# iceprincefounder/ZeldaEngine

Hardware: AMD Instinct MI355X
Metric: Mpixels/s shaded (deferred PBR, 1080p, 100k meshlets) + achieved HBM GB/s (higher is better)
Workload: dtype f32

## Files before the change

### include/zelda_render.h

```cpp
#ifndef ZELDA_RENDER_H
#define ZELDA_RENDER_H

#include "zelda_abi.h"

#ifdef __cplusplus
extern "C" {
#endif

#define ZR_OK            0
#define ZR_ERR_ARG      -1
#define ZR_ERR_DEVICE   -2
#define ZR_ERR_OOM      -3
#define ZR_ERR_PARSE    -4
#define ZR_ERR_IO       -5
#define ZR_ERR_STATE    -6
#define ZR_ERR_OVERFLOW -7
#define ZR_ERR_UNSUPPORTED -8

#define ZR_ABI_VERSION 7u

#ifndef ZR_TILE
#define ZR_TILE 32
#endif

// ... 90 lines not shown
int  zr_object_set_instance_visibility(zr_ctx* ctx, uint32_t index, uint32_t first, const uint8_t* visible, uint32_t n);
int  zr_object_update_instance_visibility_async(zr_ctx* ctx, uint32_t index, uint32_t first, const uint32_t* idx_dev,
                                                const uint8_t* visible_dev, uint32_t n, void* hip_stream);
int  zr_object_get_visibility(zr_ctx* ctx, uint32_t index, int* object_visible, uint8_t* dst, uint32_t* n);
int  zr_mesh_set_vertices(zr_ctx* ctx, uint32_t mesh_id, uint32_t first, const XkVertex* v, uint32_t n);
int  zr_mesh_update_vertices_async(zr_ctx* ctx, uint32_t mesh_id, uint32_t first, const XkVertex* v_dev, uint32_t n, void* hip_stream);
int  zr_mesh_get_vertices(zr_ctx* ctx, uint32_t mesh_id, XkVertex* dst, uint32_t* n);
int  zr_object_set_texture(zr_ctx* ctx, uint32_t index, uint32_t slot, const zr_image* img);
int  zr_object_update_texture_async(zr_ctx* ctx, uint32_t index, uint32_t slot, const void* rgba8_dev, uint32_t width, uint32_t height,
                                    void* hip_stream);
int  zr_object_get_texture(zr_ctx* ctx, uint32_t index, uint32_t slot, uint32_t level, uint8_t* dst, size_t cap, uint32_t* w, uint32_t* h,
                           uint32_t* levels);
int  zr_set_cubemap(zr_ctx* ctx, const uint8_t* const faces[6], uint32_t dim);

int  zr_set_skydome(zr_ctx* ctx, const XkVertex* v, uint32_t nv, const uint32_t* idx, uint32_t ni, const zr_image* tex);
int  zr_set_background(zr_ctx* ctx, const zr_image* tex);
int  zr_set_sky_flags(zr_ctx* ctx, int enable_skydome, int enable_background);

int  zr_update_uniforms(zr_ctx* ctx, const zr_camera* cam,
                        const XkLight* dir, uint32_t n_dir, const XkLight* point, uint32_t n_point,
                        const XkLight* spot, uint32_t n_spot, float roll_stage, float roll_light, float time);
int  zr_set_frame(zr_ctx* ctx, const XkUniformBufferMVP* camera, const XkUniformBufferMVP* shadow, const XkView* view);
int  zr_get_frame(zr_ctx* ctx, XkUniformBufferMVP* camera, XkUniformBufferMVP* shadow, XkView* view);
int  zr_set_debug_view(zr_ctx* ctx, uint32_t spec_constants);
#define ZR_SHADING_DEFERRED 0u
#define ZR_SHADING_FORWARD  1u
int  zr_set_shading(zr_ctx* ctx, uint32_t mode);

int  zr_render(zr_ctx* ctx);
int  zr_render_shadow(zr_ctx* ctx);
int  zr_render_gbuffer(zr_ctx* ctx);
int  zr_render_lighting(zr_ctx* ctx);
int  zr_render_geometry(zr_ctx* ctx);
int  zr_stream_wait_shadow(zr_ctx* ctx, void* hip_stream);
int  zr_finish(zr_ctx* ctx);
int  zr_get_pass_times(zr_ctx* ctx, float ms[ZR_PASS_COUNT]);
int  zr_get_pass_times_avg(zr_ctx* ctx, uint32_t last_n, float ms[ZR_PASS_COUNT]);
int  zr_get_frame_latencies(zr_ctx* ctx, uint32_t n, float* ms);
int  zr_get_frame_periods(zr_ctx* ctx, uint32_t n, float* ms);
int  zr_set_timing_interval(zr_ctx* ctx, uint32_t interval);
int  zr_get_stats(zr_ctx* ctx, zr_stats* out, size_t bytes);
#define ZR_LIGHT_PLANE_IGNORED 0u
#define ZR_LIGHT_PLANE_FILLED  1u
#define ZR_LIGHT_PLANE_READ    2u
typedef struct zr_light_keep {
    uint32_t last, _pad;
    uint64_t ignored, filled, read;
    uint64_t plane_bytes;
    uint64_t read_by_arg;
} zr_light_keep;
int  zr_get_light_keep(zr_ctx* ctx, zr_light_keep* out, size_t bytes);
int  zr_get_rest_settled(zr_ctx* ctx, uint32_t* parts, uint32_t* settled);
int  zr_get_rest_settled_parts(zr_ctx* ctx, uint8_t* standing, size_t bytes);

int  zr_read_color(zr_ctx* ctx, uint8_t* rgba8, size_t bytes);
int  zr_read_gbuffer(zr_ctx* ctx, int target, void* dst, size_t bytes);
int  zr_read_shadowmap(zr_ctx* ctx, float* dst, size_t bytes);
int  zr_copy_frame_async(zr_ctx* ctx, void* color_dev, void* shadow_dev);

typedef struct zr_frame_delta {
    uint32_t n_tiles;
    uint32_t total_tiles;
    uint32_t full;
    uint32_t serial;
} zr_frame_delta;
int  zr_set_frame_delta(zr_ctx* ctx, int enable);
int  zr_frame_delta_reset(zr_ctx* ctx);
int  zr_read_frame_delta(zr_ctx* ctx, uint32_t* tiles, uint32_t cap_tiles, uint8_t* pixels, size_t bytes, zr_frame_delta* out, size_t out_bytes);
int  zr_copy_frame_delta_async(zr_ctx* ctx, void* header_dev, void* tiles_dev, void* pixels_dev);

#define ZR_FRAME_DELTA_PACKED 3
#define ZR_FRAME_DELTA_RECORD_MAX 4104u
typedef struct zr_frame_delta_packed {
    uint32_t n_tiles, total_tiles, full, serial;
    uint32_t bytes;
    uint32_t raw_tiles;
    uint32_t reserved[2];
} zr_frame_delta_packed;
int  zr_read_frame_delta_packed(zr_ctx* ctx, uint32_t* tiles, uint32_t cap_tiles, uint32_t* offsets, uint32_t cap_offsets, uint8_t* stream, size_t cap_bytes,
                                zr_frame_delta_packed* out, size_t out_bytes);
int  zr_copy_frame_delta_packed_async(zr_ctx* ctx, void* header_dev, void* tiles_dev, void* offsets_dev, void* stream_dev);
int  zr_frame_delta_decode(const uint32_t* tiles, const uint32_t* offsets, uint32_t n, const uint8_t* stream, size_t bytes, uint32_t width, uint32_t height,
                           uint8_t* client_rgba8);

int  zr_frame_scaled_extent(uint32_t width, uint32_t height, uint32_t scale, uint32_t* w, uint32_t* h);
int  zr_frame_downscale(const uint8_t* rgba8, uint32_t width, uint32_t height, uint32_t scale, uint8_t* dst, size_t bytes);
int  zr_read_color_scaled(zr_ctx* ctx, uint32_t scale, uint8_t* rgba8, size_t bytes);
int  zr_copy_frame_scaled_async(zr_ctx* ctx, uint32_t scale, void* color_dev);
int  zr_set_frame_delta_scale(zr_ctx* ctx, uint32_t scale);
int  zr_get_frame_delta_extent(zr_ctx* ctx, uint32_t* width, uint32_t* height, uint32_t* total_tiles, uint32_t* scale);

typedef struct zr_highlight_style {
    uint8_t  outline[4];
    uint8_t  fill[4];
    uint32_t radius;
    uint32_t reserved;
} zr_highlight_style;
int  zr_highlight_set(zr_ctx* ctx, uint32_t object, uint32_t first, const uint8_t* on, uint32_t n);
int  zr_highlight_clear(zr_ctx* ctx);
int  zr_highlight_get(zr_ctx* ctx, uint8_t* dst, size_t bytes);
int  zr_set_highlight_style(zr_ctx* ctx, const zr_highlight_style* style, size_t bytes);
int  zr_get_highlight_style(zr_ctx* ctx, zr_highlight_style* style, size_t bytes);
int  zr_read_color_highlighted(zr_ctx* ctx, uint32_t scale, uint8_t* rgba8, size_t bytes);
int  zr_copy_frame_highlighted_async(zr_ctx* ctx, uint32_t scale, void* color_dev);
int  zr_set_frame_delta_highlight(zr_ctx* ctx, int on);
int  zr_frame_highlight(const uint8_t* rgba8, const uint8_t* mask, uint32_t width, uint32_t height, const zr_highlight_style* style, size_t style_bytes,
// ... 113 lines not shown
```

### zeldaengine_amd/abi.py

```python
import ctypes as C

import numpy as np

MAX_DIRECTIONAL_LIGHTS = 16
MAX_POINT_LIGHTS = 512
MAX_SPOT_LIGHTS = 16
SHADOWMAP_DIM = 1024
TILE = 32

XkVertex = np.dtype([("Position", "<f4", 3), ("Normal", "<f4", 3), ("Color", "<f4", 3), ("TexCoord", "<f4", 2)])
XkInstanceData = np.dtype([("InstancePosition", "<f4", 3), ("InstanceRotation", "<f4", 3), ("InstancePScale", "<f4"),
                           ("InstanceTexIndex", "u1"), ("_pad", "u1", 3)])
XkMeshlet = np.dtype([("VertexOffset", "<u4"), ("VertexCount", "<u4"), ("TriangleOffset", "<u4"), ("TriangleCount", "<u4"),
                      ("BoundsCenter", "<f4", 3), ("BoundsRadius", "<f4"), ("ConeApex", "<f4", 3), ("ConeAxis", "<f4", 3),
                      ("ConeCutoff", "<f4"), ("BindlessContext", "<u4")])
XkMeshletFileVertex = np.dtype([("pos", "<f4", 3), ("nrm", "<f4", 3), ("uv", "<f4", 2)])
XkLight = np.dtype([("Position", "<f4", 4), ("Color", "<f4", 4), ("Direction", "<f4", 4), ("LightInfo", "<f4", 4)])
XkUniformBufferMVP = np.dtype([("Model", "<f4", 16), ("View", "<f4", 16), ("Proj", "<f4", 16)])
XkView = np.dtype([("ViewProjSpace", "<f4", 16), ("ShadowmapSpace", "<f4", 16), ("LocalToWorld", "<f4", 16),
                   ("CameraInfo", "<f4", 4), ("ViewportInfo", "<f4", 4),
                   ("DirectionalLights", XkLight, MAX_DIRECTIONAL_LIGHTS), ("PointLights", XkLight, MAX_POINT_LIGHTS),
                   ("SpotLights", XkLight, MAX_SPOT_LIGHTS), ("LightsCount", "<i4", 4),
                   ("Time", "<f4"), ("zNear", "<f4"), ("zFar", "<f4")])

# ... 38 lines not shown
    "zr_copy_frame_scaled_async": [vp_, u32_, vp_],
    "zr_set_frame_delta_scale": [vp_, u32_],
    "zr_get_frame_delta_extent": [vp_, C.POINTER(u32_), C.POINTER(u32_), C.POINTER(u32_), C.POINTER(u32_)],
}
FRAME_SCALE_MAX = 8


class HighlightStyle(C.Structure):
    _fields_ = [("outline", C.c_uint8 * 4), ("fill", C.c_uint8 * 4), ("radius", C.c_uint32), ("reserved", C.c_uint32)]


assert C.sizeof(HighlightStyle) == 16
HIGHLIGHT_RADIUS_MAX = 8
HIGHLIGHT_SIGNATURES = {
    "zr_highlight_set": [vp_, u32_, u32_, vp_, u32_],
    "zr_highlight_clear": [vp_],
    "zr_highlight_get": [vp_, vp_, C.c_size_t],
    "zr_set_highlight_style": [vp_, C.POINTER(HighlightStyle), C.c_size_t],
    "zr_get_highlight_style": [vp_, C.POINTER(HighlightStyle), C.c_size_t],
    "zr_read_color_highlighted": [vp_, u32_, vp_, C.c_size_t],
    "zr_copy_frame_highlighted_async": [vp_, u32_, vp_],
    "zr_set_frame_delta_highlight": [vp_, C.c_int],
    "zr_frame_highlight": [vp_, vp_, u32_, u32_, C.POINTER(HighlightStyle), C.c_size_t, vp_, C.c_size_t],
}


class OverlaySegment(C.Structure):
    _fields_ = [("a", C.c_float * 3), ("b", C.c_float * 3), ("rgba", C.c_uint8 * 4), ("flags", C.c_uint32)]


class OverlayStyle(C.Structure):
    _fields_ = [("depth_bias", C.c_float), ("hidden_opacity", C.c_uint32), ("reserved", C.c_uint32 * 2)]


assert C.sizeof(OverlaySegment) == 32 and C.sizeof(OverlayStyle) == 16
OVERLAY_SEGMENT = np.dtype([("a", "<f4", 3), ("b", "<f4", 3), ("rgba", "u1", 4), ("flags", "<u4")])
assert OVERLAY_SEGMENT.itemsize == 32
OVERLAY_XRAY = 1
OVERLAY_MAX_SEGMENTS = 16384
OVERLAY_SIGNATURES = {
    "zr_overlay_set": [vp_, vp_, u32_],
    "zr_overlay_get": [vp_, vp_, C.POINTER(u32_)],
    "zr_set_overlay_style": [vp_, C.POINTER(OverlayStyle), C.c_size_t],
    "zr_get_overlay_style": [vp_, C.POINTER(OverlayStyle), C.c_size_t],
    "zr_read_color_overlaid": [vp_, u32_, C.c_int, vp_, C.c_size_t],
    "zr_copy_frame_overlaid_async": [vp_, u32_, C.c_int, vp_],
    "zr_set_frame_delta_overlay": [vp_, C.c_int],
    "zr_frame_overlay": [vp_, vp_, u32_, u32_, vp_, vp_, u32_, C.POINTER(OverlayStyle), C.c_size_t, vp_, C.c_size_t],
}
REST_SETTLE_SIGNATURES = {
    "zr_get_rest_settled": [C.c_void_p, C.POINTER(C.c_uint32), C.POINTER(C.c_uint32)],
    "zr_get_rest_settled_parts": [C.c_void_p, C.c_void_p, C.c_size_t],
}
EXTENT_SIGNATURES = {
    "zr_resize": [vp_, u32_, u32_],
    "zr_get_extent": [vp_, C.POINTER(u32_), C.POINTER(u32_)],
}
del vp_, u32_


def make_highlight_style(outline=(255, 160, 0, 255), fill=(255, 160, 0, 0), radius=2):
    return HighlightStyle((C.c_uint8 * 4)(*outline), (C.c_uint8 * 4)(*fill), radius, 0)


def make_overlay_style(depth_bias=0.0, hidden_opacity=0):
    return OverlayStyle(depth_bias, hidden_opacity, (C.c_uint32 * 2)(0, 0))


def make_overlay_segments(segments):
    if isinstance(segments, np.ndarray) and segments.dtype == OVERLAY_SEGMENT:
        return np.ascontiguousarray(segments).reshape(-1)
    rows = [tuple(s) for s in segments]
    out = np.zeros(len(rows), dtype=OVERLAY_SEGMENT)
    for i, s in enumerate(rows):
        out[i]["a"], out[i]["b"], out[i]["rgba"], out[i]["flags"] = s[0:3], s[3:6], s[6:10], s[10] if len(s) > 10 else 0
    return out


class Camera(C.Structure):
    _fields_ = [("Position", C.c_float * 3), ("Lookat", C.c_float * 3), ("Speed", C.c_float), ("FOV", C.c_float),
                ("zNear", C.c_float), ("zFar", C.c_float)]


class Config(C.Structure):
    _fields_ = [("width", C.c_uint32), ("height", C.c_uint32), ("shadow_dim", C.c_uint32), ("debug_view", C.c_uint32),
                ("device", C.c_int32), ("tile_rank", C.c_uint32), ("tile_world", C.c_uint32), ("flags", C.c_uint32)]


class Stats(C.Structure):
    _fields_ = [("work_items", C.c_uint64 * 2), ("survivors", C.c_uint64 * 2), ("bin_entries", C.c_uint64 * 2),
                ("covered_pixels", C.c_uint64), ("covered_shadow_texels", C.c_uint64), ("overflow", C.c_uint32), ("hiz_culled", C.c_uint32),
                ("round1_survivors", C.c_uint64), ("shadow_occluded", C.c_uint32), ("shadow_late", C.c_uint32),
                ("hiz_culled_geom", C.c_uint32), ("struct_bytes", C.c_uint32)]


class LightKeep(C.Structure):
    _fields_ = [("last", C.c_uint32), ("_pad", C.c_uint32), ("ignored", C.c_uint64), ("filled", C.c_uint64), ("read", C.c_uint64),
                ("plane_bytes", C.c_uint64), ("read_by_arg", C.c_uint64)]


LIGHT_PLANE_IGNORED, LIGHT_PLANE_FILLED, LIGHT_PLANE_READ = 0, 1, 2


class WorldDelta(C.Structure):
    _fields_ = [("struct_bytes", C.c_uint32), ("differs", C.c_uint32), ("scene_changed", C.c_uint32), ("objects_kept", C.c_uint32),
                ("objects_reinstanced", C.c_uint32), ("objects_added", C.c_uint32), ("objects_removed", C.c_uint32),
# ... 98 lines not shown
```

### zeldaengine_amd/csrc/zr_context.cpp

```cpp
#include "zr_ctx.h"
#include "zr_math.h"

#include <algorithm>
#include <cmath>
#include <cstring>
#include <cstdlib>

int zr_fail(zr_ctx* c, int code, const std::string& msg)
{
    if (c) { try { c->err = msg; } catch (...) { c->err.clear(); } }
    return code;
}

int zr_stage_idle(zr_ctx* c, const char* what, bool hint)
{
    if (c->stage == 0) return ZR_OK;
    return zr_fail(c, ZR_ERR_STATE, std::string(what) + (hint ? " between the stages of a frame (finish it with zr_render_lighting first)"
                                                              : " between the stages of a frame"));
}

hipError_t zr_sync_all(zr_ctx* c)
{
    hipError_t e = hipStreamSynchronize(c->stream);
    if (e == hipSuccess && c->cam_s) e = hipStreamSynchronize(c->cam_s);
// ... 30 lines not shown

#ifndef ZR_CAM_PRIORITY
#define ZR_CAM_PRIORITY 0
#endif
#ifndef ZR_TILE_WG_PER_CU
#define ZR_TILE_WG_PER_CU 12u
#endif

static int create_device_state(zr_ctx* c)
{
    ZrOwn& A = c->own;
    HIPCHK(c, A.stream(&c->own_stream));
    c->stream = c->own_stream;
    for (auto& fr : c->timed) for (auto& e : fr.ev) HIPCHK(c, A.event(&e));
    for (auto& e : c->ev_end) HIPCHK(c, A.event(&e));
    for (FrameCopy& F : c->fc) HIPCHK(c, A.event(&F.ev_ids, hipEventDisableTiming));
    for (FrameCopy& F : c->fc) {
        HIPCHK(c, A.alloc(&F.shadow, (size_t)c->SD * c->SD)); HIPCHK(c, A.alloc(&F.view, 1)); HIPCHK(c, A.alloc(&F.empty_rgba, 1));
    }
    HIPCHK(c, A.alloc(&c->d_stats, 1));
    HIPCHK(c, A.alloc(&c->d_sstats, 1));
    for (auto& r : c->d_rstats) HIPCHK(c, A.alloc(&r, 1));
    c->cov_block = c->d_stats;
    HIPCHK(c, A.alloc(&c->d_lut, 256));
    HIPCHK(c, hipMemcpy(c->d_lut, c->lut, sizeof c->lut, hipMemcpyHostToDevice));
    {
        std::vector<float> ul(1280);
        for (int i = 0; i < 256; ++i) {
            ul[(size_t)i] = (float)i / 255.0f;
            if (fmaf((float)i, ZR_UNORM8_HI, (float)i * ZR_UNORM8_LO) != ul[(size_t)i])
                return zr_fail(c, ZR_ERR_DEVICE, "ZR_UNORM8_HI / ZR_UNORM8_LO do not decode c / 255 exactly");
        }
        for (int i = 0; i < 1024; ++i) ul[256 + (size_t)i] = (float)i / 1023.0f;
        HIPCHK(c, A.alloc(&c->d_unorm_lut, ul.size()));
        HIPCHK(c, hipMemcpy(c->d_unorm_lut, ul.data(), ul.size() * 4, hipMemcpyHostToDevice));
    }

    c->stiles_x = (c->SD + ZR_TILE - 1) / ZR_TILE; c->stiles_y = c->stiles_x; c->sn_tiles = c->stiles_x * c->stiles_y;
    if (c->sn_tiles > 16000u) return zr_fail(c, ZR_ERR_ARG, "too many tiles");
    std::vector<uint32_t> sowned(c->sn_tiles);
    for (uint32_t t = 0; t < c->sn_tiles; ++t) sowned[t] = t;
    HIPCHK(c, upload(A, &c->d_sowned, sowned));
    {
        HIPCHK(c, A.alloc(&c->d_clear_px, 64));
        uint32_t px[16] = { 0 };
        px[0] = 0x3F800000u;
        px[1] = 0xFF000000u; px[2] = 0u; px[3] = 0xFF000000u; px[4] = 0xFF000000u;
        px[6] = 0u; px[7] = 0x3C000000u;
        px[8] = 0u;
        HIPCHK(c, hipMemcpy(c->d_clear_px, px, sizeof px, hipMemcpyHostToDevice));
        uint32_t* w = (uint32_t*)c->d_clear_px;
        c->Gclear.depth = (float*)w; c->Gclear.scene_color = w + 1; c->Gclear.gA = w + 2; c->Gclear.gB = w + 3; c->Gclear.gC = w + 4;
        c->Gclear.gD = (uint2*)(w + 6); c->Gclear.overlay = w + 8;
    }
    {
#ifdef ZR_DIAG
        const char* e;
        if ((e = getenv("ZR_DEBUG_SKIP"))) c->env_skip = (uint32_t)atoi(e);
        if ((e = getenv("ZR_DEBUG_SKIP_LIGHT"))) c->env_skip_light = (uint32_t)atoi(e);
        if ((e = getenv("ZR_LIGHT_LIST_MIN"))) c->env_light_list_min = atoi(e);
        c->env_no_empty_px = getenv("ZR_NO_EMPTY_PIXEL") != nullptr;
#endif
        c->lk.settle_off = getenv("ZR_NO_REST_SETTLE") != nullptr;
        c->end.every = ZR_REST_END_EVERY_DEFAULT;
        if (const char* r = getenv("ZR_REST_END_EVERY")) { const int v = atoi(r); c->end.every = v < 1 ? 1u : (uint32_t)v > kZrEndEveryMax ? kZrEndEveryMax : (uint32_t)v; }
    }
    HIPCHK(c, A.host(&c->h_view_ring, zr_ctx::VIEW_RING));
    for (auto& e : c->view_ev) HIPCHK(c, A.event(&e, hipEventDisableTiming));
    {
        int least = 0, greatest = 0;
        (void)hipDeviceGetStreamPriorityRange(&least, &greatest);
        HIPCHK(c, A.stream(&c->cam_s, ZR_CAM_PRIORITY == 2 ? greatest : ZR_CAM_PRIORITY == 1 ? (least + greatest) / 2 : least));
    }
    HIPCHK(c, A.event(&c->ev_cam, hipEventDisableTiming)); HIPCHK(c, A.event(&c->ev_join, hipEventDisableTiming));
    HIPCHK(c, A.event(&c->ev_lane, hipEventDisableTiming));
    { hipDeviceProp_t prop; if (hipGetDeviceProperties(&prop, c->device) == hipSuccess && prop.multiProcessorCount > 0) c->raster_blocks = (uint32_t)prop.multiProcessorCount * ZR_TILE_WG_PER_CU; }
    c->shadow_blocks = c->raster_blocks / ZR_TILE_WG_PER_CU * 8u;
    c->slow0_cap = std::max<uint32_t>(c->slow0_cap, 128u * c->sn_tiles);
    HIPCHK(c, A.alloc(&c->d_slow0, 4ull * c->slow0_cap));
#ifdef ZR_DIAG
    if (const char* e = getenv("ZR_RASTER_BLOCKS")) c->raster_blocks = (uint32_t)std::max(1, atoi(e));
    if (const char* e = getenv("ZR_SHADOW_BLOCKS")) c->shadow_blocks = (uint32_t)std::max(1, atoi(e));
#endif
    HIPCHK(c, zr_fill_sync({ { c->d_stats, 0, sizeof(ZrDevStats) }, { c->d_sstats, 0, sizeof(ZrDevStats) },
                             { c->d_rstats[0], 0, sizeof(ZrDevStats) }, { c->d_rstats[1], 0, sizeof(ZrDevStats) } }));
    if (int rc = zr_extent_create(c)) return rc;
    for (auto& fr : c->timed) for (auto& e : fr.ev) HIPCHK(c, hipEventRecord(e, c->stream));
    for (auto& e : c->ev_end) HIPCHK(c, hipEventRecord(e, c->stream));
    for (auto& e : c->view_ev) HIPCHK(c, hipEventRecord(e, c->stream));
    HIPCHK(c, hipStreamSynchronize(c->stream));
    return ZR_OK;
}

extern "C" int zr_create(const zr_config* cfg, zr_ctx** out)
{
    if (!cfg || !out) return ZR_ERR_ARG;
    return zr_guard(nullptr, [&]() -> int {
        *out = nullptr;
        if (cfg->width == 0 || cfg->height == 0 || cfg->width > 255u * ZR_TILE || cfg->height > 255u * ZR_TILE) return ZR_ERR_ARG;
        int ndev = 0;
        if (hipGetDeviceCount(&ndev) != hipSuccess || ndev <= 0) return ZR_ERR_DEVICE;
        if (cfg->device < 0 || cfg->device >= ndev) return ZR_ERR_DEVICE;
        if (hipSetDevice(cfg->device) != hipSuccess) return ZR_ERR_DEVICE;
        zr_ctx* c = new zr_ctx();
        c->cfg = *cfg;
        if (c->cfg.tile_world == 0) c->cfg.tile_world = 1;
// ... 63 lines not shown
```

### zeldaengine_amd/csrc/zr_ctx.h

```cpp
#pragma once

#include <atomic>
#include <functional>
#include <initializer_list>
#include <map>
#include <mutex>
#include <new>
#include <stdexcept>
#include <string>
#include <thread>
#include <utility>
#include <vector>

#include "zr_frame_end.h"
#include "zr_frame_plan.h"
#include "zr_ids.h"
#include "zr_meshlet.h"
#include "zr_overlay.h"
#include "zr_scale.h"
#include "zr_settle.h"
#include "zr_timed.h"
#include "zr_types.h"
#include "zr_world_doc.h"

// ... 59 lines not shown
    ZrMeshletSet ms;
    bool has_meshlets = false, uploaded = false;
    float center[3] = { 0, 0, 0 }; float radius = 0;
    XkVertex* d_v = nullptr; ZrRVertex* d_rv = nullptr; ZrRVertex* d_rt = nullptr; uint32_t* d_idx = nullptr; XkMeshlet* d_meshlets = nullptr;
    float4* d_mpos = nullptr; float4* d_mbox = nullptr; uint2* d_mtri = nullptr; uint32_t* d_tri_meshlet = nullptr;
    ZrMeshState upd = {}; bool stale[2] = { false, false }, v_stale = false, ml_stale = false;
};

struct ZrMaterialHost {
    uint32_t texel[7]; float bc_linear[3];
    std::vector<uint8_t> image[7];
    uint32_t w[7], h[7];
};

struct ZrSceneObject {
    ZrOwn mem;
    ZrOwn tex_mem;
    uint32_t mesh = 0, n_inst = 1; bool instanced = false;
    std::vector<XkInstanceData> inst;
    ZrInstance* d_inst = nullptr;
    XkInstanceData* d_raw = nullptr;
    ZrInstanceState upd = {}; uint32_t pending[2] = { 0, 0 }; bool tab1 = false, host_stale = false; uint32_t draw = 0;
    bool hidden = false, flag_pending[2] = { false, false }, vis_stale = false;
    std::vector<uint8_t> vis;
    uint32_t texel[7]; float bc_linear[3];
    uint8_t* d_tex[8] = { nullptr, nullptr, nullptr, nullptr, nullptr, nullptr, nullptr, nullptr };
    uint32_t tex_w[8] = { 0 }, tex_h[8] = { 0 }, tex_levels[8] = { 0 };
    bool mixed_sizes = false;
    std::string profab; uint32_t profab_model = 0; bool from_world = false, mat_pristine = false;
    uint32_t work_base = 0, work_inst = 0, work_meshlets = 0; bool work_valid = false;
};

static const struct { uint32_t ch, n; } kSlotPack[7] = { { ZR_PK_BC, 3 }, { ZR_PK_ME, 1 }, { ZR_PK_RO, 1 }, { ZR_PK_NO, 3 }, { ZR_PK_AO, 1 }, { ZR_PK_EM, 3 }, { ZR_PK_MS, 1 } };
static inline uint32_t zr_mip_next(uint32_t d) { return d > 1 ? d >> 1 : 1; }
struct ZrMipLevel { uint32_t w, h; size_t off; };
static inline ZrMipLevel zr_mip_level(uint32_t w, uint32_t h, uint32_t level)
{
    ZrMipLevel L = { w, h, 0 };
    for (uint32_t l = 0; l < level; ++l) { L.off += (size_t)L.w * L.h; L.w = zr_mip_next(L.w); L.h = zr_mip_next(L.h); }
    return L;
}

struct ZrProfab { uint32_t mesh; ZrMaterialHost mat; };

struct FrameCopy {
    GBufferPtrs G = {};
    float* shadow = nullptr; XkView* view = nullptr;
    uint32_t* empty_rgba = nullptr;
    uint32_t* prim_plane = nullptr;
    bool overlay_dirty = false;
    bool shadow_cleared = false;
    uint64_t view_uploaded = 0;
    uint64_t g_gen = 0;
    hipEvent_t ev_ids = nullptr; bool ids_wait = false;
};

struct ZrDeltaBuffers {
    ZrOwn mem, codec_mem;
    uint32_t *delivered = nullptr, *list = nullptr, *header = nullptr, *scaled = nullptr; uint8_t *packed = nullptr, *flags = nullptr;
    zr_frame_delta* h_header = nullptr;
    struct Codec {
        bool on = false; uint16_t* lens = nullptr; uint32_t *header = nullptr, *offsets = nullptr; uint8_t* stream = nullptr;
        zr_frame_delta_packed* h_header = nullptr;
    } codec;
};

struct zr_ctx {
    ZrOwn own, ext, pool_tiles;
    zr_config cfg;
    int device = 0;
    hipStream_t own_stream = nullptr, stream = nullptr;
    std::string err;

    std::vector<ZrMesh> meshes;
    std::vector<ZrSceneObject> objects;
    bool scene_dirty = true;
    ZrObject* d_objs = nullptr; uint32_t n_objs = 0, n_work = 0;
    ZrObject* d_objs_b[2] = { nullptr, nullptr }; ZrOwn tables;
    struct Update {
        uint64_t reader[2] = { 0, 0 };
        hipEvent_t ev_scatter = nullptr, ev_apply = nullptr; hipStream_t scatter_s = nullptr, apply_s = nullptr;
        bool scatter_wait[2] = { false, false }, apply_done = false, dual = false;
        static constexpr int RING = 4;
        struct Stage { ZrOwn mem; uint8_t* h = nullptr; uint8_t* d = nullptr; size_t cap = 0; hipEvent_t ev = nullptr; } ring[RING];
        uint32_t slot = 0;
        hipEvent_t ev_tex = nullptr; hipStream_t tex_s = nullptr; bool tex_wait = false; float* d_srgb_thr = nullptr;
    } upd;
    ZrFrameFacts facts; ZrFramePlan plan; ZrFrameCarry carry;
    ZrPass list_key[2] = {}, smap_key = {}, cam_prev_key = {};
    ZrPass pass[2]; bool pass_live[2] = { false, false };
    uint64_t caster_epoch = 0, camera_epoch = 0, surface_epoch = 0;
    int smap = 0; uint64_t shadow_draws = 0, cam_draws = 0;

    XkUniformBufferMVP cam, shadow; XkView view; bool frame_valid = false;
    struct Lens { bool valid = false; float fov = 0, zn = 0, zf = 0; } lens;
    uint32_t debug_view = 0;
    uint32_t shading = 0;

    uint32_t W = 0, H = 0, SD = 0;
    uint32_t tiles_x = 0, tiles_y = 0, n_tiles = 0, n_owned = 0, slots_per_rank = 0;
    uint32_t stiles_x = 0, stiles_y = 0, sn_tiles = 0;
    uint32_t *d_owned = nullptr, *d_sowned = nullptr;
    uint32_t* d_tile_map = nullptr;
    struct ZrDist* dist = nullptr;
    uint32_t* d_color = nullptr; uint32_t* d_tiles = nullptr;
    float* d_shadow_ext = nullptr;
    uint32_t shadow_rank = 0, shadow_world = 1; int stage = 0;
    uint32_t stile_rank = 0, stile_world = 1, s_slots_per_rank = 0, n_sowned_rank = 0;
    uint32_t *d_sowned_rank = nullptr, *d_stile_map = nullptr; ZrOwn stile_mem;
    uint32_t* d_tiles_ext = nullptr;

    ZrOwn pools;
    struct CullList { uint32_t *rects = nullptr, *work = nullptr; } sc[2];
    struct ShadowBins { uint32_t *tile_count = nullptr, *tile_offset = nullptr, *tile_cursor = nullptr, *chunk_offset = nullptr;
                        ZrBinEntry* bins = nullptr; uint4* chunk_tab = nullptr; } sb;
    uint32_t bucket_pct = 100;
    ZrTriBins tb = {};
    uint32_t chunk_capacity = 0;
    uint32_t n_inst_total = 0;
    uint8_t* d_clear_px = nullptr; GBufferPtrs Gclear = {}; bool empty_ready = false;
    uint32_t env_skip = 0, env_skip_light = 0; int32_t env_light_list_min = 4; bool env_no_empty_px = false;
    static constexpr int VIEW_RING = kZrViewRing;
    XkView* h_view_ring = nullptr; hipEvent_t view_ev[VIEW_RING] = {}; uint32_t view_slot = 0; bool view_dirty = true;
    uint64_t view_version = 1;
    FrameCopy fc[2]; int fcur = 0;
    hipStream_t cam_s = nullptr;
    hipEvent_t ev_join = nullptr, ev_cam = nullptr;
    ZrPass resolve_P; uint32_t resolve_mark = 0;
    hipEvent_t ev_lane = nullptr;
    unsigned long long* d_sky_keys = nullptr; uint32_t sky_object = 0;
    static constexpr int END_RING = kZrEndRing;
    hipEvent_t ev_end[END_RING] = {}; ZrEndState end;
    unsigned long long* d_vis[2] = { nullptr, nullptr }; uint32_t raster_blocks = 2048, shadow_blocks = 2048;
    uint4* d_slow0 = nullptr; uint32_t slow0_cap = 1u << 18;
    uint32_t work_capacity = 0, bin_capacity = 0; bool any_images = false, mixed_images = false;
    uint32_t limit_record_chunks = 0, limit_slow_triangles = 0;
    uint2* d_pxrect = nullptr; float* d_zmin = nullptr; uint8_t* d_visflag[2] = { nullptr, nullptr };
    uint2* d_spxrect = nullptr; float* d_szmin = nullptr; uint8_t* d_sflag = nullptr;
    bool history_remap = false; uint64_t history_items = 0;
    uint32_t sflag_turn = 0;
    float* d_hiz = nullptr; ZrHiz hiz = {}; int vis_cur = 0; bool last_two_round = false;
    uint32_t vis_mark_prev = 0;
    uint32_t* d_hiz_regions = nullptr; uint32_t n_hiz_regions = 0;
    ZrDevStats* d_stats = nullptr; ZrDevStats h_stats = {};
    ZrDevStats* d_sstats = nullptr;
    ZrDevStats* d_rstats[2] = { nullptr, nullptr }; ZrDevStats* cov_block = nullptr;
    uint64_t last_work[2] = { 0, 0 };

    bool id_capture = false;
    bool ids_frame = false, ids_this = false;
    uint64_t scene_gen = 0;
    struct Ids {
        uint64_t gen = 0, table_gen = ~0ull;
        ZrOwn table, pool;
        ZrIdsDraw* draws = nullptr; uint32_t n_draws = 0, n_slots = 0, slot_cap = 0;
        uint32_t *counts = nullptr, *cov = nullptr, *list = nullptr, *n = nullptr;
        unsigned long long* keys = nullptr; zr_hit* hits = nullptr; uint2* obj = nullptr;
    } ids;

    struct Delta { bool on = false, full = true; uint32_t serial = 0, scale = 1; ZrDeltaBuffers b; } delta;
    uint32_t* d_scaled = nullptr;
    struct Highlight {
        std::vector<uint8_t> set; uint64_t set_gen = ~0ull; bool dirty = true, delta = false;
        zr_highlight_style style = { { 255, 160, 0, 255 }, { 255, 160, 0, 0 }, 2u, 0u };
        ZrOwn bits_mem; uint32_t* bits = nullptr; size_t bits_words = 0;
        unsigned long long* plane = nullptr; uint32_t* frame = nullptr;
    } hl;

    ZrOwn cube_mem; CubeDesc cube = {}; uint32_t cube_dim = 0, cube_levels = 0;
    uint64_t cube_gen = 0;
    struct LightKey {
        float SB[16], cam[3]; uint32_t SD, n_dir, max_mips, cube_dim, cube_levels, debug_skip;
        XkLight dir[XK_MAX_DIRECTIONAL_LIGHTS_NUM];
// ... 149 lines not shown
```

### zeldaengine_amd/csrc/zr_dev.h

```cpp
#pragma once
#include "zr_math.h"
#include "zr_types.h"

#include <algorithm>
#include <cstddef>

#define WAVE 64
#define TILE ZR_TILE
#define TILE_PIX (TILE * TILE)
#ifndef ZR_SHADOW_APRON
#define ZR_SHADOW_APRON 12
#endif
#define SPAN(MODE) ((MODE) == ZR_MODE_SHADOW ? TILE + ZR_SHADOW_APRON : TILE)
#define SPAN_PIX(MODE) (SPAN(MODE) * SPAN(MODE))
#define QCAP 128u
#define RW (ZR_TILE >= 64 ? 8 : 4)
#define RTHREADS (RW * WAVE)
#ifndef ZR_RASTER_WAVES_DEFER
#define ZR_RASTER_WAVES_DEFER 6
#endif
#ifdef ZR_DIAG
#define ZR_DIAG_SKIP(x) (x)
#else
#define ZR_DIAG_SKIP(x) 0u
// ... 235 lines not shown
    if (VEC) return *reinterpret_cast<const uint4*>(p);
    v.x = p[0];
    if (px + 1u < W) v.y = p[1];
    if (px + 2u < W) v.z = p[2];
    if (px + 3u < W) v.w = p[3];
    return v;
}
template <bool VEC> __device__ __forceinline__ void plane_store4(uint32_t* __restrict__ plane, uint32_t W, uint32_t H, uint32_t px, uint32_t py, uint4 v)
{
    if (py >= H || px >= W) return;
    uint32_t* p = plane + (size_t)py * W + px;
    if (VEC) { *reinterpret_cast<uint4*>(p) = v; return; }
    p[0] = v.x;
    if (px + 1u < W) p[1] = v.y;
    if (px + 2u < W) p[2] = v.z;
    if (px + 3u < W) p[3] = v.w;
}

__device__ __forceinline__ bool hiz_occluded(const ZrHiz& Z, uint2 pr, float zmin)
{
    if (!(zmin >= 0.0f)) return false;
    const uint32_t x0 = pr.x & 0xFFFFu, y0 = pr.x >> 16, x1 = pr.y & 0xFFFFu, y1 = pr.y >> 16;
    uint32_t l = 0;
    while (l < 4u && (((x1 >> (2u + l)) - (x0 >> (2u + l))) > 3u || ((y1 >> (2u + l)) - (y0 >> (2u + l))) > 3u)) ++l;
    const uint32_t sh = 2u + l;
    const uint32_t tx0 = x0 >> sh, ty0 = y0 >> sh, tx1 = x1 >> sh, ty1 = y1 >> sh;
    if (tx1 - tx0 > 3u || ty1 - ty0 > 3u) return false;
    const float* __restrict__ L = l == 0u ? Z.fine : Z.lvl[l - 1u];
    const uint32_t hw = l == 0u ? Z.fw : Z.hw[l - 1u];
    float hmax = 0.0f;
#pragma unroll
    for (uint32_t j = 0; j < 4u; ++j)
#pragma unroll
        for (uint32_t i = 0; i < 4u; ++i)
            hmax = __builtin_fmaxf(hmax, L[(size_t)min(ty0 + j, ty1) * hw + min(tx0 + i, tx1)]);
    return zmin > hmax;
}

#ifndef ZR_LIGHT_TB
#define ZR_LIGHT_TB 512
#endif
#ifndef ZR_LIGHT_WAVES
#define ZR_LIGHT_WAVES 6
#endif
#ifndef ZR_LIGHT_KEPT_TB
#define ZR_LIGHT_KEPT_TB 512
#endif
#ifndef ZR_LIGHT_KEPT_WAVES
#define ZR_LIGHT_KEPT_WAVES 8
#endif
#ifndef ZR_REST_RECORDS_ONE_TRIP
#define ZR_REST_RECORDS_ONE_TRIP 1
#endif
#ifndef ZR_PIXELS_PER_THREAD
#define ZR_PIXELS_PER_THREAD 1
#endif
static_assert(TILE_PIX / ZR_PIXELS_PER_THREAD >= ZR_LIGHT_KEPT_TB, "a tile's threads must fill at least one workgroup");
static_assert(TILE_PIX / ZR_PIXELS_PER_THREAD >= ZR_LIGHT_TB && TILE_PIX / ZR_PIXELS_PER_THREAD >= 256, "a tile's threads must fill at least one workgroup");
#ifndef ZR_RESOLVE_TB
#define ZR_RESOLVE_TB 256
#endif
```

### zeldaengine_amd/csrc/zr_frame_host.cpp

```cpp
#include "zr_ctx.h"
#include "zr_math.h"

#include <cmath>
#include <cstring>

static_assert(ZRP_NO_HIZ == ZR_FLAG_NO_HIZ && ZRP_SERIAL_PASSES == ZR_FLAG_SERIAL_PASSES && ZRP_NO_LIST_REUSE == ZR_FLAG_NO_LIST_REUSE &&
              ZRP_NO_SHADOW_OCCLUSION == ZR_FLAG_NO_SHADOW_OCCLUSION && ZRP_SHADOW_OCCLUSION == ZR_FLAG_SHADOW_OCCLUSION &&
              ZRP_SHADING_FORWARD == ZR_SHADING_FORWARD, "zr_frame_plan.h: flags");
static_assert((int)ZR_ROUNDS_ONE == ZR_PLAN_ONE_ROUND && (int)ZR_ROUNDS_TWO == ZR_PLAN_DREW_ROUND2 && (int)ZR_ROUNDS_TWO_KEPT == ZR_PLAN_KEPT_ROUND2, "zr_frame_plan.h: rounds");
static_assert(ZR_TILE == 32, "the triangle-binned camera pass and the shadow pass's occlusion culling are written for 32 x 32 tiles");


static float radiansf(float deg) { return deg * 0.01745329251994329576923690768489f; }
static void perspective_rh_zo(float fovy, float aspect, float zn, float zf, float* m)
{
    const float t = tanf(fovy / 2.0f);
    memset(m, 0, 64);
    m[0] = 1.0f / (aspect * t); m[5] = 1.0f / t; m[10] = zf / (zn - zf); m[11] = -1.0f; m[14] = -(zf * zn) / (zf - zn);
}
static void look_at_rh(zf3 eye, zf3 center, zf3 up, float* m)
{
    const zf3 f = zr_normalize_ieee(center - eye);
    const zf3 s = zr_normalize_ieee(zr_cross(f, up));
    const zf3 u = zr_cross(s, f);
// ... 336 lines not shown
{
    const ZrFramePlan& p = c->plan;
    if (p.shadow == ZR_LANE_NONE) TIMED(c, EV_SHADOW_BINS, EV_SHADOW);
    else if (int rc = shadow_draw(c, lane_stream(c, p.shadow))) return rc;
    if (p.ev_join) HIPCHK(c, hipEventRecord(c->ev_join, c->stream));
    return ZR_OK;
}

static int gbuffer_pass(zr_ctx* c)
{
    const ZrFramePlan& p = c->plan;
    if (p.camera == ZR_LANE_NONE) {
        TIMED(c, EV_CAMERA, EV_CULL, EV_ROUND1, EV_HIZ, EV_ROUND2, EV_RESOLVE);
        return ZR_OK;
    }
    const hipStream_t s = lane_stream(c, p.camera);
    TIMED(c, EV_CAMERA);
    ZrPass P = c->pass[1];
    c->last_work[1] = P.n_work;
    ZrHiz Z = c->hiz;
    Z.tiles_x = c->tiles_x; Z.tile_rank = c->cfg.tile_rank; Z.tile_world = c->cfg.tile_world;
    Z.pxrect = p.hiz_on ? c->d_pxrect : nullptr; Z.zmin = p.hiz_on ? c->d_zmin : nullptr;
    Z.vis_prev = c->d_visflag[c->vis_cur ^ 1]; Z.vis_now = p.hiz_on ? c->d_visflag[c->vis_cur] : nullptr;
    const uint32_t vis_mark = 1u + (uint32_t)(c->cam_draws % 255u);
    Z.vis_stamp = c->vis_mark_prev;
    Z.phase = 0;
    c->last_two_round = p.rounds != ZR_ROUNDS_ONE;
    zr_launch_cull_box(P, c->d_objs, c->sc[1].work, c->sc[1].rects, Z, c->d_stats, 1, s, c->tb.sel, c->last_two_round ? Z.vis_prev : nullptr, p.camera_list_reuse);
    TIMED(c, EV_CULL);
    if (c->last_two_round) Z.phase = 1;
    tri_raster(c, P, Z, 1, s, p.rounds != ZR_ROUNDS_TWO, p.count_first);
    TIMED(c, EV_ROUND1);
    if (p.rounds == ZR_ROUNDS_TWO) {
        zr_launch_hiz_build(c->d_vis[c->fcur], c->W, c->H, Z, c->d_hiz_regions, c->n_hiz_regions, s);
        Z.phase = 2;
        tri_select(c, P, Z, 2, s);
        TIMED(c, EV_HIZ);
        tri_raster(c, P, Z, 2, s, true, false);
    } else
        TIMED(c, EV_HIZ);
    {
        const bool sky = c->sky_set && c->sky_enabled;
        P.write_overlay = (sky || c->fc[c->fcur].overlay_dirty) ? 1u : 0u;
        c->fc[c->fcur].overlay_dirty = sky;
        P.sky_keys = nullptr; P.sky_object = c->sky_object;
        if (sky && c->d_sky_keys) { zr_launch_sky_tiles(P, c->d_objs, c->d_owned, c->n_owned, c->d_sky_keys, s); P.sky_keys = c->d_sky_keys; }
    }
    TIMED(c, EV_ROUND2);
    if (p.resolve_deferred) {
        zr_launch_mark(P, c->d_objs, c->d_owned, c->n_owned, c->d_vis[c->fcur], Z.vis_now, s, vis_mark);
        TIMED(c, EV_MARK);
        c->resolve_P = P; c->resolve_mark = vis_mark;
    } else {
        zr_launch_resolve_gbuffer(P, c->d_objs, c->d_owned, c->n_owned, c->d_vis[c->fcur], c->fc[c->fcur].G, c->d_lut, c->d_unorm_lut, Z.vis_now, c->d_stats, s, vis_mark);
        c->cov_block = c->d_stats; c->fc[c->fcur].g_gen = p.g_gen;
        TIMED(c, EV_RESOLVE);
    }
    if (p.ev_cam == ZR_EVCAM_BEHIND_MARK || p.ev_cam == ZR_EVCAM_BEHIND_RESOLVE) HIPCHK(c, hipEventRecord(c->ev_cam, s));
    c->vis_mark_prev = vis_mark; c->cam_draws++;
    if (P.n_work != 0) zr_launch_plan(c->tb, c->d_owned, c->n_owned, c->d_stats, false, c->bucket_pct, s, p.rounds);
    if (p.hiz_on) c->vis_cur ^= 1;
    HIPCHK(c, hipGetLastError());
    c->cam_prev_key = c->pass[1]; c->carry = zr_frame_carry(c->carry, c->facts, p, ZR_STAGE_CAMERA);
    return ZR_OK;
}

extern "C" int zr_render_gbuffer(zr_ctx* c)
{
    if (!c) return ZR_ERR_ARG;
    return zr_guard(c, [&]() -> int {
        if (c->stage != 1) return zr_fail(c, ZR_ERR_STATE, "zr_render_gbuffer out of order");
        HIPCHK(c, hipSetDevice(c->device));
        const int rc = gbuffer_pass(c);
        if (rc == ZR_OK) c->stage = 2;
        return rc;
    });
}

extern "C" int zr_stream_wait_shadow(zr_ctx* c, void* hip_stream)
{
    if (!c) return ZR_ERR_ARG;
    return zr_guard(c, [&]() -> int {
        HIPCHK(c, hipStreamWaitEvent((hipStream_t)hip_stream, c->ev_join, 0));
        return ZR_OK;
    });
}

static int geometry_passes(zr_ctx* c, ZrEntry entry)
{
    const ZrFramePlan& p = c->plan;
    int rc = frame_begin(c, entry);
    if (rc == ZR_OK) rc = shadow_pass(c);
    if (rc == ZR_OK) rc = gbuffer_pass(c);
    if (rc == ZR_OK && p.one_pixel == ZR_LANE_CAM) rc = empty_pixel_pass(c);
    if (rc == ZR_OK && (p.ev_cam == ZR_EVCAM_BEHIND_ONE_PIXEL || p.ev_cam == ZR_EVCAM_LANE_END)) HIPCHK(c, hipEventRecord(c->ev_cam, c->cam_s));
    if (rc == ZR_OK) c->stage = 2;
    return rc;
}

extern "C" int zr_render_shadow(zr_ctx* c)
{
    if (!c) return ZR_ERR_ARG;
    return zr_guard(c, [&]() -> int {
        int rc = frame_begin(c, ZR_ENTRY_STAGED);
        if (rc == ZR_OK) rc = shadow_pass(c);
        if (rc == ZR_OK) c->stage = 1;
        return rc;
    });
}

extern "C" int zr_render_geometry(zr_ctx* c)
{
    if (!c) return ZR_ERR_ARG;
    return zr_guard(c, [&]() -> int { return geometry_passes(c, ZR_ENTRY_GEOMETRY); });
}

static int deferred_resolve(zr_ctx* c)
{
    const hipStream_t s = lane_stream(c, c->plan.resolve);
    ZrDevStats* const tally = c->d_rstats[c->fcur];
    zr_launch_fill32(tally->covered_part, 0u, 32, s);
    TIMED(c, EV_HOST_RESOLVE);
    zr_launch_resolve_gbuffer(c->resolve_P, c->d_objs, c->d_owned, c->n_owned, c->d_vis[c->fcur], c->fc[c->fcur].G, c->d_lut, c->d_unorm_lut, nullptr, tally, s, c->resolve_mark);
    TIMED(c, EV_RESOLVE);
    c->cov_block = tally; c->fc[c->fcur].g_gen = c->plan.g_gen;
    HIPCHK(c, hipGetLastError());
    return ZR_OK;
}

extern "C" int zr_render_lighting(zr_ctx* c)
{
    if (!c) return ZR_ERR_ARG;
    return zr_guard(c, [&]() -> int {
        if (c->stage != 2) return zr_fail(c, ZR_ERR_STATE, "zr_render_lighting out of order");
        HIPCHK(c, hipSetDevice(c->device));
        const ZrFramePlan& p = c->plan;
        if (p.host_waits_ev_cam) HIPCHK(c, hipStreamWaitEvent(lane_stream(c, p.lighting), c->ev_cam, 0));
        int rc = p.resolve_deferred ? deferred_resolve(c) : ZR_OK;
        if (rc == ZR_OK && p.one_pixel != ZR_LANE_CAM) rc = empty_pixel_pass(c);
        if (rc == ZR_OK) rc = lighting_pass(c);
        return rc;
    });
}

extern "C" int zr_render(zr_ctx* c)
{
    if (!c) return ZR_ERR_ARG;
    return zr_guard(c, [&]() -> int {
        int rc = geometry_passes(c, ZR_ENTRY_RENDER);
        if (rc == ZR_OK) rc = zr_render_lighting(c);
        if (rc != ZR_OK) c->stage = 0;
        return rc;
    });
}

extern "C" int zr_set_shadow_partition(zr_ctx* c, uint32_t rank, uint32_t world)
{
    if (!c) return ZR_ERR_ARG;
    return zr_guard(c, [&]() -> int {
        ARGCHK(c, world >= 1 && rank < world);
        if (world > 1 && c->stile_world > 1) return zr_fail(c, ZR_ERR_STATE, "zr_set_shadow_partition: the map is already owned by tiles (zr_set_shadow_tiles)");
        c->shadow_rank = rank; c->shadow_world = world; zr_casters_changed(c);
        return ZR_OK;
    });
}

extern "C" int zr_set_shadow_tiles(zr_ctx* c, uint32_t rank, uint32_t world)
{
    if (!c) return ZR_ERR_ARG;
    return zr_guard(c, [&]() -> int {
        ARGCHK(c, world >= 1 && rank < world);
        if (int rc = zr_stage_idle(c, "zr_set_shadow_tiles", false)) return rc;
        if (world > 1 && c->shadow_world > 1) return zr_fail(c, ZR_ERR_STATE, "zr_set_shadow_tiles: the casters are already split by instance (zr_set_shadow_partition)");
        HIPCHK(c, hipSetDevice(c->device));
        HIPCHK(c, zr_sync_all(c));
        c->stile_mem.release(); c->d_sowned_rank = c->d_stile_map = nullptr;
        c->stile_rank = 0; c->stile_world = 1; c->s_slots_per_rank = c->sn_tiles; c->n_sowned_rank = 0;
        zr_history_forgotten(c, ZR_HIST_SHADOW_LIST); zr_casters_changed(c);
// ... 52 lines not shown
```

### zeldaengine_amd/csrc/zr_lighting.hip

```cpp
#include "zr_dev.h"
#include "zr_surface.h"
#include "zr_shade.h"

__device__ __forceinline__ bool light_pixel_empty(uint32_t sc, uint32_t A, uint32_t B, uint32_t Cc, uint2 D)
{
    return sc == 0xFF000000u && A == 0u && B == 0xFF000000u && Cc == 0xFF000000u && D.x == 0u && D.y == 0x3C000000u;
}

struct LitPixel { zf3 BaseColor, Normal, N, Pw; float Metallic, Roughness, AO, Mask; };
__device__ __forceinline__ LitPixel light_decode(const float* u8, const float* u10, uint32_t sc, uint32_t A, uint32_t B, uint32_t Cc, uint2 D)
{
    LitPixel q;
    q.BaseColor = zr3(u8[Cc & 255u], u8[(Cc >> 8) & 255u], u8[(Cc >> 16) & 255u]);
    q.Metallic = zr_saturate(u8[B & 255u]);
    q.Roughness = zr_saturate(u8[(B >> 16) & 255u]);
    q.Normal = zr3(__builtin_fmaf(u10[(A >> 20) & 1023u], 2.0f, -1.0f), __builtin_fmaf(u10[(A >> 10) & 1023u], 2.0f, -1.0f),
                   __builtin_fmaf(u10[A & 1023u], 2.0f, -1.0f));
    q.AO = zr_saturate(u8[Cc >> 24]);
    q.Mask = u8[sc >> 24];
    q.Roughness = __builtin_fmaxf(0.01f, q.Roughness);
    q.N = zr_normalize(q.Normal);
    q.Pw = zr3(f16_to_f32_hw(D.x & 0xFFFFu), f16_to_f32_hw(D.x >> 16), f16_to_f32_hw(D.y & 0xFFFFu));
    return q;
}
__device__ __forceinline__ uint32_t light_compose(const ZrLightParams& L, const LitPixel& q, zf3 Direct, zf3 Indirect, zf3 RefC, float ShadowFactor, int px, int py)
{
    zf3 Final = ((Direct + Indirect) + RefC) * q.Mask;
    Final = gamma3(Final);
    zf3 o;
    switch (L.debug_view) {
    case 0: o = Final; break;
    case 1: o = gamma3(q.BaseColor); break;
    case 2: o = zr3(q.Metallic, q.Metallic, q.Metallic); break;
    case 3: o = zr3(q.Roughness, q.Roughness, q.Roughness); break;
    case 4: o = q.Normal; break;
    case 5: o = zr3(q.AO, q.AO, q.AO); break;
    case 7: o = RefC; break;
    case 8: o = zr3(ShadowFactor, ShadowFactor, ShadowFactor); break;
    case 9: o = Final; break;
    case 6: {
        const float u = ((float)px + 0.5f) / (float)L.W, v = ((float)py + 0.5f) / (float)L.H;
        o = v >= u ? zr3(1.0f - v, u, v - u) : zr3(1.0f - u, v, u - v);
        break;
    }
    default: o = Final * ShadowFactor; break;
    }
    return pack_rgb8(o);
}
template <int TB>
__device__ __forceinline__ void light_clear_next_slice(const ZrLightParams& L)
{
    if (!L.clear_next) return;
    const uint32_t per = (L.clear_n + gridDim.x - 1u) / gridDim.x, b = blockIdx.x * per;
    for (uint32_t i = threadIdx.x; i < per && b + i < L.clear_n; i += (uint32_t)TB) L.clear_next[b + i] = 0x3F800000u;
}

template <bool LIGHT_LIST, bool BACKGROUND, int TB, int PPT, uint32_t MODE>
__global__ __launch_bounds__(TB) __attribute__((amdgpu_waves_per_eu(MODE == ZR_LIGHT_KEPT ? ZR_LIGHT_KEPT_WAVES : ZR_LIGHT_WAVES, MODE == ZR_LIGHT_KEPT ? ZR_LIGHT_KEPT_WAVES : ZR_LIGHT_WAVES))) void k_lighting(ZrLightParams L, const XkView* __restrict__ view,
                                                  const uint32_t* __restrict__ owned_tiles, GBufferPtrs G,
                                                  const float* __restrict__ shadowmap, CubeDesc C,
                                                  const float* __restrict__ srgb_lut, const float* __restrict__ unorm_lut,
                                                  uint32_t* __restrict__ out, float4* __restrict__ plane, float4* __restrict__ rest)
{
    __shared__ float tl[512];
    __shared__ float u10[1024];
    float* const slut = tl; float* const u8 = tl + 256;
    constexpr uint32_t T = TILE_PIX / (uint32_t)PPT, PARTS = T / (uint32_t)TB, WAVES = (uint32_t)TB / 64u;
    const uint32_t tid = threadIdx.x + (blockIdx.x % PARTS) * (uint32_t)TB;
    const uint32_t tile_slot = blockIdx.x / PARTS;
    for (uint32_t i = threadIdx.x; i < 256u; i += (uint32_t)TB) { u8[i] = unorm_lut[i]; slut[i] = srgb_lut[i]; }
    for (uint32_t i = threadIdx.x; i < 1024u; i += (uint32_t)TB) u10[i] = unorm_lut[256u + i];
    __syncthreads();
    light_clear_next_slice<TB>(L);
    const uint32_t tile = owned_tiles[tile_slot];
    const int tx0 = (int)(tile % L.tiles_x) * TILE, ty0 = (int)(tile / L.tiles_x) * TILE;
    const zf3 cam = zr3(view->CameraInfo[0], view->CameraInfo[1], view->CameraInfo[2]);
    const uint32_t nDir = (uint32_t)view->LightsCount[0], nPoint = (uint32_t)view->LightsCount[1];
    const float maxmips = (float)(uint32_t)view->LightsCount[3];
    const float dxy = 1.5f * 1.0f / (float)L.SD;

    __shared__ float bbp[LIGHT_LIST ? WAVES : 1][6];
    __shared__ uint32_t lmask[LIGHT_LIST ? XK_MAX_POINT_LIGHTS_NUM / 32 : 1];
    constexpr bool use_mask = LIGHT_LIST;
    constexpr bool RECORDS = MODE == ZR_LIGHT_FILL && PPT == 1;
    if constexpr (LIGHT_LIST || RECORDS) {
        float lo[3] = { __builtin_inff(), __builtin_inff(), __builtin_inff() }, hi[3] = { -__builtin_inff(), -__builtin_inff(), -__builtin_inff() };
        bool odd = false;
        bool empty = false;
        for (uint32_t i = tid; i < TILE_PIX; i += T) {
            const int px = tx0 + (int)(i & (TILE - 1)), py = ty0 + (int)(i / TILE);
            if (px >= (int)L.W || py >= (int)L.H) continue;
            const size_t p = (size_t)py * L.W + (size_t)px;
            if constexpr (RECORDS) empty = light_pixel_empty(G.scene_color[p], G.gA[p], G.gB[p], G.gC[p], G.gD[p]);
            if ((G.scene_color[p] >> 24) == 0u) continue;
            const uint2 D = G.gD[p];
            const float q[3] = { f16_to_f32_hw(D.x & 0xFFFFu), f16_to_f32_hw(D.x >> 16), f16_to_f32_hw(D.y & 0xFFFFu) };
            for (int a = 0; a < 3; ++a) {
                if (!(__builtin_fabsf(q[a]) <= 3.402823466e38f)) odd = true;
                lo[a] = __builtin_fminf(lo[a], q[a]); hi[a] = __builtin_fmaxf(hi[a], q[a]);
            }
        }
        for (int a = 0; a < 3; ++a) { lo[a] = wave_fmin(lo[a]); hi[a] = wave_fmax(hi[a]); }
        const bool wodd = __ballot(odd) != 0ull;
        if constexpr (RECORDS) {
            const unsigned long long em = __ballot(empty);
            if (rest != nullptr && (threadIdx.x & 63u) == 0u) {
                ZrRestRecord* r = (ZrRestRecord*)(rest + ZR_REST_SLOT) + ((size_t)tile_slot * ZR_REST_RECORDS_PER_TILE + (tid >> 6));
                for (int a = 0; a < 3; ++a) { r->lo[a] = wodd ? -__builtin_inff() : lo[a]; r->hi[a] = wodd ? __builtin_inff() : hi[a]; }
                r->empty[0] = (uint32_t)em; r->empty[1] = (uint32_t)(em >> 32);
            }
        }
        if constexpr (LIGHT_LIST) {
            if ((threadIdx.x & 63u) == 0u) {
                float* o = bbp[threadIdx.x >> 6];
                o[0] = wodd ? -__builtin_inff() : lo[0]; o[1] = wodd ? -__builtin_inff() : lo[1]; o[2] = wodd ? -__builtin_inff() : lo[2];
                o[3] = wodd ? __builtin_inff() : hi[0]; o[4] = wodd ? __builtin_inff() : hi[1]; o[5] = wodd ? __builtin_inff() : hi[2];
            }
            for (uint32_t i = threadIdx.x; i < XK_MAX_POINT_LIGHTS_NUM / 32; i += (uint32_t)TB) lmask[i] = 0u;
            __syncthreads();
            float blo[3], bhi[3];
            for (int a = 0; a < 3; ++a) {
                blo[a] = bbp[0][a]; bhi[a] = bbp[0][3 + a];
                for (uint32_t w = 1; w < WAVES; ++w) { blo[a] = __builtin_fminf(blo[a], bbp[w][a]); bhi[a] = __builtin_fmaxf(bhi[a], bbp[w][3 + a]); }
            }
            for (uint32_t li = threadIdx.x; li < nPoint; li += (uint32_t)TB)
                if (light_listed(ViewLight{ &view->PointLights[li] }, blo, bhi)) atomicOr(&lmask[li >> 5], 1u << (li & 31u));
            __syncthreads();
        }
    }

    for (uint32_t i = tid; i < TILE_PIX; i += T) {
        const int px = tx0 + (int)(i & (TILE - 1)), py = ty0 + (int)(i / TILE);
        if (px >= (int)L.W || py >= (int)L.H) continue;
        const size_t p = (size_t)py * L.W + (size_t)px;
        const uint32_t sc = G.scene_color[p], A = G.gA[p], B = G.gB[p], Cc = G.gC[p];
        const uint2 D = G.gD[p];
        if (L.empty_rgba != nullptr && sc == 0xFF000000u && A == 0u && B == 0xFF000000u && Cc == 0xFF000000u && D.x == 0u && D.y == 0x3C000000u) {
            light_emit<BACKGROUND>(L, G, tl, out, *L.empty_rgba, px, py, p, tile_slot, i);
            continue;
        }
        const LitPixel q = light_decode(u8, u10, sc, A, B, Cc, D);
        zf3 Direct, Indirect, RefC; float ShadowFactor;
        if constexpr (MODE == ZR_LIGHT_KEPT) {
            const float4 ka = plane[p], kb = plane[(size_t)L.W * L.H + p];
            Direct = zr3(ka.x, ka.y, ka.z); ShadowFactor = ka.w; RefC = zr3(kb.x, kb.y, kb.z);
            shade_points<use_mask>(L, view, lmask, nDir, nPoint, cam, q.BaseColor, q.Metallic, q.Roughness, q.N, q.Pw, Direct);
            Indirect = shade_indirect(q.BaseColor, q.Metallic, q.AO, ShadowFactor);
        } else if constexpr (MODE == ZR_LIGHT_FILL) {
            shade_standing(L, view, shadowmap, C, slut, nDir, maxmips, dxy, cam, q.BaseColor, q.Metallic, q.Roughness, q.N, q.AO, q.Pw, Direct, RefC, ShadowFactor);
            plane[p] = make_float4(Direct.x, Direct.y, Direct.z, ShadowFactor);
            plane[(size_t)L.W * L.H + p] = make_float4(RefC.x, RefC.y, RefC.z, 0.0f);
            shade_points<use_mask>(L, view, lmask, nDir, nPoint, cam, q.BaseColor, q.Metallic, q.Roughness, q.N, q.Pw, Direct);
            Indirect = shade_indirect(q.BaseColor, q.Metallic, q.AO, ShadowFactor);
        } else
            shade_surface<use_mask>(L, view, shadowmap, C, slut, lmask, nDir, nPoint, maxmips, dxy, cam, q.BaseColor, q.Metallic, q.Roughness, q.N, q.AO, q.Pw,
                                    Direct, Indirect, RefC, ShadowFactor);
        light_emit<BACKGROUND>(L, G, tl, out, light_compose(L, q, Direct, Indirect, RefC, ShadowFactor, px, py), px, py, p, tile_slot, i);
    }
}

#if ZR_PIXELS_PER_THREAD == 1
template <uint32_t WAVES>
__device__ __forceinline__ uint32_t rest_records_fetch(const float4* __restrict__ rest, uint32_t first_record)
{
    constexpr uint32_t RECW = (uint32_t)(sizeof(ZrRestRecord) / 4u);
    const uint32_t* __restrict__ w = (const uint32_t*)(rest + ZR_REST_SLOT) + (size_t)first_record * RECW;
    return w[((threadIdx.x & 7u) % WAVES) * RECW + ((threadIdx.x >> 3) & 7u)];
}

template <bool LIGHT_LIST, bool BACKGROUND, int TB>
__global__ __launch_bounds__(TB) __attribute__((amdgpu_waves_per_eu(ZR_LIGHT_KEPT_WAVES, ZR_LIGHT_KEPT_WAVES)))
void k_lighting_rest(ZrLightParams L, ZrRestArgs R, const uint32_t* __restrict__ owned_tiles, GBufferPtrs G, const float* __restrict__ srgb_lut,
                     const float* __restrict__ unorm_lut, uint32_t* __restrict__ out, const float4* __restrict__ plane, const float4* __restrict__ rest)
{
    static_assert(sizeof(ZrLightParams) + sizeof(ZrRestArgs) + sizeof(GBufferPtrs) + 6 * sizeof(void*) + 256  < 4096,
                  "k_lighting_rest: the argument block");
    constexpr uint32_t PARTS = TILE_PIX / (uint32_t)TB, WAVES = (uint32_t)TB / 64u, NONE = 0xFFFFFFFFu;
    static_assert((WAVES <= 8u || !ZR_REST_RECORDS_ONE_TRIP) && 1536u % (uint32_t)TB == 0u, "k_lighting_rest: a part's records are a dword per lane");
    __shared__ float tab[1536];
    __shared__ uint32_t empty_px;
    __shared__ ZrRestLight lpt[LIGHT_LIST ? ZR_REST_ARG_LIGHTS : 1];
    float* const tl = tab; float* const u8 = tab + 256; float* const u10 = tab + 512;
    const uint32_t part = blockIdx.x % PARTS, tile_slot = blockIdx.x / PARTS;
    const uint32_t i = threadIdx.x + part * (uint32_t)TB;
    const uint32_t first_record = tile_slot * ZR_REST_RECORDS_PER_TILE + part * WAVES;
    uint32_t rec = 0u;
    {
        constexpr uint32_t NT = 1536u / (uint32_t)TB, LW = ZR_REST_ARG_LIGHTS * (uint32_t)(sizeof(ZrRestLight) / 4u), NL = LIGHT_LIST ? (LW + (uint32_t)TB - 1u) / (uint32_t)TB : 0u;
        float tv[NT], lv[NL ? NL : 1u];
#pragma unroll
        for (uint32_t k = 0; k < NT; ++k) { const uint32_t j = threadIdx.x + k * (uint32_t)TB; tv[k] = j < 256u ? srgb_lut[j] : unorm_lut[j - 256u]; }
#pragma unroll
        for (uint32_t k = 0; k < NL; ++k) { const uint32_t j = threadIdx.x + k * (uint32_t)TB; lv[k] = ((const float*)R.pt)[LW % (uint32_t)TB == 0u || j < LW ? j : 0u]; }
        if (ZR_REST_RECORDS_ONE_TRIP) rec = rest_records_fetch<WAVES>(rest, first_record);
#pragma unroll
        for (uint32_t k = 0; k < NT; ++k) tab[threadIdx.x + k * (uint32_t)TB] = tv[k];
#pragma unroll
        for (uint32_t k = 0; k < NL; ++k) { const uint32_t j = threadIdx.x + k * (uint32_t)TB; if (LW % (uint32_t)TB == 0u || j < LW) ((float*)lpt)[j] = lv[k]; }
    }
    const uint32_t tile = owned_tiles[tile_slot];
    __syncthreads();
    light_clear_next_slice<TB>(L);
    const int tx0 = (int)(tile % L.tiles_x) * TILE, ty0 = (int)(tile / L.tiles_x) * TILE;
    const zf3 cam = zr3(R.cam[0], R.cam[1], R.cam[2]);

    const uint32_t wave = (uint32_t)__builtin_amdgcn_readfirstlane((int)(threadIdx.x >> 6));
    float blo[3] = { __builtin_inff(), __builtin_inff(), __builtin_inff() }, bhi[3] = { -__builtin_inff(), -__builtin_inff(), -__builtin_inff() };
    uint32_t first = NONE;
    unsigned long long mine = 0ull;
#if ZR_REST_RECORDS_ONE_TRIP
    if constexpr (LIGHT_LIST) {
        int lo, hi;
        { const int idn = 0x7F800000; int r = (int)rec; ZR_DPP_STEP(op_fmin, 0x111, 0xF); ZR_DPP_STEP(op_fmin, 0x112, 0xF); ZR_DPP_STEP(op_fmin, 0x114, 0xF); lo = r; }
        { const int idn = (int)0xFF800000; int r = (int)rec; ZR_DPP_STEP(op_fmax, 0x111, 0xF); ZR_DPP_STEP(op_fmax, 0x112, 0xF); ZR_DPP_STEP(op_fmax, 0x114, 0xF); hi = r; }
        for (int a = 0; a < 3; ++a) { blo[a] = zr_u2f((uint32_t)__builtin_amdgcn_readlane(lo, 8 * a + 7)); bhi[a] = zr_u2f((uint32_t)__builtin_amdgcn_readlane(hi, 8 * (3 + a) + 7)); }
    }
    {
        const uint32_t lane = threadIdx.x & 63u;
        const unsigned long long nz64 = __ballot(lane >= 48u && (lane & 7u) < WAVES && rec != 0u);
        const uint32_t nz = ((uint32_t)(nz64 >> 48) | (uint32_t)(nz64 >> 56)) & 255u;
        if (nz != 0u) {
            const int w0 = __builtin_ctz(nz);
// ... 192 lines not shown
        if (!(__builtin_fabsf(x) < 1.0e9f)) x = 0.0f;
        if (!(__builtin_fabsf(y) < 1.0e9f)) y = 0.0f;
        const float fx = __builtin_floorf(x), fy = __builtin_floorf(y);
        const float ax = __builtin_floorf(__builtin_fmaf(x - fx, 256.0f, 0.5f)) / 256.0f;
        const float ay = __builtin_floorf(__builtin_fmaf(y - fy, 256.0f, 0.5f)) / 256.0f;
        const int x0 = wrap_index((int)fx, (int)L.W), x1 = wrap_index((int)fx + 1, (int)L.W);
        const int y0 = wrap_index((int)fy, (int)L.H), y1 = wrap_index((int)fy + 1, (int)L.H);
        const GTexel t00 = gbuffer_texel(G, L.W, x0, y0), t10 = gbuffer_texel(G, L.W, x1, y0);
        const GTexel t01 = gbuffer_texel(G, L.W, x0, y1), t11 = gbuffer_texel(G, L.W, x1, y1);
        float g[20];
        for (int k = 0; k < 20; ++k) {
            const float top = __builtin_fmaf(ax, t10.v[k] - t00.v[k], t00.v[k]), bot = __builtin_fmaf(ax, t11.v[k] - t01.v[k], t01.v[k]);
            g[k] = __builtin_fmaf(ay, bot - top, top);
        }
        const zf3 BaseColor = zr3(g[12], g[13], g[14]);
        const float Metallic = zr_saturate(g[8]);
        const float Roughness = __builtin_fmaxf(0.01f, zr_saturate(g[10]));
        const zf3 Normal = zr3(__builtin_fmaf(g[4], 2.0f, -1.0f), __builtin_fmaf(g[5], 2.0f, -1.0f), __builtin_fmaf(g[6], 2.0f, -1.0f));
        const float AO = zr_saturate(g[15]);
        const zf3 N = zr_normalize(Normal);
        const zf3 Pw = zr3(g[16], g[17], g[18]);
        switch (cell) {
        case 0: o = gamma3(BaseColor); break;
        case 1: o = zr3(Metallic, Metallic, Metallic); break;
        case 2: o = zr3(Roughness, Roughness, Roughness); break;
        case 3: o = N; break;
        case 4: o = zr3(AO, AO, AO); break;
        case 5: o = zr3(0.0f, 0.0f, 0.0f); break;
        case 6: {
            const zf3 cam = zr3(view->CameraInfo[0], view->CameraInfo[1], view->CameraInfo[2]);
            const zf3 Vv = zr_normalize(cam - Pw), Nn = zr_normalize(N);
            o = cube_sample(C, srgb_lut, L.cube_dim, (int)L.cube_levels, shade_refract(Nn, Vv), 0.0f) * 10.0f;
            break;
        }
        default: {
            const zf4 s4 = zr_mat4_point(L.SB, Pw);
            const float sx = s4.x / s4.w, sy = s4.y / s4.w, sz = s4.z / s4.w, sw = s4.w / s4.w;
            const float dxy = 1.5f * 1.0f / (float)L.SD;
            float sum = 0.0f;
            for (int xo = -2; xo <= 2; ++xo)
                for (int yo = -2; yo <= 2; ++yo) sum += shadow_tap(shadowmap, (int)L.SD, sx, sy, sz, sw, dxy * (float)xo, dxy * (float)yo);
            const float sf = sum * 0.04f;
            o = zr3(sf, sf, sf);
            break;
        }
        }
    }
    out[(size_t)py * L.W + px] = pack_rgb8(o);
}


void zr_launch_lighting(const ZrLightParams& L, const XkView* view, const uint32_t* owned_tiles, uint32_t n_owned,
                        const GBufferPtrs& G, const float* shadowmap, const CubeDesc& C, const float* lut, const float* unorm_lut,
                        uint32_t* out, hipStream_t s, ZrLightMode mode, float4* plane, float4* rest)
{
    if (n_owned == 0) return;
    if (!plane) mode = ZR_LIGHT_PLAIN;
    if (mode != ZR_LIGHT_FILL) rest = nullptr;
#define ZR_LAUNCH_LIGHTING_TB(LL, BG, TB, MODE) hipLaunchKernelGGL((k_lighting<LL, BG, TB, ZR_PIXELS_PER_THREAD, MODE>), dim3(n_owned * (TILE_PIX / ZR_PIXELS_PER_THREAD / TB)), dim3(TB), 0, s, L, view, owned_tiles, G, shadowmap, C, lut, unorm_lut, out, plane, rest)
#define ZR_LAUNCH_LIGHTING(LL, BG) do { if (mode == ZR_LIGHT_KEPT) ZR_LAUNCH_LIGHTING_TB(LL, BG, ZR_LIGHT_KEPT_TB, ZR_LIGHT_KEPT); \
                                        else if (mode == ZR_LIGHT_FILL) ZR_LAUNCH_LIGHTING_TB(LL, BG, ZR_LIGHT_TB, ZR_LIGHT_FILL); \
                                        else ZR_LAUNCH_LIGHTING_TB(LL, BG, ZR_LIGHT_TB, ZR_LIGHT_PLAIN); } while (0)
    if (L.light_list) { if (L.bg_enabled) ZR_LAUNCH_LIGHTING(true, true); else ZR_LAUNCH_LIGHTING(true, false); }
    else { if (L.bg_enabled) ZR_LAUNCH_LIGHTING(false, true); else ZR_LAUNCH_LIGHTING(false, false); }
#undef ZR_LAUNCH_LIGHTING
#undef ZR_LAUNCH_LIGHTING_TB
}
bool zr_lighting_rest_available() { return ZR_PIXELS_PER_THREAD == 1; }
void zr_launch_lighting_rest(const ZrLightParams& L, const ZrRestArgs& R, const uint32_t* owned_tiles, uint32_t n_owned, const GBufferPtrs& G,
                             const float* lut, const float* unorm_lut, uint32_t* out, hipStream_t s, const float4* plane, const float4* rest)
{
#if ZR_PIXELS_PER_THREAD == 1
    if (n_owned == 0) return;
#define ZR_LAUNCH_REST(LL, BG) hipLaunchKernelGGL((k_lighting_rest<LL, BG, ZR_LIGHT_KEPT_TB>), dim3(n_owned * (TILE_PIX / ZR_LIGHT_KEPT_TB)), dim3(ZR_LIGHT_KEPT_TB), 0, s, L, R, owned_tiles, G, lut, unorm_lut, out, plane, rest)
    if (L.light_list) { if (L.bg_enabled) ZR_LAUNCH_REST(true, true); else ZR_LAUNCH_REST(true, false); }
    else { if (L.bg_enabled) ZR_LAUNCH_REST(false, true); else ZR_LAUNCH_REST(false, false); }
#undef ZR_LAUNCH_REST
#endif
}
uint32_t zr_lighting_stand_parts() { return TILE_PIX / ZR_LIGHT_KEPT_TB; }
void zr_launch_lighting_stand(const ZrLightParams& L, const ZrRestArgs& R, const uint32_t* owned_tiles, uint32_t n_owned, const GBufferPtrs& G,
                              const float* lut, const float* unorm_lut, uint32_t* out, hipStream_t s, const float4* plane, const float4* rest,
                              uint32_t* marks, uint32_t gen)
{
#if ZR_PIXELS_PER_THREAD == 1
    if (n_owned == 0) return;
    const dim3 grid(n_owned * (TILE_PIX / ZR_LIGHT_KEPT_TB)), block(ZR_LIGHT_KEPT_TB);
    if (L.bg_enabled) hipLaunchKernelGGL((k_lighting_stand<true, ZR_LIGHT_KEPT_TB>), grid, block, 0, s, L, R, owned_tiles, G, lut, unorm_lut, out, plane, rest, marks, gen);
    else hipLaunchKernelGGL((k_lighting_stand<false, ZR_LIGHT_KEPT_TB>), grid, block, 0, s, L, R, owned_tiles, G, lut, unorm_lut, out, plane, rest, marks, gen);
#endif
}
void zr_launch_gbuffer_vis(const ZrLightParams& L, const XkView* view, const GBufferPtrs& G, const float* shadowmap, const CubeDesc& C,
                           const float* lut, uint32_t* out, hipStream_t s)
{
    hipLaunchKernelGGL(k_gbuffer_vis, dim3((L.W + 15) / 16, (L.H + 15) / 16), dim3(256), 0, s, L, view, G, shadowmap, C, lut, out);
}
```

### zeldaengine_amd/csrc/zr_lighting_host.cpp

```cpp
#include "zr_ctx.h"
#include "zr_math.h"

#include <cstring>

static void light_params(const zr_ctx* c, ZrLightParams* Lp)
{
    ZrLightParams& L = *Lp; memset(&L, 0, sizeof L);
    static const float Bias[16] = { 0.5f, 0, 0, 0, 0, 0.5f, 0, 0, 0, 0, 1, 0, 0.5f, 0.5f, 0, 1 };
    zr_mat4_mul(Bias, c->view.ShadowmapSpace, L.SB);
    L.W = c->W; L.H = c->H; L.SD = c->SD; L.tiles_x = c->tiles_x; L.debug_view = c->debug_view;
    L.cube_dim = c->cube_dim; L.cube_levels = c->cube_levels; L.tile_world = c->cfg.tile_world;
    L.packed_out = (c->cfg.tile_world > 1 || (c->cfg.flags & ZR_FLAG_PACKED_TILES)) ? 1u : 0u;
    L.debug_skip = c->env_skip_light;
    L.bg_enabled = (c->bg_set && c->bg_enabled) ? 1u : 0u;
    L.has_overlay = c->fc[c->fcur].overlay_dirty ? 1u : 0u;
    { const int32_t np = c->view.LightsCount[1]; L.light_list = (np >= c->env_light_list_min && np <= XK_MAX_POINT_LIGHTS_NUM) ? 1u : 0u; }
    L.bg.data = c->d_bg; L.bg.w = c->bg_w; L.bg.h = c->bg_h; L.bg.levels = c->bg_levels; L.bg._pad = 0;
}

static bool empty_px_on(const zr_ctx* c) { return c->shading != ZR_SHADING_FORWARD && c->debug_view != 6u && !c->env_no_empty_px; }

static void light_key(const zr_ctx* c, zr_ctx::LightKey* K)
{
    ZrLightParams L; light_params(c, &L);
// ... 3 lines not shown
    const int32_t nd = c->view.LightsCount[0];
    K->n_dir = (uint32_t)nd;
    for (int32_t i = 0; i < nd && i < XK_MAX_DIRECTIONAL_LIGHTS_NUM; ++i) K->dir[i] = c->view.DirectionalLights[i];
}

static bool rest_launch_fits(const zr_ctx* c)
{
    const int32_t np = c->view.LightsCount[1];
    return np >= 0 && np <= ZR_REST_ARG_LIGHTS && c->lk.rest != nullptr && c->debug_view != 9u;
}

void zr_light_facts(zr_ctx* c, ZrFrameFacts* f)
{
    light_key(c, &c->lk.now);
    f->light_plane_ok = !c->lk.alloc_failed;
    f->light_uniforms_same = c->lk.plane != nullptr && memcmp(&c->lk.now, &c->lk.key, sizeof c->lk.key) == 0;
    f->cube_gen = c->cube_gen;
    f->light_empty_px = empty_px_on(c);
    f->light_slot = zr_lighting_rest_available() && (c->lk.rest != nullptr || (c->lk.plane == nullptr && !c->lk.alloc_failed));
    f->light_by_arg = zr_lighting_rest_available() && f->light_empty_px && rest_launch_fits(c);
}

bool zr_light_plane_make(zr_ctx* c)
{
    if (c->lk.plane) return true;
    if (!c->lk.alloc_failed && c->ext.alloc(&c->lk.plane, 2 * (size_t)c->W * c->H) != hipSuccess) {
        (void)hipGetLastError();
        c->lk.plane = nullptr; c->lk.alloc_failed = true;
    }
    if (c->lk.plane && !c->lk.rest && zr_lighting_rest_available() &&
        c->ext.alloc(&c->lk.rest, ZR_REST_SLOT + (size_t)c->n_owned * ZR_REST_RECORDS_PER_TILE * (sizeof(ZrRestRecord) / sizeof(float4))) != hipSuccess) {
        (void)hipGetLastError();
        c->lk.rest = nullptr;
    }
    if (c->lk.rest && !c->lk.marks && !c->lk.settle_off) {
        const size_t n = (size_t)c->n_owned * zr_lighting_stand_parts();
        if (c->ext.alloc(&c->lk.marks, n) != hipSuccess || hipMemsetAsync(c->lk.marks, 0, (n ? n : 1) * sizeof(uint32_t), c->stream) != hipSuccess) {
            (void)hipGetLastError();
            c->lk.marks = nullptr;
        }
        zr_settle_forget(&c->lk.settle);
    }
    return c->lk.plane != nullptr;
}

int empty_pixel_pass(zr_ctx* c)
{
    c->empty_ready = false;
    const bool fill_slot = c->plan.light_fill && c->lk.rest != nullptr;
    if (c->plan.one_pixel == ZR_LANE_NONE || (!empty_px_on(c) && !fill_slot)) return ZR_OK;
    ZrLightParams L; light_params(c, &L);
    L.W = 1; L.H = 1; L.tiles_x = 1; L.packed_out = 0; L.bg_enabled = 0;
    zr_launch_lighting(L, c->fc[c->fcur].view, c->d_sowned, 1, c->Gclear, shadow_buf(c), c->cube, c->d_lut, c->d_unorm_lut, c->fc[c->fcur].empty_rgba,
                       lane_stream(c, c->plan.one_pixel), fill_slot ? ZR_LIGHT_FILL : ZR_LIGHT_PLAIN, fill_slot ? c->lk.rest : nullptr);
    HIPCHK(c, hipGetLastError());
    c->empty_ready = empty_px_on(c);
    return ZR_OK;
}

static void rest_args(const zr_ctx* c, ZrRestArgs* R)
{
    const XkView& V = c->view;
    memset(R, 0, sizeof *R);
    memcpy(R->cam, V.CameraInfo, sizeof R->cam);
    R->nDir = (uint32_t)V.LightsCount[0]; R->nPoint = (uint32_t)V.LightsCount[1];
    for (uint32_t i = 0; i < R->nPoint && i < ZR_REST_ARG_LIGHTS; ++i) {
        memcpy(R->pt[i].color, V.PointLights[i].Color, sizeof R->pt[i].color);
        memcpy(R->pt[i].pos_falloff, V.PointLights[i].Position, 3 * sizeof(float));
        R->pt[i].pos_falloff[3] = V.PointLights[i].Direction[3];
    }
}

static bool settle_allowed(const zr_ctx* c)
{
    return c->lk.marks != nullptr && !c->lk.settle_off && !c->lk.handed_out && c->d_tiles_ext == nullptr && c->dist == nullptr && c->cfg.tile_world <= 1u;
}
static void settle_key(const zr_ctx* c, const ZrLightParams& L, const ZrRestArgs& R, const uint32_t* out, zr_ctx::SettleKey* K)
{
    memset(K, 0, sizeof *K);
    K->L = L; K->L.clear_next = nullptr; K->L.clear_n = 0;
    memcpy(K->cam, R.cam, sizeof K->cam); K->nDir = R.nDir; K->n_owned = c->n_owned;
    K->out = out; K->plane = c->lk.plane; K->rest = c->lk.rest; K->owned = c->d_owned; K->marks = c->lk.marks;
}

int lighting_pass(zr_ctx* c)
{
    const ZrFramePlan& p = c->plan;
    const hipStream_t s = lane_stream(c, p.lighting);
    ZrLightParams L; light_params(c, &L);
    const FrameCopy& F = c->fc[c->fcur];
    L.empty_rgba = c->empty_ready ? F.empty_rgba : nullptr;
    FrameCopy& next = c->fc[c->smap ^ 1];
    if (c->n_owned && !c->d_shadow_ext && !next.shadow_cleared) { L.clear_next = (uint32_t*)next.shadow; L.clear_n = c->SD * c->SD; next.shadow_cleared = true; }
    uint32_t* const frame_out = L.packed_out ? (c->d_tiles_ext ? c->d_tiles_ext : c->d_tiles) : c->d_color;
    ZrLightMode mode = p.light_keep ? ZR_LIGHT_KEPT : p.light_fill ? ZR_LIGHT_FILL : ZR_LIGHT_PLAIN;
    const bool shortcut_as_planned = p.light_args ? empty_px_on(c) : c->facts.light_empty_px == c->empty_ready;
    bool by_arg = p.light_args && rest_launch_fits(c);
    if (mode != ZR_LIGHT_PLAIN && (c->facts.cube_gen != c->cube_gen || !shortcut_as_planned || !c->lk.plane || c->shading == ZR_SHADING_FORWARD || (p.light_args && !by_arg))) {
        mode = ZR_LIGHT_PLAIN; by_arg = false; zr_history_forgotten(c, ZR_HIST_LIGHT_PLANE);
    }
    if (p.light_args && !by_arg) { if (int rc = zr_frame_uniforms(c, s, false, false)) return rc; }
    bool stood = false;
    if (c->shading == ZR_SHADING_FORWARD) {
        if (L.clear_next) { zr_launch_fill32(L.clear_next, 0x3F800000u, L.clear_n, s); L.clear_next = nullptr; }
        zr_launch_forward(c->pass[1], L, F.view, c->d_objs, c->d_owned, c->n_owned, F.G, shadow_buf(c), c->cube, c->d_lut, c->d_unorm_lut, frame_out, s);
    } else if (by_arg) {
        ZrRestArgs R; rest_args(c, &R);
        if (settle_allowed(c)) {
            zr_ctx::SettleKey K; settle_key(c, L, R, frame_out, &K);
            ZrSettleFacts sf; sf.stand = true; sf.key_same = memcmp(&K, &c->lk.settle_key, sizeof K) == 0;
            const ZrSettleStep step = zr_settle_step(c->lk.settle, sf);
            if (step.wipe) HIPCHK(c, hipMemsetAsync(c->lk.marks, 0, (size_t)c->n_owned * zr_lighting_stand_parts() * sizeof(uint32_t), s));
            zr_launch_lighting_stand(L, R, c->d_owned, c->n_owned, F.G, c->d_lut, c->d_unorm_lut, frame_out, s, c->lk.plane, c->lk.rest, c->lk.marks, step.gen);
            c->lk.settle = step.next; c->lk.settle_key = K; stood = true;
        } else
            zr_launch_lighting_rest(L, R, c->d_owned, c->n_owned, F.G, c->d_lut, c->d_unorm_lut, frame_out, s, c->lk.plane, c->lk.rest);
        c->lk.by_arg++;
    } else {
        zr_launch_lighting(L, F.view, c->d_owned, c->n_owned, F.G, shadow_buf(c), c->cube, c->d_lut, c->d_unorm_lut, frame_out, s, mode, c->lk.plane, c->lk.rest);
        if (c->debug_view == 9u)
            zr_launch_gbuffer_vis(L, F.view, F.G, shadow_buf(c), c->cube, c->d_lut, c->d_color, s);
    }
    if (!stood) c->lk.settle = zr_settle_step(c->lk.settle, ZrSettleFacts{}).next;
    TIMED(c, EV_LIGHTING);
    const bool end_recorded = zr_end_records(c->end, c->frame_no, p.light_args);
    if (end_recorded) HIPCHK(c, hipEventRecord(c->ev_end[c->frame_no % zr_ctx::END_RING], s));
    zr_end_enqueued(&c->end, c->frame_no, p.light_args, end_recorded);
    HIPCHK(c, hipGetLastError());
    if (mode == ZR_LIGHT_FILL) { c->lk.key = c->lk.now; c->carry = zr_frame_carry(c->carry, c->facts, p, ZR_STAGE_LIGHTING); }
    c->lk.last = (uint32_t)mode; c->lk.count[mode]++;
    if (c->timing_now) c->sample_no++;
    c->rendered = true; c->frame_no++; c->stage = 0;
    c->ids_frame = c->ids_this; c->ids.gen = c->scene_gen;
    return ZR_OK;
}

static_assert(ZR_LIGHT_PLANE_IGNORED == (uint32_t)ZR_LIGHT_PLAIN && ZR_LIGHT_PLANE_FILLED == (uint32_t)ZR_LIGHT_FILL && ZR_LIGHT_PLANE_READ == (uint32_t)ZR_LIGHT_KEPT,
              "zelda_render.h: what a lighting pass did with the plane");

extern "C" int zr_get_light_keep(zr_ctx* c, zr_light_keep* out, size_t bytes)
{
    if (!c || !out) return ZR_ERR_ARG;
    return zr_guard(c, [&]() -> int {
        zr_light_keep k;
        memset(&k, 0, sizeof k);
        k.last = c->rendered ? c->lk.last : ZR_LIGHT_PLANE_IGNORED;
        k.ignored = c->lk.count[ZR_LIGHT_PLAIN]; k.filled = c->lk.count[ZR_LIGHT_FILL]; k.read = c->lk.count[ZR_LIGHT_KEPT];
        k.plane_bytes = c->lk.plane ? 32ull * c->W * c->H : 0ull;
        k.read_by_arg = c->lk.by_arg;
        memcpy(out, &k, bytes < sizeof k ? bytes : sizeof k);
        return ZR_OK;
    });
}

static int settled_parts(zr_ctx* c, std::vector<uint8_t>* out)
{
    out->assign((size_t)c->n_owned * zr_lighting_stand_parts(), 0);
    if (!c->lk.marks || !c->lk.settle.standing || c->lk.settle.gen == 0u || out->empty()) return ZR_OK;
    HIPCHK(c, hipSetDevice(c->device));
    int rc = zr_finish(c);
    if (rc) return rc;
    std::vector<uint32_t> m(out->size());
    HIPCHK(c, hipMemcpy(m.data(), c->lk.marks, m.size() * sizeof(uint32_t), hipMemcpyDeviceToHost));
    for (size_t k = 0; k < m.size(); ++k) (*out)[k] = m[k] == c->lk.settle.gen ? 1 : 0;
    return ZR_OK;
}
extern "C" int zr_get_rest_settled(zr_ctx* c, uint32_t* parts, uint32_t* settled)
{
    if (!c || !parts || !settled) return ZR_ERR_ARG;
    return zr_guard(c, [&]() -> int {
        std::vector<uint8_t> st;
        int rc = settled_parts(c, &st);
// ... 19 lines not shown
```

### zeldaengine_amd/csrc/zr_readback.cpp

```cpp
#include "zr_ctx.h"

#include <algorithm>
#include <cstdio>
#include <cstddef>
#include <cstring>
#include <cstdlib>

static void merge_shadow_stats(zr_ctx* c, const ZrDevStats& sh)
{
    ZrDevStats& h = c->h_stats;
    h.survivors[0] = sh.survivors[0]; h.bin_entries[0] = sh.bin_entries[0]; h.n_chunks[0] = sh.n_chunks[0];
    h.n_slow[0] = sh.n_slow[0]; h.n_vis_work[0] = sh.n_vis_work[0];
    h.shadow_occluded = 0; for (uint32_t v : sh.covered_part) h.shadow_occluded += v;
    h.shadow_late = sh.shadow_late;
    h.survivors[0] += h.shadow_occluded + h.shadow_late;
    h.overflow |= sh.overflow;
    if (!h.overflow_sticky) h.overflow_sticky = sh.overflow_sticky;
}

extern "C" int zr_finish(zr_ctx* c)
{
    if (!c) return ZR_ERR_ARG;
    return zr_guard(c, [&]() -> int {
        HIPCHK(c, hipSetDevice(c->device));
// ... 126 lines not shown
            zr_launch_count_shadow((const uint32_t*)shadow_buf(c), (size_t)c->SD * c->SD, c->d_stats, c->stream);
            (void)hipStreamSynchronize(c->stream);
            (void)hipMemcpy(&c->h_stats.covered_shadow, &c->d_stats->covered_shadow, 4, hipMemcpyDeviceToHost);
        }
#ifdef ZR_DIAG
        if (getenv("ZR_DUMP_STATS")) {
            const ZrDevStats& h = c->h_stats;
            fprintf(stderr, "zr stats: survivors %u %u %u  bin_entries %u %u %u  n_sel %u %u %u  n_slow %u %u %u  hiz_culled %u  n_chunks %u %u %u  overflow records %u %u\n",
                    h.survivors[0], h.survivors[1], h.survivors[2], h.bin_entries[0], h.bin_entries[1], h.bin_entries[2], h.n_sel[0], h.n_sel[1], h.n_sel[2],
                    h.n_slow[0], h.n_slow[1], h.n_slow[2], h.hiz_culled, h.n_chunks[0], h.n_chunks[1], h.n_chunks[2], h.pool_used[1], h.pool_used[2]);
        }
#endif
        memset(out, 0, sizeof *out);
        for (int i = 0; i < 2; ++i) {
            out->work_items[i] = c->last_work[i]; out->survivors[i] = c->h_stats.survivors[i]; out->bin_entries[i] = c->h_stats.bin_entries[i];
        }
        out->survivors[1] += c->h_stats.survivors[2]; out->bin_entries[1] += c->h_stats.bin_entries[2];
        out->hiz_culled = c->h_stats.hiz_culled; out->round1_survivors = c->last_two_round ? c->h_stats.survivors[1] : 0;
        out->covered_pixels = 0; for (uint32_t v : c->h_stats.covered_part) out->covered_pixels += v;
        out->covered_shadow_texels = c->h_stats.covered_shadow; out->overflow = c->h_stats.overflow;
        out->shadow_occluded = c->h_stats.shadow_occluded; out->shadow_late = c->h_stats.shadow_late;
        out->hiz_culled_geom = c->h_stats.hiz_culled_geom; out->struct_bytes = (uint32_t)sizeof(zr_stats);
        memcpy(out_user, out, std::min(bytes, sizeof(zr_stats)));
        return rc;
    });
}


extern "C" int zr_read_color(zr_ctx* c, uint8_t* dst, size_t bytes)
{
    if (!c) return ZR_ERR_ARG;
    return zr_guard(c, [&]() -> int {
        ARGCHK(c, dst && bytes == (size_t)c->W * c->H * 4);
        int rc = zr_finish(c);
        if (rc) return rc;
        HIPCHK(c, hipMemcpy(dst, c->d_color, bytes, hipMemcpyDeviceToHost));
        return ZR_OK;
    });
}
extern "C" int zr_read_gbuffer(zr_ctx* c, int target, void* dst, size_t bytes)
{
    if (!c) return ZR_ERR_ARG;
    return zr_guard(c, [&]() -> int {
        const GBufferPtrs& G = c->fc[c->fcur].G;
        const void* src[6] = { G.depth, G.scene_color, G.gA, G.gB, G.gC, G.gD };
        ARGCHK(c, dst && target >= 0 && target < 6);
        ARGCHK(c, bytes == (size_t)c->W * c->H * (target == 5 ? 8 : 4));
        int rc = zr_finish(c);
        if (rc) return rc;
        HIPCHK(c, hipMemcpy(dst, src[target], bytes, hipMemcpyDeviceToHost));
        return ZR_OK;
    });
}
extern "C" int zr_read_shadowmap(zr_ctx* c, float* dst, size_t bytes)
{
    if (!c) return ZR_ERR_ARG;
    return zr_guard(c, [&]() -> int {
        ARGCHK(c, dst && bytes == (size_t)c->SD * c->SD * 4);
        int rc = zr_finish(c);
        if (rc) return rc;
        HIPCHK(c, hipMemcpy(dst, shadow_buf(c), bytes, hipMemcpyDeviceToHost));
        return ZR_OK;
    });
}

extern "C" int zr_copy_frame_async(zr_ctx* c, void* color_dev, void* shadow_dev)
{
    if (!c) return ZR_ERR_ARG;
    return zr_guard(c, [&]() -> int {
        if (!c->rendered || c->stage != 0) return zr_fail(c, ZR_ERR_STATE, "zr_copy_frame_async: no finished frame enqueued");
        HIPCHK(c, hipSetDevice(c->device));
        if (color_dev) HIPCHK(c, hipMemcpyAsync(color_dev, c->d_color, (size_t)c->W * c->H * 4, hipMemcpyDeviceToDevice, c->stream));
        if (shadow_dev) HIPCHK(c, hipMemcpyAsync(shadow_dev, shadow_buf(c), (size_t)c->SD * c->SD * 4, hipMemcpyDeviceToDevice, c->stream));
        return ZR_OK;
    });
}


int ids_prepare(zr_ctx* c)
{
    if (c->ids.table_gen == c->scene_gen && c->ids.draws) return ZR_OK;
    std::vector<uint32_t> slot_base(c->objects.size());
    uint32_t slots = 0;
    for (size_t i = 0; i < c->objects.size(); ++i) { slot_base[i] = slots; slots += c->objects[i].n_inst; }
    std::vector<ZrIdsDraw> tab;
    uint32_t prim = 0;
    for (int pass = 0; pass < 2; ++pass)
        for (size_t i = 0; i < c->objects.size(); ++i) {
            const ZrSceneObject& o = c->objects[i];
            if ((int)o.instanced != pass) continue;
            const uint32_t nt = (uint32_t)(c->meshes[o.mesh].idx.size() / 3);
            tab.push_back({ prim, nt ? nt : 1u, (uint32_t)i, slot_base[i] });
            prim += nt * o.n_inst;
        }
    tab.push_back({ prim, 1u, 0xFFFFFFFFu, slots });
    HIPCHK(c, zr_sync_all(c));
    c->ids.table.release(); c->ids.draws = nullptr;
    HIPCHK(c, upload(c->ids.table, &c->ids.draws, tab));
    c->ids.n_draws = (uint32_t)tab.size() - 1u;
    c->ids.n_slots = slots;
    if (slots > c->ids.slot_cap || !c->ids.counts) {
        ZrOwn& P = c->ids.pool;
        P.release(); c->ids.counts = c->ids.cov = c->ids.list = c->ids.n = nullptr; c->ids.keys = nullptr; c->ids.hits = nullptr;
        c->ids.slot_cap = 0;
        const size_t cap = std::max<uint32_t>(slots, 1u);
        HIPCHK(c, P.alloc(&c->ids.counts, cap)); HIPCHK(c, P.alloc(&c->ids.cov, cap)); HIPCHK(c, P.alloc(&c->ids.list, cap));
// ... 189 lines not shown
```

### zeldaengine_amd/csrc/zr_resize.cpp

```cpp
#include "zr_ctx.h"

#include <cstring>

namespace {

struct ZrExtentState {
    ZrOwn mem, pool_mem;
    uint32_t W = 0, H = 0, tiles_x = 0, tiles_y = 0, n_tiles = 0, n_owned = 0, slots_per_rank = 0;
    GBufferPtrs G[2] = {}; uint32_t* prim_plane[2] = { nullptr, nullptr };
    uint32_t *d_color = nullptr, *d_tiles = nullptr, *d_tile_map = nullptr, *d_owned = nullptr;
    unsigned long long* d_vis[2] = { nullptr, nullptr }; unsigned long long* d_sky_keys = nullptr;
    float* d_hiz = nullptr; ZrHiz hiz = {}; uint32_t* d_hiz_regions = nullptr; uint32_t n_hiz_regions = 0;
    uint32_t *tile_count = nullptr, *tile_offset = nullptr, *tile_cursor = nullptr, *chunk_offset = nullptr;
    bool pools = false; ZrTriBins tb = {}; uint4* chunk_tab = nullptr; uint32_t chunk_capacity = 0;
};

bool extent_ok(uint32_t W, uint32_t H)
{
    if (W == 0 || H == 0 || W > 255u * ZR_TILE || H > 255u * ZR_TILE) return false;
    return ((W + ZR_TILE - 1) / ZR_TILE) * ((H + ZR_TILE - 1) / ZR_TILE) <= 16000u;
}

int make_extent_state(zr_ctx* c, uint32_t W, uint32_t H, ZrExtentState* Ep)
{
    ZrExtentState& E = *Ep;
    ZrOwn& A = E.mem;
    if (!extent_ok(W, H)) return zr_fail(c, ZR_ERR_ARG, "too many tiles");
    E.W = W; E.H = H;
    const size_t n = (size_t)W * H;
    for (int i = 0; i < 2; ++i) {
        GBufferPtrs& G = E.G[i];
        HIPCHK(c, A.alloc(&G.depth, n)); HIPCHK(c, A.alloc(&G.scene_color, n)); HIPCHK(c, A.alloc(&G.gA, n)); HIPCHK(c, A.alloc(&G.gB, n));
        HIPCHK(c, A.alloc(&G.gC, n)); HIPCHK(c, A.alloc(&G.gD, n)); HIPCHK(c, A.alloc(&G.overlay, n));
        if (c->fc[i].G.prim) { HIPCHK(c, A.alloc(&E.prim_plane[i], n)); G.prim = E.prim_plane[i]; }
    }
    HIPCHK(c, A.alloc(&E.d_color, n));
    for (auto& v : E.d_vis) HIPCHK(c, A.alloc(&v, n));
    if (c->d_sky_keys) HIPCHK(c, A.alloc(&E.d_sky_keys, n));

    E.tiles_x = (W + ZR_TILE - 1) / ZR_TILE; E.tiles_y = (H + ZR_TILE - 1) / ZR_TILE; E.n_tiles = E.tiles_x * E.tiles_y;
    const ZrTilePartition tp = zr_partition(E.tiles_x, E.tiles_y, c->cfg.tile_world, c->cfg.tile_rank);
    E.slots_per_rank = tp.slots_per_rank; E.n_owned = (uint32_t)tp.owned.size();
    HIPCHK(c, upload(A, &E.d_tile_map, tp.map)); HIPCHK(c, upload(A, &E.d_owned, tp.owned));
    const size_t tile_words = (size_t)E.slots_per_rank * ZR_TILE * ZR_TILE;
    HIPCHK(c, A.alloc(&E.d_tiles, tile_words));
    const uint32_t mt = (E.n_tiles > c->sn_tiles ? E.n_tiles : c->sn_tiles) * ZR_TSTRIDE + 1;
    HIPCHK(c, A.alloc(&E.tile_count, mt)); HIPCHK(c, A.alloc(&E.tile_offset, mt));
    HIPCHK(c, A.alloc(&E.tile_cursor, mt)); HIPCHK(c, A.alloc(&E.chunk_offset, mt));

    size_t hiz_texels = 0;
    {
        for (int l = 0; l < 4; ++l) { E.hiz.hw[l] = (W + (8u << l) - 1) / (8u << l); E.hiz.hh[l] = (H + (8u << l) - 1) / (8u << l); hiz_texels += (size_t)E.hiz.hw[l] * E.hiz.hh[l]; }
        E.hiz.fw = (W + 3u) / 4u; E.hiz.fh = (H + 3u) / 4u;
        hiz_texels += (size_t)E.hiz.fw * E.hiz.fh;
        HIPCHK(c, A.alloc(&E.d_hiz, hiz_texels));
        static_assert(ZR_TILE == 32 && ZR_SUPERTILE_SHIFT >= 1, "a 64 x 64 region of the pyramid must lie inside one super-tile");
        std::vector<uint32_t> regions;
        for (uint32_t ry = 0; ry < (H + 63u) / 64u; ++ry)
            for (uint32_t rx = 0; rx < (W + 63u) / 64u; ++rx)
                if (zr_tile_owner(rx * 2u, ry * 2u, c->cfg.tile_world) == c->cfg.tile_rank) regions.push_back(rx | ry << 16);
        E.n_hiz_regions = (uint32_t)regions.size();
        HIPCHK(c, upload(A, &E.d_hiz_regions, regions));
        float* p = E.d_hiz;
        for (int l = 0; l < 4; ++l) { E.hiz.lvl[l] = p; p += (size_t)E.hiz.hw[l] * E.hiz.hh[l]; }
        E.hiz.fine = p;
    }
    HIPCHK(c, zr_fill_sync({ { E.G[0].overlay, 0, n * 4 }, { E.G[1].overlay, 0, n * 4 }, { E.d_color, 0, n * 4 },
                             { E.d_tiles, 0, tile_words * 4 },
                             { E.tile_count, 0, (size_t)mt * 4 },
                             { E.tile_cursor, 0, (size_t)mt * 4 },
                             { E.d_hiz, 0, hiz_texels * sizeof(float) } }));
    for (uint32_t* p : E.prim_plane) if (p) HIPCHK(c, zr_fill_sync({ { p, 0xFF, n * 4 } }));
    for (auto& v : E.d_vis) zr_launch_fill64(v, ZR_EMPTY_KEY, n, c->stream);
    HIPCHK(c, hipGetLastError());
    HIPCHK(c, hipStreamSynchronize(c->stream));

    if (c->work_capacity != 0) {
        E.tb = c->tb;
        if (int rc = zr_make_pool_tiles(c, E.pool_mem, E.n_tiles, &E.tb, &E.chunk_tab, &E.chunk_capacity)) return rc;
        E.pools = true;
    }
    return ZR_OK;
}

void commit_extent_state(zr_ctx* c, ZrExtentState& E)
{
    c->W = c->cfg.width = E.W; c->H = c->cfg.height = E.H;
    c->tiles_x = E.tiles_x; c->tiles_y = E.tiles_y; c->n_tiles = E.n_tiles; c->n_owned = E.n_owned; c->slots_per_rank = E.slots_per_rank;
    for (int i = 0; i < 2; ++i) { c->fc[i].G = E.G[i]; c->fc[i].prim_plane = E.prim_plane[i]; c->d_vis[i] = E.d_vis[i]; }
    c->d_color = E.d_color; c->d_tiles = E.d_tiles; c->d_tile_map = E.d_tile_map; c->d_owned = E.d_owned; c->d_sky_keys = E.d_sky_keys;
    c->d_hiz = E.d_hiz; c->hiz = E.hiz; c->d_hiz_regions = E.d_hiz_regions; c->n_hiz_regions = E.n_hiz_regions;
    c->sb.tile_count = E.tile_count; c->sb.tile_offset = E.tile_offset; c->sb.tile_cursor = E.tile_cursor; c->sb.chunk_offset = E.chunk_offset;
    c->lk.plane = nullptr; c->lk.rest = nullptr; c->lk.alloc_failed = false;
    c->lk.marks = nullptr; c->lk.handed_out = false; zr_settle_forget(&c->lk.settle);
    c->d_scaled = nullptr; c->ids.obj = nullptr; c->hl.plane = nullptr; c->hl.frame = nullptr; c->ov.frame = nullptr;
    c->d_tiles_ext = nullptr;
    memset(&c->resolve_P, 0, sizeof c->resolve_P); memset(c->pass, 0, sizeof c->pass); c->pass_live[0] = c->pass_live[1] = false;
    if (E.pools) {
        c->tb = E.tb; c->sb.chunk_tab = E.chunk_tab; c->chunk_capacity = E.chunk_capacity;
        c->pool_tiles = std::move(E.pool_mem);
    }
    c->ext = std::move(E.mem);
}

}

int zr_extent_create(zr_ctx* c)
{
    ZrExtentState E;
    if (int rc = make_extent_state(c, c->W, c->H, &E)) return rc;
    commit_extent_state(c, E);
    return ZR_OK;
}

extern "C" int zr_resize(zr_ctx* c, uint32_t width, uint32_t height)
{
    if (!c) return ZR_ERR_ARG;
    return zr_guard(c, [&]() -> int {
        if (!extent_ok(width, height)) return zr_fail(c, ZR_ERR_ARG, "zr_resize: a zero extent, one beyond 255 tiles a side, or more than 16000 tiles");
        if (int rc = zr_stage_idle(c, "zr_resize")) return rc;
        if (c->dist) return zr_fail(c, ZR_ERR_UNSUPPORTED, "zr_resize: the native multi-GPU host is attached (its buffers are sized at zr_dist_prepare)");
        if (width == c->W && height == c->H) return ZR_OK;
        HIPCHK(c, hipSetDevice(c->device));
        HIPCHK(c, zr_sync_all(c));
        ZrExtentState E;
        ZrDeltaBuffers D;
        int rc = make_extent_state(c, width, height, &E);
        if (rc == ZR_OK && c->delta.on) rc = zr_delta_make(c, width, height, c->delta.b.codec.on, &D);
        if (rc) { (void)hipGetLastError(); return rc; }
        commit_extent_state(c, E);
        if (c->delta.on) { c->delta.b = std::move(D); c->delta.full = true; }
        for (FrameCopy& F : c->fc) { F.g_gen = 0; F.overlay_dirty = false; F.ids_wait = false; }
        zr_history_forgotten(c, ZR_HIST_CAMERA_LIST | ZR_HIST_PLAN | ZR_HIST_VISIBILITY | ZR_HIST_LIGHT_PLANE);
        c->carry.cam_prev_valid = c->carry.r2_settled = c->carry.plan_two_round = c->carry.plan_behind_cam = false;
        memset(&c->cam_prev_key, 0, sizeof c->cam_prev_key); memset(&c->list_key[1], 0, sizeof c->list_key[1]);
        zr_camera_changed(c);
        c->rendered = false; c->ids_frame = false; c->last_two_round = false; c->empty_ready = false;
        c->cov_block = c->d_stats; c->last_work[1] = 0; c->h_stats = ZrDevStats{};
        if (c->lens.valid) zr_uniforms_reproject(c);
        if (E.pools) HIPCHK(c, zr_pool_plan_reset(c));
        return ZR_OK;
    });
// ... 12 lines not shown
```

### zeldaengine_amd/csrc/zr_resolve.hip

```cpp
#include "zr_dev.h"
#include "zr_surface.h"

#ifndef ZR_RESOLVE_IMG_WAVES
#define ZR_RESOLVE_IMG_WAVES 3
#endif
template <int IMAGES, int TB, int PPT>
__global__ __launch_bounds__(TB, TB == 64 ? ZR_RESOLVE_IMG_WAVES : 1) void k_resolve_gbuffer(ZrPass P, const ZrObject* __restrict__ objs,
                                                        const uint32_t* __restrict__ owned_tiles,
                                                        unsigned long long* __restrict__ vis64, GBufferPtrs G,
                                                        const float* __restrict__ srgb_lut, const float* __restrict__ unorm_lut,
                                                        uint8_t* __restrict__ vis_now, ZrDevStats* __restrict__ stats, uint32_t vis_mark)
{
    __shared__ uint32_t covered_s;
    __shared__ float tlut[IMAGES ? 512 : 1];
    constexpr uint32_t T = TILE_PIX / (uint32_t)PPT, PARTS = T / (uint32_t)TB;
    const uint32_t tid = threadIdx.x + (blockIdx.x % PARTS) * (uint32_t)TB;
    if (IMAGES) for (uint32_t i = threadIdx.x; i < 256u; i += (uint32_t)TB) { tlut[i] = srgb_lut[i]; tlut[256u + i] = unorm_lut[i]; }
    const float* __restrict__ dlut = IMAGES ? tlut : srgb_lut;
    const uint32_t tile = owned_tiles[blockIdx.x / PARTS];
    const int tx0 = (int)(tile % P.tiles_x) * TILE, ty0 = (int)(tile / P.tiles_x) * TILE;
    if (threadIdx.x == 0) covered_s = 0;
    __syncthreads();
    uint32_t ncov = 0;
    unsigned long long keys[PPT];
#pragma unroll
    for (uint32_t q = 0; q < (uint32_t)PPT; ++q) {
        const uint32_t i = tid + q * T;
        const int px = tx0 + (int)(i & (TILE - 1)), py = ty0 + (int)(i / TILE);
        keys[q] = ZR_EMPTY_KEY;
        if (px < (int)P.W && py < (int)P.H) {
            const size_t p = (size_t)py * P.W + (size_t)px;
            keys[q] = vis64[p];
            vis64[p] = ZR_EMPTY_KEY;
        }
    }
#pragma unroll
    for (uint32_t q = 0; q < (uint32_t)PPT; ++q) {
        const uint32_t i = tid + q * T;
        const int px = tx0 + (int)(i & (TILE - 1)), py = ty0 + (int)(i / TILE);
        if (px >= (int)P.W || py >= (int)P.H) continue;
        const unsigned long long k = keys[q];
        ncov += resolve_pixel<IMAGES>(P, objs, (uint32_t)k, zr_u2f((uint32_t)(k >> 32)), px, py, G, dlut, vis_now, vis_mark) ? 1u : 0u;
        if (G.prim) G.prim[(size_t)py * P.W + (size_t)px] = (uint32_t)k;
        if (IMAGES != 0 && P.sky_keys != nullptr) {
            const unsigned long long ks = P.sky_keys[(size_t)py * P.W + (size_t)px];
            if ((uint32_t)ks != ZR_EMPTY_PRIM && zr_u2f((uint32_t)(ks >> 32)) < zr_u2f((uint32_t)(k >> 32)))
                resolve_pixel<IMAGES>(P, objs, objs[P.sky_object].prim_base + (uint32_t)ks, zr_u2f((uint32_t)(ks >> 32)), px, py, G, dlut, nullptr);
        }
    }
    if (ncov) atomicAdd(&covered_s, ncov);
    __syncthreads();
    if (threadIdx.x == 0 && covered_s) atomicAdd(&stats->covered_part[blockIdx.x & 31u], covered_s);
}

__global__ __launch_bounds__(256) void k_mark(ZrPass P, const ZrObject* __restrict__ objs, const uint32_t* __restrict__ owned_tiles,
                                              const unsigned long long* __restrict__ vis64, uint8_t* __restrict__ vis_now, uint32_t vis_mark)
{
    const uint32_t i = threadIdx.x + (blockIdx.x % (TILE_PIX / 256u)) * 256u;
    const uint32_t tile = owned_tiles[blockIdx.x / (TILE_PIX / 256u)];
    const int px = (int)(tile % P.tiles_x) * TILE + (int)(i & (TILE - 1)), py = (int)(tile / P.tiles_x) * TILE + (int)(i / TILE);
    uint32_t mi = 0xFFFFFFFFu;
    if (px < (int)P.W && py < (int)P.H) {
        const uint32_t prim = (uint32_t)vis64[(size_t)py * P.W + (size_t)px];
        if (prim != ZR_EMPTY_PRIM) {
            const ZrObject* __restrict__ O = objs + find_object_prim(objs, (int)P.n_objects, prim);
            const uint32_t local = prim - O->prim_base;
            const uint32_t inst_i = local / O->n_tris, tri = local - inst_i * O->n_tris;
            mi = O->work_base + inst_i * O->n_meshlets + ld_global(O->tri_meshlet + tri);
        }
    }
    const uint32_t left = (uint32_t)__builtin_amdgcn_update_dpp((int)0xFFFFFFFEu, (int)mi, 0x111, 0xF, 0xF, false);
    if (mi != 0xFFFFFFFFu && mi != left) vis_now[mi] = (uint8_t)vis_mark;
}


void zr_launch_mark(const ZrPass& P, const ZrObject* objs, const uint32_t* owned_tiles, uint32_t n_owned, const unsigned long long* vis64,
                    uint8_t* vis_now, hipStream_t s, uint32_t vis_mark)
{
    if (n_owned == 0 || vis_now == nullptr) return;
    hipLaunchKernelGGL(k_mark, dim3(n_owned * (TILE_PIX / 256u)), dim3(256), 0, s, P, objs, owned_tiles, vis64, vis_now, vis_mark);
}

void zr_launch_resolve_gbuffer(const ZrPass& P, const ZrObject* objs, const uint32_t* owned_tiles, uint32_t n_owned,
                               unsigned long long* vis64, const GBufferPtrs& G, const float* srgb_lut, const float* unorm_lut, uint8_t* vis_now,
                               ZrDevStats* stats, hipStream_t s, uint32_t vis_mark)
{
    if (n_owned == 0) return;
#define ZR_LAUNCH_RESOLVE(IM, TB, PPT) hipLaunchKernelGGL((k_resolve_gbuffer<IM, TB, PPT>), dim3(n_owned * (TILE_PIX / (PPT) / (TB))), dim3(TB), 0, s, P, objs, owned_tiles, vis64, G, srgb_lut, unorm_lut, vis_now, stats, vis_mark)
    if (P.images == 1u) ZR_LAUNCH_RESOLVE(1, 64, ZR_PIXELS_PER_THREAD);
    else if (P.images) ZR_LAUNCH_RESOLVE(2, 64, ZR_PIXELS_PER_THREAD);
    else ZR_LAUNCH_RESOLVE(0, ZR_RESOLVE_TB, ZR_PIXELS_PER_THREAD);
#undef ZR_LAUNCH_RESOLVE
}
```

### zeldaengine_amd/csrc/zr_surface.h

```cpp
#pragma once
#include "zr_dev.h"
#include "zr_texture.h"

struct Bary { float b0, b1, b2; };
struct FastSetup { int X0, Y0; float a1, b1, a2, b2, rw0, rw1, rw2; };

__device__ __forceinline__ Bary bary_screen(const FastSetup& s, int px, int py)
{
    const float fx = (float)(px * 256 + 128 - s.X0), fy = (float)(py * 256 + 128 - s.Y0);
    const float l1 = __builtin_fmaf(s.b1, fy, s.a1 * fx), l2 = __builtin_fmaf(s.b2, fy, s.a2 * fx);
    const float l0 = (1.0f - l1) - l2;
    const float q0 = l0 * s.rw0, q1 = l1 * s.rw1, q2 = l2 * s.rw2;
    const float inv = 1.0f / ((q0 + q1) + q2);
    Bary r; r.b0 = q0 * inv; r.b1 = q1 * inv; r.b2 = q2 * inv;
    return r;
}
__device__ __forceinline__ Bary bary_homog(const zf4* c, float hw, float hh, int px, int py)
{
    const float u = (((float)px + 0.5f) - hw) / hw, v = (((float)py + 0.5f) - hh) / hh;
    float k[3];
    for (int i = 0; i < 3; ++i) {
        const zf4 p = c[(i + 1) % 3], q = c[(i + 2) % 3];
        const float kx = __builtin_fmaf(p.y, q.w, -(q.y * p.w));
        const float ky = __builtin_fmaf(q.x, p.w, -(p.x * q.w));
// ... 54 lines not shown
    Bary b0;
};
__device__ __forceinline__ PixGeom pixel_geom(const ZrPass& P, const ZrObject* __restrict__ objs, uint32_t prim, int px, int py,
                                              uint8_t* __restrict__ vis_now = nullptr, uint32_t vis_mark = 1u)
{
    PixGeom g;
    const ZrObject* __restrict__ O = objs + find_object_prim(objs, (int)P.n_objects, prim);
    const uint32_t local = prim - O->prim_base;
    const uint32_t inst_i = local / O->n_tris, tri = local - inst_i * O->n_tris;
    const bool instanced = O->instanced != 0;
    const ZrInstance I = ld_record(O->inst + inst_i);
    g.O = O; g.tri = tri; g.inst_i = inst_i;
    if (vis_now) vis_now[O->work_base + inst_i * O->n_meshlets + ld_global(O->tri_meshlet + tri)] = (uint8_t)vis_mark;
    zf4 clip[3]; zf3 WP[3], WN[3]; float U[3], V[3]; uint32_t fl[3];
    for (int k = 0; k < 3; ++k) {
        const float4* __restrict__ rv = (const float4*)(O->rtris + 3u * tri + (uint32_t)k);
        const float4 q0 = ld_global(rv), q1 = ld_global(rv + 1);
        const zf3 pos = vs_position(zr3(q0.x, q0.y, q0.z), I, instanced);
        clip[k] = zr_mat4_point(P.PVM, pos);
        WP[k] = model_point(P, pos);
        const zf3 mn = model_point(P, zr3(q1.x, q1.y, q1.z));
        WN[k] = instanced ? zr_rowvec_mat3(mn, I.R) : mn;
        U[k] = q0.w; V[k] = q1.w;
        fl[k] = vertex_flags(clip[k]);
    }
    const int cls = classify(fl[0], fl[1], fl[2]);
    const int qx = px ^ 1, qy = py ^ 1;
    Bary b0, bh, bv;
    if (cls == 1) {
        const SV s0 = project(clip[0], P.hw, P.hh), s1 = project(clip[1], P.hw, P.hh), s2 = project(clip[2], P.hw, P.hh);
        const long long A = (long long)(s1.X - s0.X) * (s2.Y - s0.Y) - (long long)(s2.X - s0.X) * (s1.Y - s0.Y);
        const float invA = 1.0f / (float)A;
        FastSetup fs;
        fs.X0 = s0.X; fs.Y0 = s0.Y;
        fs.a1 = (float)(s2.Y - s0.Y) * invA; fs.b1 = (float)(s0.X - s2.X) * invA;
        fs.a2 = (float)(s0.Y - s1.Y) * invA; fs.b2 = (float)(s1.X - s0.X) * invA;
        fs.rw0 = s0.rw; fs.rw1 = s1.rw; fs.rw2 = s2.rw;
        b0 = bary_screen(fs, px, py); bh = bary_screen(fs, qx, py); bv = bary_screen(fs, px, qy);
    } else {
        b0 = bary_homog(clip, P.hw, P.hh, px, py); bh = bary_homog(clip, P.hw, P.hh, qx, py); bv = bary_homog(clip, P.hw, P.hh, px, qy);
    }
    const zf3 P0 = interp3(b0, WP[0], WP[1], WP[2]), Ph = interp3(bh, WP[0], WP[1], WP[2]), Pv = interp3(bv, WP[0], WP[1], WP[2]);
    g.P0 = P0; g.b0 = b0;
    g.N0 = interp3(b0, WN[0], WN[1], WN[2]);
    const float u0 = interp1(b0, U[0], U[1], U[2]), uh = interp1(bh, U[0], U[1], U[2]), uv_ = interp1(bv, U[0], U[1], U[2]);
    const float v0 = interp1(b0, V[0], V[1], V[2]), vh = interp1(bh, V[0], V[1], V[2]), vv = interp1(bv, V[0], V[1], V[2]);
    const float sx = (px & 1) ? 1.0f : -1.0f, sy = (py & 1) ? 1.0f : -1.0f;
    g.pos_dx = (P0 - Ph) * sx; g.pos_dy = (P0 - Pv) * sy;
    g.u0 = u0; g.v0 = v0;
    g.s1 = (u0 - uh) * sx; g.t1 = (v0 - vh) * sx; g.s2 = (u0 - uv_) * sy; g.t2 = (v0 - vv) * sy;
    return g;
}

template <int IMAGES>
__device__ __forceinline__ bool resolve_pixel(const ZrPass& P, const ZrObject* __restrict__ objs, uint32_t prim, float depth,
                                              int px, int py, const GBufferPtrs& G, const float* __restrict__ lut,
                                              uint8_t* __restrict__ vis_now, uint32_t vis_mark = 1u)
{
    const size_t p = (size_t)py * P.W + (size_t)px;
    if (prim == ZR_EMPTY_PRIM) {
        G.depth[p] = 1.0f; G.scene_color[p] = 0xFF000000u; G.gA[p] = 0u; G.gB[p] = 0xFF000000u; G.gC[p] = 0xFF000000u;
        G.gD[p] = make_uint2(0u, 0x3C000000u);
        if (P.write_overlay) G.overlay[p] = 0u;
        return false;
    }
    const PixGeom g = pixel_geom(P, objs, prim, px, py, vis_now, vis_mark);
    const ZrObject* __restrict__ O = g.O;
    const zf3 P0 = g.P0, N0 = g.N0, pos_dx = g.pos_dx, pos_dy = g.pos_dy;
    const float u0 = g.u0, v0 = g.v0, s1 = g.s1, t1 = g.t1, s2 = g.s2, t2 = g.t2;

    if (O->flags & ZR_OBJ_SKY) {
        const zf4 sk = tex_sample<IMAGES>(O->tex[0], O->texc[0], true, lut, u0, v0, s1, t1, s2, t2);
        G.overlay[p] = pack_rgb8(gamma3(zr3(sk.x, sk.y, sk.z)));
        return false;
    }
    if (P.write_overlay) G.overlay[p] = 0u;
    uint32_t w_sc, w_gB, w_gC;
    zf3 ts;
    if (!IMAGES) {
        w_sc = O->c_scene_color; w_gB = O->c_gB; w_gC = O->c_gC;
        ts = zr3(O->ts_const[0], O->ts_const[1], O->ts_const[2]);
    } else {
        zf4 tb, tme, tro, tno, tao, tem, tms;
        if (IMAGES == 1) {
            tb.x = O->texc[0][0]; tb.y = O->texc[0][1]; tb.z = O->texc[0][2]; tme.x = O->texc[1][0]; tro.x = O->texc[2][0];
            tno.x = O->texc[3][0]; tno.y = O->texc[3][1]; tno.z = O->texc[3][2]; tao.x = O->texc[4][0];
            tem.x = O->texc[5][0]; tem.y = O->texc[5][1]; tem.z = O->texc[5][2]; tms.x = O->texc[6][0];
            if (O->packed.data != nullptr) {
                float pk[ZR_PK_CHANNELS];
                tex_sample_packed(O->packed, lut, u0, v0, s1, t1, s2, t2, pk);
                const uint32_t cs = O->const_slots;
                if (!(cs & 1u)) { tb.x = pk[ZR_PK_BC]; tb.y = pk[ZR_PK_BC + 1]; tb.z = pk[ZR_PK_BC + 2]; }
                if (!(cs & 2u)) tme.x = pk[ZR_PK_ME];
                if (!(cs & 4u)) tro.x = pk[ZR_PK_RO];
                if (!(cs & 8u)) { tno.x = pk[ZR_PK_NO]; tno.y = pk[ZR_PK_NO + 1]; tno.z = pk[ZR_PK_NO + 2]; }
                if (!(cs & 16u)) tao.x = pk[ZR_PK_AO];
                if (!(cs & 32u)) { tem.x = pk[ZR_PK_EM]; tem.y = pk[ZR_PK_EM + 1]; tem.z = pk[ZR_PK_EM + 2]; }
                if (!(cs & 64u)) tms.x = pk[ZR_PK_MS];
            }
        } else {
            zf4 ms[ZR_MATERIAL_SLOTS];
            tex_sample_material(O, lut, u0, v0, s1, t1, s2, t2, ms);
            tb = ms[0]; tme = ms[1]; tro = ms[2]; tno = ms[3]; tao = ms[4]; tem = ms[5]; tms = ms[6];
        }
        const float Rough = __builtin_fmaxf(0.01f, tro.x);
        w_sc = zr_unorm(tem.x, 255.0f) | zr_unorm(tem.y, 255.0f) << 8 | zr_unorm(tem.z, 255.0f) << 16 | zr_unorm(tms.x, 255.0f) << 24;
        w_gB = zr_unorm(tme.x, 255.0f) | zr_unorm(1.0f, 255.0f) << 8 | zr_unorm(Rough, 255.0f) << 16 | 255u << 24;
        w_gC = zr_unorm(tb.x, 255.0f) | zr_unorm(tb.y, 255.0f) << 8 | zr_unorm(tb.z, 255.0f) << 16 | zr_unorm(tao.x, 255.0f) << 24;
        ts = (O->const_slots & 8u) ? zr3(O->ts_const[0], O->ts_const[1], O->ts_const[2]) : zr_tangent_space_normal(zr3(tno.x, tno.y, tno.z));
    }
    const zf3 Nw = compute_normal(pos_dx, pos_dy, s1, t1, s2, t2, N0, ts);
    const zf3 Nn = zr_normalize(Nw);
    const zf3 NP = zr3((Nn.x + 1.0f) / 2.0f, (Nn.y + 1.0f) / 2.0f, (Nn.z + 1.0f) / 2.0f);
    G.depth[p] = depth;
    G.scene_color[p] = w_sc;
    G.gA[p] = zr_unorm(NP.z, 1023.0f) | zr_unorm(NP.y, 1023.0f) << 10 | zr_unorm(NP.x, 1023.0f) << 20 | 3u << 30;
    G.gB[p] = w_gB;
    G.gC[p] = w_gC;
    G.gD[p] = make_uint2(f32_to_f16_hw(P0.x) | f32_to_f16_hw(P0.y) << 16, f32_to_f16_hw(P0.z) | 0x3C000000u);
    return true;
}
```

### zeldaengine_amd/csrc/zr_types.h

```cpp
#pragma once

#include <stdint.h>
#include <hip/hip_runtime.h>
#include "../../include/zelda_abi.h"
#include "../../include/zelda_render.h"

#define ZR_EMPTY_PRIM 0xFFFFFFFFu
#define ZR_EMPTY_KEY ((unsigned long long)0x3F800000u << 32 | ZR_EMPTY_PRIM)
#define ZR_GUARD 4.0f
#define ZR_RECT_CULLED 0xFFFFFFFFu
#ifndef ZR_CHUNK
#define ZR_CHUNK 64u
#endif

enum { ZR_MODE_GBUFFER = 0, ZR_MODE_SHADOW = 1 };
#define ZR_OBJ_SKY 1u
#define ZR_OBJ_HIDDEN 2u

struct ZrInstance {
    float R[9];
    float t[3];
    float s;
    float _pad[3];
};
// ... 204 lines not shown
    uint32_t* tile_cap;
    uint32_t* cursor;
    uint32_t  n_rec, bucket_max;
    uint32_t* plan;
    uint32_t* over_tile;
    uint32_t* over_cursor;
    uint4*    unit_tab;
    uint32_t  unit_cap; uint32_t* n_units;
    uint32_t  n_tiles;
    uint32_t  n_waves;
    uint32_t* wave_culled;
    uint32_t* r2_count;
    uint32_t* r2_stats;
    uint4*    slow; uint32_t slow_cap;
};
#define ZR_R2_WORDS 8u
enum { ZR_PLAN_ONE_ROUND = 0, ZR_PLAN_DREW_ROUND2 = 1, ZR_PLAN_KEPT_ROUND2 = 2 };
#define ZR_OVER_SECTIONS 64u
#ifndef ZR_TSTRIDE
#define ZR_TSTRIDE 4u
#endif
#ifdef ZR_TCHUNK_AB
#define ZR_TCHUNK ZR_TCHUNK_AB
#else
#define ZR_TCHUNK 512u
#endif
#ifndef ZR_TBATCHES
#define ZR_TBATCHES 4u
#endif
void zr_launch_select(const ZrPass& P, const ZrObject* objs, const uint32_t* work, const uint32_t* rects, const ZrHiz& Z, const ZrTriBins& B, ZrDevStats* stats,
                      int slot, hipStream_t s);
void zr_launch_geom(const ZrPass& P, const ZrHiz& Z, const ZrTriBins& B, ZrDevStats* stats, int slot, bool count_only, hipStream_t s);
void zr_launch_plan(const ZrTriBins& B, const uint32_t* owned_tiles, uint32_t n_owned, ZrDevStats* stats, bool exact, uint32_t bucket_pct, hipStream_t s,
                    uint32_t round2 = ZR_PLAN_ONE_ROUND);
void zr_launch_tile(const ZrPass& P, const ZrTriBins& B, ZrDevStats* stats, int slot, unsigned long long* vis64, uint32_t n_blocks, hipStream_t s, bool last,
                    const uint32_t* owned_tiles, uint32_t n_owned);
void zr_launch_cull_box(const ZrPass& P, const ZrObject* objs, uint32_t* work, uint32_t* rects, const ZrHiz& Z, ZrDevStats* stats,
                        int slot, hipStream_t s, ZrBinEntry* sel = nullptr, const uint8_t* vis_prev = nullptr, bool reuse_list = false);
void zr_launch_bin_fill(const ZrPass& P, const ZrObject* objs, const uint32_t* work, const uint32_t* rects, const uint32_t* tile_offset,
                        uint32_t* tile_cursor, ZrBinEntry* bins, const ZrHiz& Z, ZrDevStats* stats, hipStream_t s);
void zr_launch_frame_begin(ZrDevStats* stats, const XkView* view_src_pinned, XkView* view_dst, uint32_t rebuild_lists, hipStream_t s);
void zr_launch_fill32(uint32_t* p, uint32_t v, size_t n, hipStream_t s);
void zr_launch_fill64(unsigned long long* p, unsigned long long v, size_t n, hipStream_t s);
void zr_launch_shadow_occlusion(const ZrPass& P, const ZrObject* objs, const uint32_t* work, const uint32_t* rects, const uint2* pxrect,
                                const float* zmin, uint8_t* flags, const uint32_t* shadow_bits, ZrBinEntry* bins, ZrDevStats* stats,
                                uint32_t n_blocks, uint32_t retest, hipStream_t s);
void zr_launch_raster_chunks(const ZrPass& P, const ZrObject* objs, const uint4* chunk_tab, const ZrBinEntry* bins, ZrDevStats* stats,
                             uint32_t* shadow_bits, uint32_t n_blocks, hipStream_t s, uint4* slow, uint32_t slow_cap, const uint32_t* tiles,
                             uint32_t n_tiles, int stage);
void zr_launch_mark(const ZrPass& P, const ZrObject* objs, const uint32_t* owned_tiles, uint32_t n_owned, const unsigned long long* vis64,
                    uint8_t* vis_now, hipStream_t s, uint32_t vis_mark);
void zr_launch_resolve_gbuffer(const ZrPass& P, const ZrObject* objs, const uint32_t* owned_tiles, uint32_t n_owned,
                               unsigned long long* vis64, const GBufferPtrs& G, const float* srgb_lut, const float* unorm_lut, uint8_t* vis_now,
                               ZrDevStats* stats, hipStream_t s, uint32_t vis_mark = 1u);
void zr_launch_sky_tiles(const ZrPass& P, const ZrObject* objs, const uint32_t* owned_tiles, uint32_t n_owned, unsigned long long* sky64, hipStream_t s);
void zr_launch_count_shadow(const uint32_t* bits, size_t n, ZrDevStats* stats, hipStream_t s);
enum ZrLightMode : uint32_t { ZR_LIGHT_PLAIN = 0u, ZR_LIGHT_FILL = 1u, ZR_LIGHT_KEPT = 2u };
#define ZR_REST_ARG_LIGHTS 64
struct ZrRestLight { float color[4]; float pos_falloff[4]; };
struct ZrRestArgs { float cam[3]; uint32_t nDir, nPoint, _pad[3]; ZrRestLight pt[ZR_REST_ARG_LIGHTS]; };
struct ZrRestRecord { float lo[3], hi[3]; uint32_t empty[2]; };
#define ZR_REST_SLOT 2u
#define ZR_REST_RECORDS_PER_TILE 16u
static_assert(sizeof(ZrRestRecord) == 32 && sizeof(ZrRestLight) == 32 && sizeof(ZrRestArgs) == 32 + 32 * ZR_REST_ARG_LIGHTS, "zr_types.h: the resting frame's records");
void zr_launch_lighting(const ZrLightParams& L, const XkView* view, const uint32_t* owned_tiles, uint32_t n_owned,
                        const GBufferPtrs& G, const float* shadowmap, const CubeDesc& C, const float* lut, const float* unorm_lut,
                        uint32_t* out, hipStream_t s, ZrLightMode mode = ZR_LIGHT_PLAIN, float4* plane = nullptr, float4* rest = nullptr);
bool zr_lighting_rest_available();
void zr_launch_lighting_rest(const ZrLightParams& L, const ZrRestArgs& R, const uint32_t* owned_tiles, uint32_t n_owned, const GBufferPtrs& G,
                             const float* lut, const float* unorm_lut, uint32_t* out, hipStream_t s, const float4* plane, const float4* rest);
uint32_t zr_lighting_stand_parts();
void zr_launch_lighting_stand(const ZrLightParams& L, const ZrRestArgs& R, const uint32_t* owned_tiles, uint32_t n_owned, const GBufferPtrs& G,
                              const float* lut, const float* unorm_lut, uint32_t* out, hipStream_t s, const float4* plane, const float4* rest,
                              uint32_t* marks, uint32_t gen);
void zr_launch_forward(const ZrPass& P, const ZrLightParams& L, const XkView* view, const ZrObject* objs, const uint32_t* owned_tiles, uint32_t n_owned,
                       const GBufferPtrs& G, const float* shadowmap, const CubeDesc& C, const float* lut, const float* unorm_lut, uint32_t* out, hipStream_t s);
void zr_launch_gbuffer_vis(const ZrLightParams& L, const XkView* view, const GBufferPtrs& G, const float* shadowmap, const CubeDesc& C,
                           const float* lut, uint32_t* out, hipStream_t s);
void zr_launch_untile(const uint32_t* gathered, const uint32_t* tile_map, uint32_t* frame, uint32_t W, uint32_t H, uint32_t tiles_x,
                      uint32_t n_tiles, hipStream_t s);
void zr_launch_pack_tiles(const uint32_t* plane, const uint32_t* tiles, uint32_t n_tiles, uint32_t* packed, uint32_t W, uint32_t H, uint32_t tiles_x,
                          uint32_t pad, hipStream_t s);
void zr_launch_frame_delta(const uint32_t* frame, uint32_t* delivered, uint8_t* flags, uint32_t* header, uint32_t* list, void* packed,
                           uint32_t W, uint32_t H, uint32_t tiles_x, uint32_t n_tiles, uint32_t full, uint32_t serial, hipStream_t s);
void zr_launch_frame_delta_packed(const uint32_t* frame, uint32_t* delivered, uint8_t* flags, uint16_t* lens, uint32_t* header, uint32_t* list, uint32_t* offsets,
                                  void* stream, uint32_t W, uint32_t H, uint32_t tiles_x, uint32_t n_tiles, uint32_t full, uint32_t serial, hipStream_t s);
void zr_launch_frame_scale(const uint32_t* frame, uint32_t* dst, uint32_t W, uint32_t H, uint32_t s, hipStream_t st);
```

### zeldaengine_amd/engine.py

```python
import ctypes as C
import os

import numpy as np

from . import abi

_HERE = os.path.dirname(os.path.abspath(__file__))
LIB_PATH = os.environ.get("ZELDA_RENDER_LIB") or os.path.join(_HERE, "libzelda_render.so")

_lib = None


class ZeldaRenderError(RuntimeError):
    def __init__(self, code, msg):
        super().__init__("zelda_render error %d: %s" % (code, msg))
        self.code = code


def lib():
    global _lib
    if _lib is not None:
        return _lib
    if not os.path.exists(LIB_PATH):
        raise ImportError("libzelda_render.so is not built: run `python -m zeldaengine_amd.build` "
                          "(hipcc --offload-arch=gfx950); there is no fallback path")
    try:
        import torch
    except ImportError:
        pass
    L = C.CDLL(LIB_PATH)
    vp, u32, sz = C.c_void_p, C.c_uint32, C.c_size_t
    sig = {
        "zr_create": [C.POINTER(abi.Config), C.POINTER(vp)],
        "zr_set_stream": [vp, vp],
        "zr_mesh_create": [vp, vp, u32, vp, u32, C.POINTER(u32)],
        "zr_mesh_set_meshlets": [vp, u32, vp, u32, vp, sz, vp, sz],
        "zr_mesh_build_meshlets": [vp, u32, u32, u32, C.c_float],
        "zr_mesh_get_meshlets": [vp, u32, vp, C.POINTER(u32), vp, C.POINTER(sz), vp, C.POINTER(sz)],
        "zr_meshlets_build": [vp, u32, vp, u32, u32, u32, C.c_float, vp, C.POINTER(u32), vp, C.POINTER(sz), vp, C.POINTER(sz), vp],
        "zr_object_add": [vp, u32, vp, vp, u32],
        "zr_scene_clear": [vp],
        "zr_set_limits": [vp, u32, u32],
        "zr_set_bucket_share": [vp, u32],
        "zr_object_count": [vp, C.POINTER(u32)],
        "zr_object_get_instances": [vp, u32, C.POINTER(u32), vp, C.POINTER(u32)],
        "zr_object_set_instances": [vp, u32, u32, vp, u32],
        "zr_object_update_instances_async": [vp, u32, u32, vp, vp, u32, vp],
        "zr_mesh_set_vertices": [vp, u32, u32, vp, u32],
        "zr_mesh_update_vertices_async": [vp, u32, u32, vp, u32, vp],
        "zr_mesh_get_vertices": [vp, u32, vp, C.POINTER(u32)],
        **abi.TEXTURE_UPDATE_SIGNATURES,
        **abi.VISIBILITY_SIGNATURES,
        **abi.FRAME_DELTA_SIGNATURES,
        **abi.FRAME_SCALE_SIGNATURES,
        **abi.HIGHLIGHT_SIGNATURES,
        **abi.OVERLAY_SIGNATURES,
        **abi.EXTENT_SIGNATURES,
        **abi.REST_SETTLE_SIGNATURES,
        "zr_set_cubemap": [vp, vp, u32],
        "zr_set_skydome": [vp, vp, u32, vp, u32, vp],
        "zr_set_background": [vp, vp],
        "zr_set_sky_flags": [vp, C.c_int, C.c_int],
        "zr_update_uniforms": [vp, vp, vp, u32, vp, u32, vp, u32, C.c_float, C.c_float, C.c_float],
        "zr_set_frame": [vp, vp, vp, vp],
        "zr_get_frame": [vp, vp, vp, vp],
        "zr_set_debug_view": [vp, u32],
        "zr_set_shading": [vp, u32],
        "zr_render": [vp],
        "zr_render_shadow": [vp], "zr_render_gbuffer": [vp], "zr_render_lighting": [vp],
        "zr_render_geometry": [vp], "zr_stream_wait_shadow": [vp, vp],
        "zr_set_shadow_partition": [vp, u32, u32], "zr_set_shadow_buffer": [vp, vp],
        "zr_set_shadow_tiles": [vp, u32, u32], "zr_shadow_tiles_bytes": [vp, C.POINTER(sz)],
        "zr_shadow_pack": [vp, vp, vp], "zr_shadow_unpack": [vp, vp, vp],
        "zr_finish": [vp],
        "zr_get_pass_times": [vp, vp],
        "zr_get_pass_times_avg": [vp, u32, vp],
        "zr_set_timing_interval": [vp, u32],
        "zr_get_frame_latencies": [vp, u32, vp],
        "zr_get_frame_periods": [vp, u32, vp],
        "zr_get_stats": [vp, C.POINTER(abi.Stats), sz],
        "zr_get_light_keep": [vp, C.POINTER(abi.LightKeep), sz],
        "zr_read_color": [vp, vp, sz],
        "zr_read_gbuffer": [vp, C.c_int, vp, sz],
        "zr_read_shadowmap": [vp, vp, sz],
        "zr_copy_frame_async": [vp, vp, vp],
        "zr_set_id_capture": [vp, C.c_int],
        "zr_read_ids": [vp, C.c_int, vp, sz],
        "zr_pick": [vp, u32, u32, u32, u32, vp, u32, C.POINTER(u32)],
        "zr_instance_coverage": [vp, vp, sz],
        "zr_instance_coverage_async": [vp, vp, sz],
        "zr_tiles_device_buffer": [vp, C.POINTER(vp), C.POINTER(sz)],
        "zr_composite": [vp, vp],
        "zr_read_tiles": [vp, vp, sz],
        "zr_set_tiles_buffer": [vp, vp],
        "zr_tile_size": [],
        "zr_color_device_ptr": [vp, C.POINTER(vp)],
        "zr_tile_partition": [u32, u32, u32, u32, vp, C.POINTER(u32), C.POINTER(u32)],
        "zr_dist_unique_id": [vp, sz],
        "zr_dist_init": [vp, vp, sz, u32, u32, u32],
        "zr_dist_prepare": [vp, u32, u32, u32],
        "zr_dist_connect": [vp, vp, sz],
        "zr_dist_frame": [vp],
        "zr_dist_copy_frame_async": [vp, vp],
        "zr_profab_register": [vp, C.c_char_p, u32, vp],
        "zr_world_load_json": [vp, C.c_char_p, sz],
        "zr_set_asset_root": [vp, C.c_char_p],
        "zr_asset_path_search": [vp, C.c_char_p, vp, sz, C.POINTER(sz)],
        "zr_load_obj": [C.c_char_p, vp, C.POINTER(u32), vp, C.POINTER(u32)],
        "zr_load_png_rgba8": [C.c_char_p, vp, sz, C.POINTER(u32), C.POINTER(u32)],
        "zr_load_meshlet_file": [vp, C.c_char_p, C.POINTER(u32)],
        "zr_world_load_file": [vp, C.c_char_p],
# ... 486 lines not shown

    def set_shadow_buffer(self, dev_ptr):
        self._chk(self.L.zr_set_shadow_buffer(self.h, C.c_void_p(dev_ptr) if dev_ptr else None))

    def finish(self):
        self._chk(self.L.zr_finish(self.h))

    def set_timing_interval(self, interval):
        self._chk(self.L.zr_set_timing_interval(self.h, interval))

    def pass_times(self, last_n=1):
        ms = (C.c_float * len(abi.PASS_NAMES))()
        self._chk(self.L.zr_get_pass_times_avg(self.h, last_n, ms))
        return dict(zip(abi.PASS_NAMES, [float(x) for x in ms]))

    def frame_latencies(self, n=64):
        ms = (C.c_float * n)()
        got = self.L.zr_get_frame_latencies(self.h, n, ms)
        if got < 0:
            self._chk(got)
        return [float(ms[i]) for i in range(got)]

    def frame_periods(self, n=511):
        ms = (C.c_float * n)()
        got = self.L.zr_get_frame_periods(self.h, n, ms)
        if got < 0:
            self._chk(got)
        return [float(ms[i]) for i in range(got)]

    def stats(self):
        s = abi.Stats()
        self._chk(self.L.zr_get_stats(self.h, C.byref(s), C.sizeof(s)))
        return {"work_items": list(s.work_items), "survivors": list(s.survivors), "bin_entries": list(s.bin_entries),
                "covered_pixels": int(s.covered_pixels), "covered_shadow_texels": int(s.covered_shadow_texels), "overflow": int(s.overflow),
                "hiz_culled": int(s.hiz_culled), "hiz_culled_geom": int(s.hiz_culled_geom), "round1_survivors": int(s.round1_survivors),
                "shadow_occluded": int(s.shadow_occluded), "shadow_late": int(s.shadow_late)}

    def light_keep(self):
        k = abi.LightKeep()
        self._chk(self.L.zr_get_light_keep(self.h, C.byref(k), C.sizeof(k)))
        return {"last": ("ignored", "filled", "read")[int(k.last)], "ignored": int(k.ignored), "filled": int(k.filled), "read": int(k.read),
                "plane_bytes": int(k.plane_bytes), "read_by_arg": int(k.read_by_arg)}

    def rest_settled(self):
        parts, settled = C.c_uint32(), C.c_uint32()
        self._chk(self.L.zr_get_rest_settled(self.h, C.byref(parts), C.byref(settled)))
        return int(parts.value), int(settled.value)

    def rest_settled_parts(self):
        out = np.zeros(self.rest_settled()[0], dtype=np.uint8)
        self._chk(self.L.zr_get_rest_settled_parts(self.h, _ptr(out) if out.size else None, out.nbytes))
        return out

    def color(self):
        out = np.zeros((self.H, self.W, 4), dtype=np.uint8)
        self._chk(self.L.zr_read_color(self.h, _ptr(out), out.nbytes))
        return out

    def gbuffer(self, target):
        out = np.zeros((self.H, self.W), dtype=abi.GBUFFER_DTYPES[target])
        self._chk(self.L.zr_read_gbuffer(self.h, target, _ptr(out), out.nbytes))
        return out

    def shadowmap(self):
        out = np.zeros((self.SD, self.SD), dtype=np.float32)
        self._chk(self.L.zr_read_shadowmap(self.h, _ptr(out), out.nbytes))
        return out

    def copy_frame_async(self, color_dev=None, shadow_dev=None):
        self._chk(self.L.zr_copy_frame_async(self.h, C.c_void_p(color_dev) if color_dev else None, C.c_void_p(shadow_dev) if shadow_dev else None))

    def set_frame_delta(self, on=True):
        self._chk(self.L.zr_set_frame_delta(self.h, int(on)))

    def frame_delta_reset(self):
        self._chk(self.L.zr_frame_delta_reset(self.h))

    def frame_delta_tiles(self):
        return self.frame_delta_extent()[2]

    def set_frame_delta_scale(self, s):
        self._chk(self.L.zr_set_frame_delta_scale(self.h, s))

    def frame_delta_extent(self):
        w, h, t, s = C.c_uint32(), C.c_uint32(), C.c_uint32(), C.c_uint32()
        self._chk(self.L.zr_get_frame_delta_extent(self.h, C.byref(w), C.byref(h), C.byref(t), C.byref(s)))
        return w.value, h.value, t.value, s.value

    def _scaled_shape(self, s):
        s = max(s, 1)
        return -(-self.H // s), -(-self.W // s), 4

    def color_scaled(self, s):
        out = np.zeros(self._scaled_shape(s), dtype=np.uint8)
        self._chk(self.L.zr_read_color_scaled(self.h, s, _ptr(out), out.nbytes))
        return out

    def copy_frame_scaled_async(self, s, color_dev):
        self._chk(self.L.zr_copy_frame_scaled_async(self.h, s, C.c_void_p(color_dev) if color_dev else None))

    def highlight_set(self, obj, on=True, first=0):
        on = np.ascontiguousarray(np.atleast_1d(np.asarray(on)) != 0, dtype=np.uint8)
        self._chk(self.L.zr_highlight_set(self.h, obj, first, _ptr(on), on.size))

    def highlight_clear(self):
        self._chk(self.L.zr_highlight_clear(self.h))
# ... 244 lines not shown
```

Baseline: 114,800.

## Emit per-wave bbox/empty records in G-buffer resolve and consume them in lighting

The G-buffer resolve pass now also writes per-wave tile records (position bounding box plus an empty-pixel mask). The plain lighting kernel reads these records instead of rescanning the G-buffer to build its light-culling box. It also skips loading G-buffer words for pixels marked empty. This removes a full G-buffer read pass inside lighting and the loads for background pixels, in exchange for extra record writes during resolve and a new kernel variant.

```diff
diff --git a/include/zelda_render.h b/include/zelda_render.h
--- a/include/zelda_render.h
+++ b/include/zelda_render.h
@@ -166,6 +166,8 @@
 int  zr_get_light_keep(zr_ctx* ctx, zr_light_keep* out, size_t bytes);
 int  zr_get_rest_settled(zr_ctx* ctx, uint32_t* parts, uint32_t* settled);
 int  zr_get_rest_settled_parts(zr_ctx* ctx, uint8_t* standing, size_t bytes);
+typedef struct zr_gbuffer_record { float lo[3], hi[3]; uint32_t empty[2]; } zr_gbuffer_record;
+int  zr_get_gbuffer_records(zr_ctx* ctx, int copy, zr_gbuffer_record* out, size_t bytes);
 
 int  zr_read_color(zr_ctx* ctx, uint8_t* rgba8, size_t bytes);
 int  zr_read_gbuffer(zr_ctx* ctx, int target, void* dst, size_t bytes);
diff --git a/zeldaengine_amd/abi.py b/zeldaengine_amd/abi.py
--- a/zeldaengine_amd/abi.py
+++ b/zeldaengine_amd/abi.py
@@ -114,6 +114,11 @@
     "zr_get_rest_settled": [C.c_void_p, C.POINTER(C.c_uint32), C.POINTER(C.c_uint32)],
     "zr_get_rest_settled_parts": [C.c_void_p, C.c_void_p, C.c_size_t],
 }
+GBUFFER_RECORD_DTYPE = [("lo", "<f4", (3,)), ("hi", "<f4", (3,)), ("empty", "<u4", (2,))]
+GBUFFER_RECORDS_PER_TILE = 16
+GBUFFER_RECORD_SIGNATURES = {
+    "zr_get_gbuffer_records": [C.c_void_p, C.c_int, C.c_void_p, C.c_size_t],
+}
 EXTENT_SIGNATURES = {
     "zr_resize": [vp_, u32_, u32_],
     "zr_get_extent": [vp_, C.POINTER(u32_), C.POINTER(u32_)],
diff --git a/zeldaengine_amd/csrc/zr_context.cpp b/zeldaengine_amd/csrc/zr_context.cpp
--- a/zeldaengine_amd/csrc/zr_context.cpp
+++ b/zeldaengine_amd/csrc/zr_context.cpp
@@ -106,6 +106,11 @@
         uint32_t* w = (uint32_t*)c->d_clear_px;
         c->Gclear.depth = (float*)w; c->Gclear.scene_color = w + 1; c->Gclear.gA = w + 2; c->Gclear.gB = w + 3; c->Gclear.gC = w + 4;
         c->Gclear.gD = (uint2*)(w + 6); c->Gclear.overlay = w + 8;
+        ZrRestRecord rec[ZR_REST_RECORDS_PER_TILE];
+        for (ZrRestRecord& r : rec) r = ZrRestRecord{ { INFINITY, INFINITY, INFINITY }, { -INFINITY, -INFINITY, -INFINITY }, { 0u, 0u } };
+        rec[0] = ZrRestRecord{ { 0.0f, 0.0f, 0.0f }, { 0.0f, 0.0f, 0.0f }, { 1u, 0u } };
+        HIPCHK(c, A.alloc(&c->d_clear_records, ZR_REST_RECORDS_PER_TILE));
+        HIPCHK(c, hipMemcpy(c->d_clear_records, rec, sizeof rec, hipMemcpyHostToDevice));
     }
     {
 #ifdef ZR_DIAG
diff --git a/zeldaengine_amd/csrc/zr_ctx.h b/zeldaengine_amd/csrc/zr_ctx.h
--- a/zeldaengine_amd/csrc/zr_ctx.h
+++ b/zeldaengine_amd/csrc/zr_ctx.h
@@ -135,6 +135,7 @@
     bool shadow_cleared = false;
     uint64_t view_uploaded = 0;
     uint64_t g_gen = 0;
+    ZrRestRecord* records = nullptr; bool records_valid = false;
     hipEvent_t ev_ids = nullptr; bool ids_wait = false;
 };
 
@@ -202,6 +203,7 @@
     uint32_t chunk_capacity = 0;
     uint32_t n_inst_total = 0;
     uint8_t* d_clear_px = nullptr; GBufferPtrs Gclear = {}; bool empty_ready = false;
+    ZrRestRecord* d_clear_records = nullptr;
     uint32_t env_skip = 0, env_skip_light = 0; int32_t env_light_list_min = 4; bool env_no_empty_px = false;
     static constexpr int VIEW_RING = kZrViewRing;
     XkView* h_view_ring = nullptr; hipEvent_t view_ev[VIEW_RING] = {}; uint32_t view_slot = 0; bool view_dirty = true;
diff --git a/zeldaengine_amd/csrc/zr_dev.h b/zeldaengine_amd/csrc/zr_dev.h
--- a/zeldaengine_amd/csrc/zr_dev.h
+++ b/zeldaengine_amd/csrc/zr_dev.h
@@ -311,6 +311,12 @@
 #ifndef ZR_REST_RECORDS_ONE_TRIP
 #define ZR_REST_RECORDS_ONE_TRIP 1
 #endif
+#ifndef ZR_LIGHT_BOX_FROM_RECORDS
+#define ZR_LIGHT_BOX_FROM_RECORDS 1
+#endif
+#ifndef ZR_LIGHT_SKIP_EMPTY_LOADS
+#define ZR_LIGHT_SKIP_EMPTY_LOADS 1
+#endif
 #ifndef ZR_PIXELS_PER_THREAD
 #define ZR_PIXELS_PER_THREAD 1
 #endif
diff --git a/zeldaengine_amd/csrc/zr_frame_host.cpp b/zeldaengine_amd/csrc/zr_frame_host.cpp
--- a/zeldaengine_amd/csrc/zr_frame_host.cpp
+++ b/zeldaengine_amd/csrc/zr_frame_host.cpp
@@ -412,8 +412,9 @@
         TIMED(c, EV_MARK);
         c->resolve_P = P; c->resolve_mark = vis_mark;
     } else {
-        zr_launch_resolve_gbuffer(P, c->d_objs, c->d_owned, c->n_owned, c->d_vis[c->fcur], c->fc[c->fcur].G, c->d_lut, c->d_unorm_lut, Z.vis_now, c->d_stats, s, vis_mark);
-        c->cov_block = c->d_stats; c->fc[c->fcur].g_gen = p.g_gen;
+        zr_launch_resolve_gbuffer(P, c->d_objs, c->d_owned, c->n_owned, c->d_vis[c->fcur], c->fc[c->fcur].G, c->d_lut, c->d_unorm_lut, Z.vis_now, c->d_stats, s, vis_mark,
+                                  c->fc[c->fcur].records);
+        c->cov_block = c->d_stats; c->fc[c->fcur].g_gen = p.g_gen; c->fc[c->fcur].records_valid = zr_lighting_rest_available() && c->fc[c->fcur].records != nullptr;
         TIMED(c, EV_RESOLVE);
     }
     if (p.ev_cam == ZR_EVCAM_BEHIND_MARK || p.ev_cam == ZR_EVCAM_BEHIND_RESOLVE) HIPCHK(c, hipEventRecord(c->ev_cam, s));
@@ -481,9 +482,10 @@
     ZrDevStats* const tally = c->d_rstats[c->fcur];
     zr_launch_fill32(tally->covered_part, 0u, 32, s);
     TIMED(c, EV_HOST_RESOLVE);
-    zr_launch_resolve_gbuffer(c->resolve_P, c->d_objs, c->d_owned, c->n_owned, c->d_vis[c->fcur], c->fc[c->fcur].G, c->d_lut, c->d_unorm_lut, nullptr, tally, s, c->resolve_mark);
+    zr_launch_resolve_gbuffer(c->resolve_P, c->d_objs, c->d_owned, c->n_owned, c->d_vis[c->fcur], c->fc[c->fcur].G, c->d_lut, c->d_unorm_lut, nullptr, tally, s, c->resolve_mark,
+                              c->fc[c->fcur].records);
     TIMED(c, EV_RESOLVE);
-    c->cov_block = tally; c->fc[c->fcur].g_gen = c->plan.g_gen;
+    c->cov_block = tally; c->fc[c->fcur].g_gen = c->plan.g_gen; c->fc[c->fcur].records_valid = zr_lighting_rest_available() && c->fc[c->fcur].records != nullptr;
     HIPCHK(c, hipGetLastError());
     return ZR_OK;
 }
diff --git a/zeldaengine_amd/csrc/zr_lighting.hip b/zeldaengine_amd/csrc/zr_lighting.hip
--- a/zeldaengine_amd/csrc/zr_lighting.hip
+++ b/zeldaengine_amd/csrc/zr_lighting.hip
@@ -1,11 +1,7 @@
 #include "zr_dev.h"
 #include "zr_surface.h"
 #include "zr_shade.h"
-
-__device__ __forceinline__ bool light_pixel_empty(uint32_t sc, uint32_t A, uint32_t B, uint32_t Cc, uint2 D)
-{
-    return sc == 0xFF000000u && A == 0u && B == 0xFF000000u && Cc == 0xFF000000u && D.x == 0u && D.y == 0x3C000000u;
-}
+#include "zr_rest_record.h"
 
 struct LitPixel { zf3 BaseColor, Normal, N, Pw; float Metallic, Roughness, AO, Mask; };
 __device__ __forceinline__ LitPixel light_decode(const float* u8, const float* u10, uint32_t sc, uint32_t A, uint32_t B, uint32_t Cc, uint2 D)
@@ -55,6 +51,7 @@
     for (uint32_t i = threadIdx.x; i < per && b + i < L.clear_n; i += (uint32_t)TB) L.clear_next[b + i] = 0x3F800000u;
 }
 
+constexpr uint32_t ZR_LIGHT_PLAIN_RECORDS = 3u;
 template <bool LIGHT_LIST, bool BACKGROUND, int TB, int PPT, uint32_t MODE>
 __global__ __launch_bounds__(TB) __attribute__((amdgpu_waves_per_eu(MODE == ZR_LIGHT_KEPT ? ZR_LIGHT_KEPT_WAVES : ZR_LIGHT_WAVES, MODE == ZR_LIGHT_KEPT ? ZR_LIGHT_KEPT_WAVES : ZR_LIGHT_WAVES))) void k_lighting(ZrLightParams L, const XkView* __restrict__ view,
                                                   const uint32_t* __restrict__ owned_tiles, GBufferPtrs G,
@@ -66,55 +63,60 @@
     __shared__ float u10[1024];
     float* const slut = tl; float* const u8 = tl + 256;
     constexpr uint32_t T = TILE_PIX / (uint32_t)PPT, PARTS = T / (uint32_t)TB, WAVES = (uint32_t)TB / 64u;
+    constexpr bool FROM_RECORDS = MODE == ZR_LIGHT_PLAIN_RECORDS;
+    static_assert(!FROM_RECORDS || (PPT == 1 && WAVES <= 8u), "k_lighting: a part's records are a dword per lane of a kernel with one pixel per thread");
+    const ZrRestRecord* __restrict__ const records = FROM_RECORDS ? (const ZrRestRecord*)rest : nullptr;
+    constexpr bool BOX_RECORDS = FROM_RECORDS && LIGHT_LIST && ZR_LIGHT_BOX_FROM_RECORDS != 0;
+    constexpr bool SKIP_LOADS = FROM_RECORDS && ZR_LIGHT_SKIP_EMPTY_LOADS != 0;
     const uint32_t tid = threadIdx.x + (blockIdx.x % PARTS) * (uint32_t)TB;
     const uint32_t tile_slot = blockIdx.x / PARTS;
+    __shared__ float bbp[LIGHT_LIST && !BOX_RECORDS ? WAVES : 1][6];
+    __shared__ uint32_t lmask[LIGHT_LIST ? XK_MAX_POINT_LIGHTS_NUM / 32 : 1];
+    constexpr bool use_mask = LIGHT_LIST;
+    uint32_t rec = 0u;
+    if constexpr (BOX_RECORDS || SKIP_LOADS) rec = rest_records_fetch_at<WAVES>(records, tile_slot * ZR_REST_RECORDS_PER_TILE + (blockIdx.x % PARTS) * WAVES);
+    uint32_t tile_ahead = 0u;
+    if constexpr (FROM_RECORDS) tile_ahead = owned_tiles[tile_slot];
     for (uint32_t i = threadIdx.x; i < 256u; i += (uint32_t)TB) { u8[i] = unorm_lut[i]; slut[i] = srgb_lut[i]; }
     for (uint32_t i = threadIdx.x; i < 1024u; i += (uint32_t)TB) u10[i] = unorm_lut[256u + i];
+    if constexpr (BOX_RECORDS)
+        for (uint32_t i = threadIdx.x; i < XK_MAX_POINT_LIGHTS_NUM / 32; i += (uint32_t)TB) lmask[i] = 0u;
     __syncthreads();
     light_clear_next_slice<TB>(L);
-    const uint32_t tile = owned_tiles[tile_slot];
+    const uint32_t tile = FROM_RECORDS ? tile_ahead : owned_tiles[tile_slot];
     const int tx0 = (int)(tile % L.tiles_x) * TILE, ty0 = (int)(tile / L.tiles_x) * TILE;
     const zf3 cam = zr3(view->CameraInfo[0], view->CameraInfo[1], view->CameraInfo[2]);
     const uint32_t nDir = (uint32_t)view->LightsCount[0], nPoint = (uint32_t)view->LightsCount[1];
     const float maxmips = (float)(uint32_t)view->LightsCount[3];
     const float dxy = 1.5f * 1.0f / (float)L.SD;
 
-    __shared__ float bbp[LIGHT_LIST ? WAVES : 1][6];
-    __shared__ uint32_t lmask[LIGHT_LIST ? XK_MAX_POINT_LIGHTS_NUM / 32 : 1];
-    constexpr bool use_mask = LIGHT_LIST;
     constexpr bool RECORDS = MODE == ZR_LIGHT_FILL && PPT == 1;
-    if constexpr (LIGHT_LIST || RECORDS) {
-        float lo[3] = { __builtin_inff(), __builtin_inff(), __builtin_inff() }, hi[3] = { -__builtin_inff(), -__builtin_inff(), -__builtin_inff() };
-        bool odd = false;
+    if constexpr (BOX_RECORDS) {
+        float blo[3], bhi[3];
+        rest_records_box(rec, blo, bhi);
+        for (uint32_t li = threadIdx.x; li < nPoint; li += (uint32_t)TB)
+            if (light_listed(ViewLight{ &view->PointLights[li] }, blo, bhi)) atomicOr(&lmask[li >> 5], 1u << (li & 31u));
+        __syncthreads();
+    } else if constexpr (LIGHT_LIST || RECORDS) {
+        RestBox box = rest_box_none();
         bool empty = false;
         for (uint32_t i = tid; i < TILE_PIX; i += T) {
             const int px = tx0 + (int)(i & (TILE - 1)), py = ty0 + (int)(i / TILE);
             if (px >= (int)L.W || py >= (int)L.H) continue;
             const size_t p = (size_t)py * L.W + (size_t)px;
             if constexpr (RECORDS) empty = light_pixel_empty(G.scene_color[p], G.gA[p], G.gB[p], G.gC[p], G.gD[p]);
-            if ((G.scene_color[p] >> 24) == 0u) continue;
-            const uint2 D = G.gD[p];
-            const float q[3] = { f16_to_f32_hw(D.x & 0xFFFFu), f16_to_f32_hw(D.x >> 16), f16_to_f32_hw(D.y & 0xFFFFu) };
-            for (int a = 0; a < 3; ++a) {
-                if (!(__builtin_fabsf(q[a]) <= 3.402823466e38f)) odd = true;
-                lo[a] = __builtin_fminf(lo[a], q[a]); hi[a] = __builtin_fmaxf(hi[a], q[a]);
-            }
-        }
-        for (int a = 0; a < 3; ++a) { lo[a] = wave_fmin(lo[a]); hi[a] = wave_fmax(hi[a]); }
-        const bool wodd = __ballot(odd) != 0ull;
+            if (!rest_box_counts(G.scene_color[p])) continue;
+            rest_box_count(box, G.gD[p]);
+        }
+        rest_box_wave(box);
         if constexpr (RECORDS) {
-            const unsigned long long em = __ballot(empty);
-            if (rest != nullptr && (threadIdx.x & 63u) == 0u) {
-                ZrRestRecord* r = (ZrRestRecord*)(rest + ZR_REST_SLOT) + ((size_t)tile_slot * ZR_REST_RECORDS_PER_TILE + (tid >> 6));
-                for (int a = 0; a < 3; ++a) { r->lo[a] = wodd ? -__builtin_inff() : lo[a]; r->hi[a] = wodd ? __builtin_inff() : hi[a]; }
-                r->empty[0] = (uint32_t)em; r->empty[1] = (uint32_t)(em >> 32);
-            }
+            if (rest != nullptr) rest_record_write((ZrRestRecord*)(rest + ZR_REST_SLOT) + ((size_t)tile_slot * ZR_REST_RECORDS_PER_TILE + (tid >> 6)), box, empty);
         }
         if constexpr (LIGHT_LIST) {
             if ((threadIdx.x & 63u) == 0u) {
                 float* o = bbp[threadIdx.x >> 6];
-                o[0] = wodd ? -__builtin_inff() : lo[0]; o[1] = wodd ? -__builtin_inff() : lo[1]; o[2] = wodd ? -__builtin_inff() : lo[2];
-                o[3] = wodd ? __builtin_inff() : hi[0]; o[4] = wodd ? __builtin_inff() : hi[1]; o[5] = wodd ? __builtin_inff() : hi[2];
+                o[0] = rest_box_lo(box, 0); o[1] = rest_box_lo(box, 1); o[2] = rest_box_lo(box, 2);
+                o[3] = rest_box_hi(box, 0); o[4] = rest_box_hi(box, 1); o[5] = rest_box_hi(box, 2);
             }
             for (uint32_t i = threadIdx.x; i < XK_MAX_POINT_LIGHTS_NUM / 32; i += (uint32_t)TB) lmask[i] = 0u;
             __syncthreads();
@@ -128,14 +130,22 @@
             __syncthreads();
         }
     }
+    unsigned long long mine = 0ull;
+    if constexpr (SKIP_LOADS) mine = rest_records_empty(rec, (uint32_t)__builtin_amdgcn_readfirstlane((int)(threadIdx.x >> 6)));
 
     for (uint32_t i = tid; i < TILE_PIX; i += T) {
         const int px = tx0 + (int)(i & (TILE - 1)), py = ty0 + (int)(i / TILE);
         if (px >= (int)L.W || py >= (int)L.H) continue;
         const size_t p = (size_t)py * L.W + (size_t)px;
+        if constexpr (SKIP_LOADS) {
+            if (L.empty_rgba != nullptr && ((mine >> (threadIdx.x & 63u)) & 1ull) != 0ull) {
+                light_emit<BACKGROUND>(L, G, tl, out, *L.empty_rgba, px, py, p, tile_slot, i);
+                continue;
+            }
+        }
         const uint32_t sc = G.scene_color[p], A = G.gA[p], B = G.gB[p], Cc = G.gC[p];
         const uint2 D = G.gD[p];
-        if (L.empty_rgba != nullptr && sc == 0xFF000000u && A == 0u && B == 0xFF000000u && Cc == 0xFF000000u && D.x == 0u && D.y == 0x3C000000u) {
+        if (!SKIP_LOADS && L.empty_rgba != nullptr && sc == 0xFF000000u && A == 0u && B == 0xFF000000u && Cc == 0xFF000000u && D.x == 0u && D.y == 0x3C000000u) {
             light_emit<BACKGROUND>(L, G, tl, out, *L.empty_rgba, px, py, p, tile_slot, i);
             continue;
         }
@@ -160,14 +170,6 @@
 }
 
 #if ZR_PIXELS_PER_THREAD == 1
-template <uint32_t WAVES>
-__device__ __forceinline__ uint32_t rest_records_fetch(const float4* __restrict__ rest, uint32_t first_record)
-{
-    constexpr uint32_t RECW = (uint32_t)(sizeof(ZrRestRecord) / 4u);
-    const uint32_t* __restrict__ w = (const uint32_t*)(rest + ZR_REST_SLOT) + (size_t)first_record * RECW;
-    return w[((threadIdx.x & 7u) % WAVES) * RECW + ((threadIdx.x >> 3) & 7u)];
-}
-
 template <bool LIGHT_LIST, bool BACKGROUND, int TB>
 __global__ __launch_bounds__(TB) __attribute__((amdgpu_waves_per_eu(ZR_LIGHT_KEPT_WAVES, ZR_LIGHT_KEPT_WAVES)))
 void k_lighting_rest(ZrLightParams L, ZrRestArgs R, const uint32_t* __restrict__ owned_tiles, GBufferPtrs G, const float* __restrict__ srgb_lut,
@@ -466,18 +468,28 @@
 
 void zr_launch_lighting(const ZrLightParams& L, const XkView* view, const uint32_t* owned_tiles, uint32_t n_owned,
                         const GBufferPtrs& G, const float* shadowmap, const CubeDesc& C, const float* lut, const float* unorm_lut,
-                        uint32_t* out, hipStream_t s, ZrLightMode mode, float4* plane, float4* rest)
+                        uint32_t* out, hipStream_t s, ZrLightMode mode, float4* plane, float4* rest, const ZrRestRecord* records)
 {
     if (n_owned == 0) return;
     if (!plane) mode = ZR_LIGHT_PLAIN;
     if (mode != ZR_LIGHT_FILL) rest = nullptr;
+    constexpr bool pieces = ZR_PIXELS_PER_THREAD == 1 && (ZR_LIGHT_BOX_FROM_RECORDS != 0 || ZR_LIGHT_SKIP_EMPTY_LOADS != 0);
+    const bool from_records = pieces && mode == ZR_LIGHT_PLAIN && records != nullptr;
+    if (from_records) rest = (float4*)records;
 #define ZR_LAUNCH_LIGHTING_TB(LL, BG, TB, MODE) hipLaunchKernelGGL((k_lighting<LL, BG, TB, ZR_PIXELS_PER_THREAD, MODE>), dim3(n_owned * (TILE_PIX / ZR_PIXELS_PER_THREAD / TB)), dim3(TB), 0, s, L, view, owned_tiles, G, shadowmap, C, lut, unorm_lut, out, plane, rest)
+#if ZR_PIXELS_PER_THREAD == 1
+#define ZR_LAUNCH_LIGHTING_PLAIN(LL, BG) do { if (from_records) ZR_LAUNCH_LIGHTING_TB(LL, BG, ZR_LIGHT_TB, ZR_LIGHT_PLAIN_RECORDS); \
+                                              else ZR_LAUNCH_LIGHTING_TB(LL, BG, ZR_LIGHT_TB, ZR_LIGHT_PLAIN); } while (0)
+#else
+#define ZR_LAUNCH_LIGHTING_PLAIN(LL, BG) ZR_LAUNCH_LIGHTING_TB(LL, BG, ZR_LIGHT_TB, ZR_LIGHT_PLAIN)
+#endif
 #define ZR_LAUNCH_LIGHTING(LL, BG) do { if (mode == ZR_LIGHT_KEPT) ZR_LAUNCH_LIGHTING_TB(LL, BG, ZR_LIGHT_KEPT_TB, ZR_LIGHT_KEPT); \
                                         else if (mode == ZR_LIGHT_FILL) ZR_LAUNCH_LIGHTING_TB(LL, BG, ZR_LIGHT_TB, ZR_LIGHT_FILL); \
-                                        else ZR_LAUNCH_LIGHTING_TB(LL, BG, ZR_LIGHT_TB, ZR_LIGHT_PLAIN); } while (0)
+                                        else ZR_LAUNCH_LIGHTING_PLAIN(LL, BG); } while (0)
     if (L.light_list) { if (L.bg_enabled) ZR_LAUNCH_LIGHTING(true, true); else ZR_LAUNCH_LIGHTING(true, false); }
     else { if (L.bg_enabled) ZR_LAUNCH_LIGHTING(false, true); else ZR_LAUNCH_LIGHTING(false, false); }
 #undef ZR_LAUNCH_LIGHTING
+#undef ZR_LAUNCH_LIGHTING_PLAIN
 #undef ZR_LAUNCH_LIGHTING_TB
 }
 bool zr_lighting_rest_available() { return ZR_PIXELS_PER_THREAD == 1; }
diff --git a/zeldaengine_amd/csrc/zr_lighting_host.cpp b/zeldaengine_amd/csrc/zr_lighting_host.cpp
--- a/zeldaengine_amd/csrc/zr_lighting_host.cpp
+++ b/zeldaengine_amd/csrc/zr_lighting_host.cpp
@@ -79,7 +79,7 @@
     ZrLightParams L; light_params(c, &L);
     L.W = 1; L.H = 1; L.tiles_x = 1; L.packed_out = 0; L.bg_enabled = 0;
     zr_launch_lighting(L, c->fc[c->fcur].view, c->d_sowned, 1, c->Gclear, shadow_buf(c), c->cube, c->d_lut, c->d_unorm_lut, c->fc[c->fcur].empty_rgba,
-                       lane_stream(c, c->plan.one_pixel), fill_slot ? ZR_LIGHT_FILL : ZR_LIGHT_PLAIN, fill_slot ? c->lk.rest : nullptr);
+                       lane_stream(c, c->plan.one_pixel), fill_slot ? ZR_LIGHT_FILL : ZR_LIGHT_PLAIN, fill_slot ? c->lk.rest : nullptr, nullptr, c->d_clear_records);
     HIPCHK(c, hipGetLastError());
     c->empty_ready = empty_px_on(c);
     return ZR_OK;
@@ -144,7 +144,8 @@
             zr_launch_lighting_rest(L, R, c->d_owned, c->n_owned, F.G, c->d_lut, c->d_unorm_lut, frame_out, s, c->lk.plane, c->lk.rest);
         c->lk.by_arg++;
     } else {
-        zr_launch_lighting(L, F.view, c->d_owned, c->n_owned, F.G, shadow_buf(c), c->cube, c->d_lut, c->d_unorm_lut, frame_out, s, mode, c->lk.plane, c->lk.rest);
+        zr_launch_lighting(L, F.view, c->d_owned, c->n_owned, F.G, shadow_buf(c), c->cube, c->d_lut, c->d_unorm_lut, frame_out, s, mode, c->lk.plane, c->lk.rest,
+                           F.records_valid ? F.records : nullptr);
         if (c->debug_view == 9u)
             zr_launch_gbuffer_vis(L, F.view, F.G, shadow_buf(c), c->cube, c->d_lut, c->d_color, s);
     }
diff --git a/zeldaengine_amd/csrc/zr_readback.cpp b/zeldaengine_amd/csrc/zr_readback.cpp
--- a/zeldaengine_amd/csrc/zr_readback.cpp
+++ b/zeldaengine_amd/csrc/zr_readback.cpp
@@ -202,6 +202,22 @@
         return ZR_OK;
     });
 }
+extern "C" int zr_get_gbuffer_records(zr_ctx* c, int copy, zr_gbuffer_record* out, size_t bytes)
+{
+    if (!c) return ZR_ERR_ARG;
+    return zr_guard(c, [&]() -> int {
+        static_assert(sizeof(zr_gbuffer_record) == sizeof(ZrRestRecord), "zelda_render.h: zr_gbuffer_record is ZrRestRecord");
+        ARGCHK(c, copy >= -1 && copy <= 1);
+        ARGCHK(c, (out || bytes == 0) && bytes == (size_t)c->n_owned * ZR_REST_RECORDS_PER_TILE * sizeof(ZrRestRecord));
+        const FrameCopy& F = c->fc[copy < 0 ? c->fcur : copy];
+        if (!F.records_valid) return zr_fail(c, ZR_ERR_STATE, "zr_get_gbuffer_records: no resolve has written this copy's records (no frame drawn since zr_create or zr_resize)");
+        HIPCHK(c, hipSetDevice(c->device));
+        int rc = zr_finish(c);
+        if (rc) return rc;
+        if (bytes) HIPCHK(c, hipMemcpy(out, F.records, bytes, hipMemcpyDeviceToHost));
+        return ZR_OK;
+    });
+}
 extern "C" int zr_read_shadowmap(zr_ctx* c, float* dst, size_t bytes)
 {
     if (!c) return ZR_ERR_ARG;
diff --git a/zeldaengine_amd/csrc/zr_resize.cpp b/zeldaengine_amd/csrc/zr_resize.cpp
--- a/zeldaengine_amd/csrc/zr_resize.cpp
+++ b/zeldaengine_amd/csrc/zr_resize.cpp
@@ -7,7 +7,7 @@
 struct ZrExtentState {
     ZrOwn mem, pool_mem;
     uint32_t W = 0, H = 0, tiles_x = 0, tiles_y = 0, n_tiles = 0, n_owned = 0, slots_per_rank = 0;
-    GBufferPtrs G[2] = {}; uint32_t* prim_plane[2] = { nullptr, nullptr };
+    GBufferPtrs G[2] = {}; uint32_t* prim_plane[2] = { nullptr, nullptr }; ZrRestRecord* records[2] = { nullptr, nullptr };
     uint32_t *d_color = nullptr, *d_tiles = nullptr, *d_tile_map = nullptr, *d_owned = nullptr;
     unsigned long long* d_vis[2] = { nullptr, nullptr }; unsigned long long* d_sky_keys = nullptr;
     float* d_hiz = nullptr; ZrHiz hiz = {}; uint32_t* d_hiz_regions = nullptr; uint32_t n_hiz_regions = 0;
@@ -42,6 +42,7 @@
     const ZrTilePartition tp = zr_partition(E.tiles_x, E.tiles_y, c->cfg.tile_world, c->cfg.tile_rank);
     E.slots_per_rank = tp.slots_per_rank; E.n_owned = (uint32_t)tp.owned.size();
     HIPCHK(c, upload(A, &E.d_tile_map, tp.map)); HIPCHK(c, upload(A, &E.d_owned, tp.owned));
+    for (auto& r : E.records) HIPCHK(c, A.alloc(&r, (size_t)E.n_owned * ZR_REST_RECORDS_PER_TILE));
     const size_t tile_words = (size_t)E.slots_per_rank * ZR_TILE * ZR_TILE;
     HIPCHK(c, A.alloc(&E.d_tiles, tile_words));
     const uint32_t mt = (E.n_tiles > c->sn_tiles ? E.n_tiles : c->sn_tiles) * ZR_TSTRIDE + 1;
@@ -88,6 +89,7 @@
     c->W = c->cfg.width = E.W; c->H = c->cfg.height = E.H;
     c->tiles_x = E.tiles_x; c->tiles_y = E.tiles_y; c->n_tiles = E.n_tiles; c->n_owned = E.n_owned; c->slots_per_rank = E.slots_per_rank;
     for (int i = 0; i < 2; ++i) { c->fc[i].G = E.G[i]; c->fc[i].prim_plane = E.prim_plane[i]; c->d_vis[i] = E.d_vis[i]; }
+    for (int i = 0; i < 2; ++i) { c->fc[i].records = E.records[i]; c->fc[i].records_valid = false; }
     c->d_color = E.d_color; c->d_tiles = E.d_tiles; c->d_tile_map = E.d_tile_map; c->d_owned = E.d_owned; c->d_sky_keys = E.d_sky_keys;
     c->d_hiz = E.d_hiz; c->hiz = E.hiz; c->d_hiz_regions = E.d_hiz_regions; c->n_hiz_regions = E.n_hiz_regions;
     c->sb.tile_count = E.tile_count; c->sb.tile_offset = E.tile_offset; c->sb.tile_cursor = E.tile_cursor; c->sb.chunk_offset = E.chunk_offset;
diff --git a/zeldaengine_amd/csrc/zr_resolve.hip b/zeldaengine_amd/csrc/zr_resolve.hip
--- a/zeldaengine_amd/csrc/zr_resolve.hip
+++ b/zeldaengine_amd/csrc/zr_resolve.hip
@@ -1,5 +1,6 @@
 #include "zr_dev.h"
 #include "zr_surface.h"
+#include "zr_rest_record.h"
 
 #ifndef ZR_RESOLVE_IMG_WAVES
 #define ZR_RESOLVE_IMG_WAVES 3
@@ -9,7 +10,8 @@
                                                         const uint32_t* __restrict__ owned_tiles,
                                                         unsigned long long* __restrict__ vis64, GBufferPtrs G,
                                                         const float* __restrict__ srgb_lut, const float* __restrict__ unorm_lut,
-                                                        uint8_t* __restrict__ vis_now, ZrDevStats* __restrict__ stats, uint32_t vis_mark)
+                                                        uint8_t* __restrict__ vis_now, ZrDevStats* __restrict__ stats, uint32_t vis_mark,
+                                                        ZrRestRecord* __restrict__ records)
 {
     __shared__ uint32_t covered_s;
     __shared__ float tlut[IMAGES ? 512 : 1];
@@ -23,6 +25,7 @@
     __syncthreads();
     uint32_t ncov = 0;
     unsigned long long keys[PPT];
+    GBufferWords words = {}; bool inside = false;
 #pragma unroll
     for (uint32_t q = 0; q < (uint32_t)PPT; ++q) {
         const uint32_t i = tid + q * T;
@@ -40,12 +43,22 @@
         const int px = tx0 + (int)(i & (TILE - 1)), py = ty0 + (int)(i / TILE);
         if (px >= (int)P.W || py >= (int)P.H) continue;
         const unsigned long long k = keys[q];
-        ncov += resolve_pixel<IMAGES>(P, objs, (uint32_t)k, zr_u2f((uint32_t)(k >> 32)), px, py, G, dlut, vis_now, vis_mark) ? 1u : 0u;
+        inside = true;
+        ncov += resolve_pixel<IMAGES>(P, objs, (uint32_t)k, zr_u2f((uint32_t)(k >> 32)), px, py, G, dlut, vis_now, vis_mark, PPT == 1 ? &words : nullptr) ? 1u : 0u;
         if (G.prim) G.prim[(size_t)py * P.W + (size_t)px] = (uint32_t)k;
         if (IMAGES != 0 && P.sky_keys != nullptr) {
             const unsigned long long ks = P.sky_keys[(size_t)py * P.W + (size_t)px];
             if ((uint32_t)ks != ZR_EMPTY_PRIM && zr_u2f((uint32_t)(ks >> 32)) < zr_u2f((uint32_t)(k >> 32)))
                 resolve_pixel<IMAGES>(P, objs, objs[P.sky_object].prim_base + (uint32_t)ks, zr_u2f((uint32_t)(ks >> 32)), px, py, G, dlut, nullptr);
+        }
+    }
+    if constexpr (PPT == 1) {
+        if (records != nullptr) {
+            RestBox box = rest_box_none();
+            if (inside && rest_box_counts(words.sc)) rest_box_count(box, words.D);
+            rest_box_wave(box);
+            rest_record_write(records + ((size_t)(blockIdx.x / PARTS) * ZR_REST_RECORDS_PER_TILE + (tid >> 6)), box,
+                              inside && light_pixel_empty(words.sc, words.A, words.B, words.Cc, words.D));
         }
     }
     if (ncov) atomicAdd(&covered_s, ncov);
@@ -83,10 +96,10 @@
 
 void zr_launch_resolve_gbuffer(const ZrPass& P, const ZrObject* objs, const uint32_t* owned_tiles, uint32_t n_owned,
                                unsigned long long* vis64, const GBufferPtrs& G, const float* srgb_lut, const float* unorm_lut, uint8_t* vis_now,
-                               ZrDevStats* stats, hipStream_t s, uint32_t vis_mark)
+                               ZrDevStats* stats, hipStream_t s, uint32_t vis_mark, ZrRestRecord* records)
 {
     if (n_owned == 0) return;
-#define ZR_LAUNCH_RESOLVE(IM, TB, PPT) hipLaunchKernelGGL((k_resolve_gbuffer<IM, TB, PPT>), dim3(n_owned * (TILE_PIX / (PPT) / (TB))), dim3(TB), 0, s, P, objs, owned_tiles, vis64, G, srgb_lut, unorm_lut, vis_now, stats, vis_mark)
+#define ZR_LAUNCH_RESOLVE(IM, TB, PPT) hipLaunchKernelGGL((k_resolve_gbuffer<IM, TB, PPT>), dim3(n_owned * (TILE_PIX / (PPT) / (TB))), dim3(TB), 0, s, P, objs, owned_tiles, vis64, G, srgb_lut, unorm_lut, vis_now, stats, vis_mark, records)
     if (P.images == 1u) ZR_LAUNCH_RESOLVE(1, 64, ZR_PIXELS_PER_THREAD);
     else if (P.images) ZR_LAUNCH_RESOLVE(2, 64, ZR_PIXELS_PER_THREAD);
     else ZR_LAUNCH_RESOLVE(0, ZR_RESOLVE_TB, ZR_PIXELS_PER_THREAD);
diff --git a/zeldaengine_amd/csrc/zr_rest_record.h b/zeldaengine_amd/csrc/zr_rest_record.h
--- /dev/null
+++ b/zeldaengine_amd/csrc/zr_rest_record.h
@@ -0,0 +1,63 @@
+#pragma once
+#include "zr_dev.h"
+#include "zr_surface.h"
+
+__device__ __forceinline__ bool light_pixel_empty(uint32_t sc, uint32_t A, uint32_t B, uint32_t Cc, uint2 D)
+{
+    return sc == 0xFF000000u && A == 0u && B == 0xFF000000u && Cc == 0xFF000000u && D.x == 0u && D.y == 0x3C000000u;
+}
+
+struct RestBox { float lo[3], hi[3]; bool odd; };
+__device__ __forceinline__ RestBox rest_box_none()
+{
+    return RestBox{ { __builtin_inff(), __builtin_inff(), __builtin_inff() }, { -__builtin_inff(), -__builtin_inff(), -__builtin_inff() }, false };
+}
+__device__ __forceinline__ bool rest_box_counts(uint32_t sc) { return (sc >> 24) != 0u; }
+__device__ __forceinline__ void rest_box_count(RestBox& b, uint2 D)
+{
+    const float q[3] = { f16_to_f32_hw(D.x & 0xFFFFu), f16_to_f32_hw(D.x >> 16), f16_to_f32_hw(D.y & 0xFFFFu) };
+    for (int a = 0; a < 3; ++a) {
+        if (!(__builtin_fabsf(q[a]) <= 3.402823466e38f)) b.odd = true;
+        b.lo[a] = __builtin_fminf(b.lo[a], q[a]); b.hi[a] = __builtin_fmaxf(b.hi[a], q[a]);
+    }
+}
+__device__ __forceinline__ void rest_box_wave(RestBox& b)
+{
+    for (int a = 0; a < 3; ++a) { b.lo[a] = wave_fmin(b.lo[a]); b.hi[a] = wave_fmax(b.hi[a]); }
+    b.odd = __ballot(b.odd) != 0ull;
+}
+__device__ __forceinline__ float rest_box_lo(const RestBox& b, int a) { return b.odd ? -__builtin_inff() : b.lo[a]; }
+__device__ __forceinline__ float rest_box_hi(const RestBox& b, int a) { return b.odd ? __builtin_inff() : b.hi[a]; }
+__device__ __forceinline__ void rest_record_write(ZrRestRecord* __restrict__ r, const RestBox& wave_box, bool empty)
+{
+    const unsigned long long em = __ballot(empty);
+    if ((threadIdx.x & 63u) == 0u) {
+        for (int a = 0; a < 3; ++a) { r->lo[a] = rest_box_lo(wave_box, a); r->hi[a] = rest_box_hi(wave_box, a); }
+        r->empty[0] = (uint32_t)em; r->empty[1] = (uint32_t)(em >> 32);
+    }
+}
+
+template <uint32_t WAVES>
+__device__ __forceinline__ uint32_t rest_records_fetch_at(const ZrRestRecord* __restrict__ recs, uint32_t first_record)
+{
+    constexpr uint32_t RECW = (uint32_t)(sizeof(ZrRestRecord) / 4u);
+    const uint32_t* __restrict__ w = (const uint32_t*)recs + (size_t)first_record * RECW;
+    return w[((threadIdx.x & 7u) % WAVES) * RECW + ((threadIdx.x >> 3) & 7u)];
+}
+template <uint32_t WAVES>
+__device__ __forceinline__ uint32_t rest_records_fetch(const float4* __restrict__ rest, uint32_t first_record)
+{
+    return rest_records_fetch_at<WAVES>((const ZrRestRecord*)(rest + ZR_REST_SLOT), first_record);
+}
+__device__ __forceinline__ void rest_records_box(uint32_t rec, float* blo, float* bhi)
+{
+    int lo, hi;
+    { const int idn = 0x7F800000; int r = (int)rec; ZR_DPP_STEP(op_fmin, 0x111, 0xF); ZR_DPP_STEP(op_fmin, 0x112, 0xF); ZR_DPP_STEP(op_fmin, 0x114, 0xF); lo = r; }
+    { const int idn = (int)0xFF800000; int r = (int)rec; ZR_DPP_STEP(op_fmax, 0x111, 0xF); ZR_DPP_STEP(op_fmax, 0x112, 0xF); ZR_DPP_STEP(op_fmax, 0x114, 0xF); hi = r; }
+    for (int a = 0; a < 3; ++a) { blo[a] = zr_u2f((uint32_t)__builtin_amdgcn_readlane(lo, 8 * a + 7)); bhi[a] = zr_u2f((uint32_t)__builtin_amdgcn_readlane(hi, 8 * (3 + a) + 7)); }
+}
+__device__ __forceinline__ unsigned long long rest_records_empty(uint32_t rec, uint32_t wave)
+{
+    return (unsigned long long)(uint32_t)__builtin_amdgcn_readlane((int)rec, 48 + (int)wave) |
+           (unsigned long long)(uint32_t)__builtin_amdgcn_readlane((int)rec, 56 + (int)wave) << 32;
+}
diff --git a/zeldaengine_amd/csrc/zr_surface.h b/zeldaengine_amd/csrc/zr_surface.h
--- a/zeldaengine_amd/csrc/zr_surface.h
+++ b/zeldaengine_amd/csrc/zr_surface.h
@@ -130,16 +130,19 @@
     return g;
 }
 
+struct GBufferWords { uint32_t sc, A, B, Cc; uint2 D; };
 template <int IMAGES>
 __device__ __forceinline__ bool resolve_pixel(const ZrPass& P, const ZrObject* __restrict__ objs, uint32_t prim, float depth,
                                               int px, int py, const GBufferPtrs& G, const float* __restrict__ lut,
-                                              uint8_t* __restrict__ vis_now, uint32_t vis_mark = 1u)
+                                              uint8_t* __restrict__ vis_now, uint32_t vis_mark = 1u, GBufferWords* words = nullptr)
 {
     const size_t p = (size_t)py * P.W + (size_t)px;
     if (prim == ZR_EMPTY_PRIM) {
-        G.depth[p] = 1.0f; G.scene_color[p] = 0xFF000000u; G.gA[p] = 0u; G.gB[p] = 0xFF000000u; G.gC[p] = 0xFF000000u;
-        G.gD[p] = make_uint2(0u, 0x3C000000u);
+        const GBufferWords w = { 0xFF000000u, 0u, 0xFF000000u, 0xFF000000u, make_uint2(0u, 0x3C000000u) };
+        G.depth[p] = 1.0f; G.scene_color[p] = w.sc; G.gA[p] = w.A; G.gB[p] = w.B; G.gC[p] = w.Cc;
+        G.gD[p] = w.D;
         if (P.write_overlay) G.overlay[p] = 0u;
+        if (words) *words = w;
         return false;
     }
     const PixGeom g = pixel_geom(P, objs, prim, px, py, vis_now, vis_mark);
@@ -150,6 +153,7 @@
     if (O->flags & ZR_OBJ_SKY) {
         const zf4 sk = tex_sample<IMAGES>(O->tex[0], O->texc[0], true, lut, u0, v0, s1, t1, s2, t2);
         G.overlay[p] = pack_rgb8(gamma3(zr3(sk.x, sk.y, sk.z)));
+        if (words) *words = GBufferWords{ G.scene_color[p], G.gA[p], G.gB[p], G.gC[p], G.gD[p] };
         return false;
     }
     if (P.write_overlay) G.overlay[p] = 0u;
@@ -190,11 +194,14 @@
     const zf3 Nw = compute_normal(pos_dx, pos_dy, s1, t1, s2, t2, N0, ts);
     const zf3 Nn = zr_normalize(Nw);
     const zf3 NP = zr3((Nn.x + 1.0f) / 2.0f, (Nn.y + 1.0f) / 2.0f, (Nn.z + 1.0f) / 2.0f);
+    const GBufferWords w = { w_sc, zr_unorm(NP.z, 1023.0f) | zr_unorm(NP.y, 1023.0f) << 10 | zr_unorm(NP.x, 1023.0f) << 20 | 3u << 30, w_gB, w_gC,
+                             make_uint2(f32_to_f16_hw(P0.x) | f32_to_f16_hw(P0.y) << 16, f32_to_f16_hw(P0.z) | 0x3C000000u) };
     G.depth[p] = depth;
-    G.scene_color[p] = w_sc;
-    G.gA[p] = zr_unorm(NP.z, 1023.0f) | zr_unorm(NP.y, 1023.0f) << 10 | zr_unorm(NP.x, 1023.0f) << 20 | 3u << 30;
-    G.gB[p] = w_gB;
-    G.gC[p] = w_gC;
-    G.gD[p] = make_uint2(f32_to_f16_hw(P0.x) | f32_to_f16_hw(P0.y) << 16, f32_to_f16_hw(P0.z) | 0x3C000000u);
+    G.scene_color[p] = w.sc;
+    G.gA[p] = w.A;
+    G.gB[p] = w.B;
+    G.gC[p] = w.Cc;
+    G.gD[p] = w.D;
+    if (words) *words = w;
     return true;
 }
diff --git a/zeldaengine_amd/csrc/zr_types.h b/zeldaengine_amd/csrc/zr_types.h
--- a/zeldaengine_amd/csrc/zr_types.h
+++ b/zeldaengine_amd/csrc/zr_types.h
@@ -280,7 +280,7 @@
                     uint8_t* vis_now, hipStream_t s, uint32_t vis_mark);
 void zr_launch_resolve_gbuffer(const ZrPass& P, const ZrObject* objs, const uint32_t* owned_tiles, uint32_t n_owned,
                                unsigned long long* vis64, const GBufferPtrs& G, const float* srgb_lut, const float* unorm_lut, uint8_t* vis_now,
-                               ZrDevStats* stats, hipStream_t s, uint32_t vis_mark = 1u);
+                               ZrDevStats* stats, hipStream_t s, uint32_t vis_mark, struct ZrRestRecord* records);
 void zr_launch_sky_tiles(const ZrPass& P, const ZrObject* objs, const uint32_t* owned_tiles, uint32_t n_owned, unsigned long long* sky64, hipStream_t s);
 void zr_launch_count_shadow(const uint32_t* bits, size_t n, ZrDevStats* stats, hipStream_t s);
 enum ZrLightMode : uint32_t { ZR_LIGHT_PLAIN = 0u, ZR_LIGHT_FILL = 1u, ZR_LIGHT_KEPT = 2u };
@@ -293,7 +293,8 @@
 static_assert(sizeof(ZrRestRecord) == 32 && sizeof(ZrRestLight) == 32 && sizeof(ZrRestArgs) == 32 + 32 * ZR_REST_ARG_LIGHTS, "zr_types.h: the resting frame's records");
 void zr_launch_lighting(const ZrLightParams& L, const XkView* view, const uint32_t* owned_tiles, uint32_t n_owned,
                         const GBufferPtrs& G, const float* shadowmap, const CubeDesc& C, const float* lut, const float* unorm_lut,
-                        uint32_t* out, hipStream_t s, ZrLightMode mode = ZR_LIGHT_PLAIN, float4* plane = nullptr, float4* rest = nullptr);
+                        uint32_t* out, hipStream_t s, ZrLightMode mode = ZR_LIGHT_PLAIN, float4* plane = nullptr, float4* rest = nullptr,
+                        const ZrRestRecord* records = nullptr);
 bool zr_lighting_rest_available();
 void zr_launch_lighting_rest(const ZrLightParams& L, const ZrRestArgs& R, const uint32_t* owned_tiles, uint32_t n_owned, const GBufferPtrs& G,
                              const float* lut, const float* unorm_lut, uint32_t* out, hipStream_t s, const float4* plane, const float4* rest);
diff --git a/zeldaengine_amd/engine.py b/zeldaengine_amd/engine.py
--- a/zeldaengine_amd/engine.py
+++ b/zeldaengine_amd/engine.py
@@ -57,6 +57,7 @@
         **abi.OVERLAY_SIGNATURES,
         **abi.EXTENT_SIGNATURES,
         **abi.REST_SETTLE_SIGNATURES,
+        **abi.GBUFFER_RECORD_SIGNATURES,
         "zr_set_cubemap": [vp, vp, u32],
         "zr_set_skydome": [vp, vp, u32, vp, u32, vp],
         "zr_set_background": [vp, vp],
@@ -649,6 +650,13 @@
         self._chk(self.L.zr_get_rest_settled_parts(self.h, _ptr(out) if out.size else None, out.nbytes))
         return out
 
+    def gbuffer_records(self, copy=-1, n_owned=None):
+        if n_owned is None:
+            n_owned = ((self.W + 31) // 32) * ((self.H + 31) // 32)
+        out = np.zeros((n_owned, abi.GBUFFER_RECORDS_PER_TILE), dtype=np.dtype(abi.GBUFFER_RECORD_DTYPE))
+        self._chk(self.L.zr_get_gbuffer_records(self.h, int(copy), _ptr(out) if out.size else None, out.nbytes))
+        return out
+
     def color(self):
         out = np.zeros((self.H, self.W, 4), dtype=np.uint8)
         self._chk(self.L.zr_read_color(self.h, _ptr(out), out.nbytes))
```

Measured after the change: 113,400. -1.2%, worse.
